# jxhe/vae-lagging-encoder

Measured on AMD Instinct MI355X. Metric: aggressive-loop seqs/sec, higher is better.
Workload: dtype bf16

## Files before the change

### include/lvae.h

```cpp
#ifndef LVAE_H
#define LVAE_H

#include <stdint.h>

#ifdef __cplusplus
extern "C" {
#endif

int lv_gemm_f32(int transA, int transB, int M, int N, int K, float alpha,
                const float* A, long lda, const float* B, long ldb, float* C, long ldc, int accumulate,
                const float* add1, long ld1, int mod1, const float* add2, long ld2, int mod2,
                float* ws , long ws_floats, void* stream);

int lv_gemm_bf16(int transA, int transB, int M, int N, int K, float alpha,
                 const float* A, long lda, const float* B, long ldb, float* C, long ldc, int accumulate,
                 const float* add1, long ld1, int mod1, const float* add2, long ld2, int mod2,
                 float* ws, long ws_floats, void* stream);

int lv_gemm_b16(int transA, int M, int N, int K, float alpha,
                const uint16_t* A, long lda, const uint16_t* B, long ldb, float* C, long ldc, int accumulate,
                const float* add1, long ld1, int mod1, const float* add2, long ld2, int mod2,
                float* ws, long ws_floats, void* stream);
int lv_gemm_b16_dual_supported(int M, int N, int K, long ws_floats);
int lv_gemm_b16_dual(int transA, int M, int N, int K, const uint16_t* A, long lda, const uint16_t* B, long ldb,
                     float* C1, long ldc1, int nsplit, float* C2, long ldc2, float* ws, long ws_floats, void* stream);
int lv_gemm_b16_pair_supported(int transA0, int M0, int N0, int K0, int transA1, int M1, int N1, int K1, long ws_floats);
int lv_gemm_b16_pair_pending(int* pending, void* stream);
int lv_gemm_b16_pair(int transA0, int M0, int N0, int K0, const uint16_t* A0, long lda0, const uint16_t* B0, long ldb0,
                     float* C0, long ldc0, int nsplit0, float* C0b, long ldc0b,
                     int transA1, int M1, int N1, int K1, const uint16_t* A1, long lda1, const uint16_t* B1, long ldb1,
                     float* C1, long ldc1, float* ws, long ws_floats, void* stream);
int lv_gemm_b16_keep(int M, int N, int K, const uint16_t* A, long lda, const uint16_t* B, long ldb, float* C,
                     const uint8_t* keep, float kscale, int Bsz, float* ws, long ws_floats, void* stream);
int lv_gemm_b16_sumsq_parts(int M, int N, int K, long ws_floats);
int lv_gemm_b16_sumsq(int transA, int M, int N, int K, const uint16_t* A, long lda, const uint16_t* B, long ldb, float* C, long ldc,
                      float* ws, long ws_floats, float* sq, int sq_only, void* stream);
int lv_gemm_b16_nll_parts(int N);
int lv_gemm_b16_tile(int tile, int transA, int M, int N, int K, float alpha,
                     const uint16_t* A, long lda, const uint16_t* B, long ldb, float* C, long ldc, int accumulate,
                     const float* add1, long ld1, int mod1, const float* add2, long ld2, int mod2,
                     float* ws, long ws_floats, void* stream);
int lv_gemm_b16_nll_tile(int tile, int M, int N, int K, const uint16_t* A, long lda, const uint16_t* B, long ldb, uint16_t* logits16,
                         long ldl16, const int64_t* ids, long ids_stride, int tgt_off, int Bsz, float* part, float* tgt_logit,
                         void* stream);
int lv_gemm_b16_nll(int M, int N, int K, const uint16_t* A, long lda, const uint16_t* B, long ldb, uint16_t* logits16, long ldl16,
                    const int64_t* ids, long ids_stride, int tgt_off, int Bsz, float* part, float* tgt_logit, void* stream);
int lv_softmax_nll_merge_f32(const float* part, int nparts, const float* tgt_logit, float* lse, float* nll, int R, void* stream);
int lv_softmax_nll_bwd_h16(const uint16_t* logits16, long ldl, const float* lse, const int64_t* ids, long ids_stride, int tgt_off,
                           const float* rowscale, uint16_t* dlogits, long ldo, int T, int B, int V, void* stream);
int lv_cvt_bf16_f32(const float* src, long lds, int R, int C, uint16_t* dst, long ldd, uint16_t* dstT, long ldt,
                    void* stream);
int lv_cvt_bf16_keep_f32(const float* src, long lds, int T, int Bsz, int C, const uint8_t* keep, float kscale,
                         uint16_t* dst, long ldd, uint16_t* dstT, long ldt, void* stream);
int lv_cvt_bf16_hs3_f32(const float* src, long lds, int T, int Bsz, int C, const uint8_t* keep, float kscale, uint16_t* dst, long ldd,
                        uint16_t* dstT, long ldt, uint16_t* hT, long ldh, void* stream);
int lv_cvt_f32_bf16_scaled(const uint16_t* src, long n, float scale, float* dst, void* stream);
int lv_keep_scale_f32(float* x, const uint8_t* keep, float kscale, int T, int Bsz, int C, void* stream);

int lv_cvt_bf16_gates_f32(const float* src, long lds, int H, int C, uint16_t* dst, long ldd, uint16_t* dstT, long ldt,
                          void* stream);
int lv_cvt_bf16_lo_f32(const float* src, long lds, int R, int C, int gate_H, const int64_t* ids, long ids_stride, int Bsz, int V,
                       uint16_t* dst, long ldd, uint16_t* dstT, long ldt, void* stream);
int lv_cvt_h16_f32(const float* src, long lds, int R, int C, int gate_H, const int64_t* ids, long ids_stride, int Bsz, int V,
                   uint16_t* dst, long ldd, uint16_t* dstT, long ldt, void* stream);
int lv_gemm_h16(int M, int N, int K, float alpha, const uint16_t* A, long lda, const uint16_t* B, long ldb,
                float* C, long ldc, int accumulate, const float* add1, long ld1, int mod1,
                const float* add2, long ld2, int mod2, float* ws, long ws_floats, void* stream);
int lv_transpose_f32(const float* in, float* out, int rows, int cols, void* stream);
int lv_transpose_ld_f32(const float* in, long in_ld, float* out, long out_ld, int rows, int cols, void* stream);

int lv_lstm_fwd_f32(const float* gx, const float* whh, float* hs, float* cs, float* gates,
                    const uint8_t* dmask, float dscale, float* hdrop, float* ws, int T, int B, int H, void* stream);
int lv_lstm_fwd_bf16(const float* gx, const float* whh, float* hs, float* cs, float* gates,
                     const uint8_t* dmask, float dscale, float* hdrop, float* ws, int T, int B, int H, void* stream);
int lv_lstm_fwd_bf16_ug(const float* gx, const float* whh, float* hs, float* cs, float* gates,
                        const uint8_t* dmask, float dscale, float* hdrop, float* ws, int T, int B, int H, void* stream);
int lv_lstm_fwd_f32_ug(const float* gx, const float* whh, float* hs, float* cs, float* gates,
                       const uint8_t* dmask, float dscale, float* hdrop, float* ws, int T, int B, int H, void* stream);
long lv_lstm_persist16_wpk_floats(void);
long lv_lstm_persist16_xch_floats(void);
int lv_lstm_persist16_xch_clear(float* xch, void* stream);
long lv_lstm_persist16_saved_floats(int T, int R);
int lv_lstm_persist16_pack(const float* whh, float* wpk, int backward, int H, void* stream);
int lv_lstm_persist16_pack2(const float* whh, float* wpk_fwd, float* wpk_bwd, int H, void* stream);
int lv_lstm_persist16_pack2_h16(const float* whh, float* wpk_fwd, float* wpk_bwd, int H, void* stream);
int lv_lstm_fwd_bf16_persist16(const float* gx, const float* wpk, float* hs, float* cs, float* saved, float* xch, int* status,
                               int T, int B, int R, int flags, int H, void* stream);
int lv_lstm_bwd_bf16_persist16(const float* dh_ext, const float* dh_last, const float* wpk, const float* saved, const float* hs,
                               const float* cs, uint16_t* dG16, float* dGsum, float* xch, int* status, float* dh0, float* dc0,
                               int tanh_init, int T, int B, int R, int flags, int H, void* stream);
int lv_lstm_persist16_import_saved(const float* gates, const float* cs, float* saved, int T, int B, int R, int H, void* stream);
int lv_gate_interleave_f32(const float* a, const float* b, int R, int H, float* out, void* stream);
int lv_lstm_bwd_bf16(const float* dh_ext, const float* dh_last, const uint8_t* dmask, float dscale,
                     const float* whh, const float* gates, const float* hs, const float* cs,
                     float* dG, float* dGsum, float* ws, float* dh0, float* dc0, int tanh_init,
                     int T, int B, int H, void* stream);
int lv_lstm_bwd_bf16_img(const float* dh_ext, const float* dh_last, const uint8_t* dmask, float dscale,
                           const float* whh, const float* gates, const float* hs, const float* cs,
                           float* dG, uint16_t* dG16, float* dGsum, float* ws, float* dh0, float* dc0, int tanh_init,
                           int T, int B, int H, void* stream);
long lv_lstm_ws_floats(int B, int H);
int lv_lstm_bwd_ksplit(int H);
int lv_lstm_bwd_f32(const float* dh_ext, const float* dh_last, const uint8_t* dmask, float dscale,
                    const float* whh, const float* gates, const float* hs, const float* cs,
                    float* dG, float* dGsum, float* ws, float* dh0, float* dc0, int tanh_init,
                    int T, int B, int H, void* stream);
int lv_lstm_fwd_len_f32(const float* gx, const float* whh, float* hs, float* cs, float* gates,
                        const uint8_t* dmask, float dscale, float* hdrop, float* ws,
                        const int* steps, int max_steps, int T, int B, int H, void* stream);
int lv_lstm_bwd_len_f32(const float* dh_ext, const float* dh_last, const uint8_t* dmask, float dscale,
                        const float* whh, const float* gates, const float* hs, const float* cs,
                        float* dG, float* dGsum, float* ws, float* dh0, float* dc0, int tanh_init,
                        const int* steps, int max_steps, int T, int B, int H, void* stream);
int lv_nll_mask_len_f32(float* nll, const int* steps, int max_steps, int T, int B, void* stream);

int lv_embed_gather_f32(const float* emb, const int64_t* ids, long ids_stride, const uint8_t* mask, float scale,
                        float* X, int T, int B, int ni, int V, void* stream);
int lv_embed_gather_b16(const float* emb, const int64_t* ids, long ids_stride, const uint8_t* keep, float kscale,
                        int T, int Bsz, int C, int V, uint16_t* dst, long ldd, uint16_t* dstT, long ldt, void* stream);
int lv_token_sort(const int64_t* ids, long ids_stride, int T, int B, int V,
                  int* out_rows, int* out_tok, int* tmp , void* stream);
int lv_embed_scatter_f32(const float* dX, const uint8_t* mask, float scale, const int* sorted_rows,
                         const int* sorted_tok, int T, int B, float* dE, int ni, int pad_idx, int accumulate,
                         void* stream);
int lv_embed_scatter_full_f32(const float* dX, const uint8_t* mask, float scale, const int* sorted_rows,
                              const int* sorted_tok, int T, int B, float* dE, int ni, int V, int pad_idx, void* stream);
int lv_embed_scatter_sumsq_parts(int T, int B);
int lv_embed_scatter_full_sumsq_f32(const float* dX, const uint8_t* mask, float scale, const int* sorted_rows,
                                    const int* sorted_tok, int T, int B, float* dE, int ni, int V, int pad_idx, float* sq, int sq_only,
                                    void* stream);
int lv_rows_merge_f32(const int64_t* ids_all, const void* rows_all, int b16, int world, int cap, int ni, int V, float scale,
                      float* dE, void* stream);

int lv_reparam_kl_fwd_f32(const float* mulv, const float* eps, float* z, float* kl, int B, int ns, int nz, void* stream);
int lv_reparam_kl_bwd_f32(const float* mulv, const float* eps, const float* dz, const float* dkl, float* dmulv,
                          int B, int ns, int nz, void* stream);

int lv_softmax_nll_fwd_f32(const float* logits, long ldl, const int64_t* ids, long ids_stride, int tgt_off,
                           float* lse, float* nll, int T, int B, int V, void* stream);
int lv_softmax_nll_bwd_f32(float* logits, long ldl, const float* lse, const int64_t* ids, long ids_stride, int tgt_off,
                           const float* rowscale, int T, int B, int V, void* stream);
int lv_softmax_nll_bwd_b16(const float* logits, long ldl, const float* lse, const int64_t* ids, long ids_stride, int tgt_off,
                           const float* rowscale, uint16_t* dlogits, long ldo, int T, int B, int V, void* stream);
int lv_vae_loss_f32(const float* nll, const float* kl, const float* kl_weight_dev, float* loss, float* rec,
                    int T, int B, void* stream);
int lv_loss_bwd_scales_f32(const float* g_loss, const float* g_rec, const float* g_kl, const float* kl_weight_dev,
                           float* rowscale, float* dkl, int B, void* stream);
int lv_loss_assemble_f32(const float* nll, const float* kl, const float* kl_weight_dev, const float* g_loss,
                         float* loss, float* rec, float* rowscale, float* dkl, float* acc_dev, int T, int B, void* stream);
int lv_loss_assemble_rng_f32(const float* nll, const float* kl, const float* kl_weight_dev, const float* g_loss,
                             float* loss, float* rec, float* rowscale, float* dkl, float* acc, int T, int B,
                             uint64_t* rng_state, uint64_t rng_inc, void* stream);

int lv_gx_expand_add_f32(const float* gxw, const float* zp, float* gx, int Td, int B, int ns, int C, void* stream);
int lv_sample_sum_f32(const float* dg, float* dgs, int Td, int B, int ns, int C, void* stream);
int lv_sample_sum_b16(const uint16_t* dg, long ld_in, uint16_t* dgs, long ld_out, int Td, int B, int ns, int C, void* stream);
int lv_repeat_rows_i64(const int64_t* x, int64_t* x_rep, int B, int T, int ns, void* stream);
int lv_loss_assemble_ns_f32(const float* nll, const float* kl, const float* kl_weight_dev, const float* g_loss,
                            float* loss, float* rec, float* rowscale, float* dkl, float* acc_dev, int T, int B, int ns,
                            void* stream);
int lv_loss_assemble_ns_rng_f32(const float* nll, const float* kl, const float* kl_weight_dev, const float* g_loss,
                                float* loss, float* rec, float* rowscale, float* dkl, float* acc_dev, int T, int B, int ns,
                                uint64_t* rng_state, uint64_t rng_inc, void* stream);

int lv_enc_head_fwd_f32(const float* hT, const float* w_lin, const float* eps, float* mulv, float* z, float* kl,
                        int B, int H, int ns, int nz, void* stream);
int lv_enc_head_bwd_f32(const float* mulv, const float* eps, const float* dz, int dz_parts, const float* dkl,
                        const float* hT, const float* w_lin, float* dmulv, float* dhT, float* gw_lin, int B, int H, int ns,
                        int nz, void* stream);
int lv_dec_init_f32(const float* z, const float* w_trans, const float* w_ih, long ld_wih, int col0, const float* b_ih,
                    const float* b_hh, float* c0, float* h0, float* zp, int unit_major, int B, int H, int nz, void* stream);
int lv_dec_tail_parts(int H);
int lv_dec_tail_bwd_f32(const float* dGsum, const float* dc0, const float* z, const float* w_ih, long ld_wih, int col0,
                        const float* w_trans, float* gw_ih, long ld_gwih, float* gw_trans, float* gb_ih, float* gb_hh,
                        float* dz_parts, int B, int H, int nz, void* stream);

int lv_tanh_f32(const float* in, float* out, long n, void* stream);
int lv_colsum_f32(const float* in, long ld, int R, int C, float* out, float* out2, void* stream);
int lv_add_f32(const float* a, const float* b, float* out, long n, void* stream);
int lv_sum_accum_f32(const float* x, long n, float* out_dev, void* stream);
int lv_add_scalar_f32(float* x_dev, float v, void* stream);

int lv_sumsq_workspace_floats(void);
int lv_sumsq_f32(const float* x, long n, float* ws, float* out_dev, int accumulate, void* stream);
int lv_clip_coef_f32(const float* sumsq_dev, float max_norm, float* coef_dev, float* norm_out_dev, void* stream);
int lv_clip_norm2_f32(const float* g1, long n1, const float* g2, long n2, float* ws, float max_norm,
                      float* sumsq_dev, float* coef_dev, float* norm_dev, void* stream);
int lv_sgd_step_f32(float* p, float* g, long n, const float* lr_dev, const float* coef_dev, int write_back_clipped,
                    void* stream);
int lv_scale_f32(float* x, long n, const float* coef_dev, void* stream);
int lv_clip_norm2_txn_f32(const float* g1, long n1, const float* g2, long n2, float* ws, float max_norm,
                          float* sumsq_dev, float* coef_dev, float* norm_dev, const int* status1, const int* status2,
                          const float* guard, float* txn, float* acc, void* stream);
int lv_clip_norm2_fold_txn_f32(const float* g1, long n1, const float* g2, long n2, float* ws, const float* extra, int n_extra,
                               float max_norm, float* sumsq_dev, float* coef_dev, float* norm_dev, const int* status1,
                               const int* status2, const float* guard, float* txn, float* acc, void* stream);
int lv_clip_coef_txn_f32(const float* sumsq_dev, float max_norm, float* coef_dev, float* norm_out_dev, const int* status1,
                         const int* status2, const float* guard, float* txn, float* acc, void* stream);
int lv_txn_guard_f32(const int* status1, const int* status2, float* guard, void* stream);
int lv_sgd_step_txn_f32(float* p, float* g, long n, const float* lr_dev, const float* coef_dev, int write_back_clipped,
                        const float* void_flag_dev, void* stream);
int lv_scale_txn_f32(float* x, long n, const float* coef_dev, const float* void_flag_dev, void* stream);
int lv_sgd_step_scale_txn_f32(float* p, float* g, long n, const float* lr_dev, const float* coef_dev, int write_back_clipped,
                              float* x2, long n2, const float* void_flag_dev, void* stream);
int lv_sgd_step_scale_rows_txn_f32(float* p, float* g, long n, const float* lr_dev, const float* coef_dev, int write_back_clipped,
                                   float* x2, long n2, const float* void_flag_dev, long emb_off, int V, int ni, const int* sorted_tok,
                                   int N, void* stream);
int lv_sgd_momentum_step_f32(float* p, float* g, float* buf, long n, const float* lr_dev, const float* coef_dev, float momentum,
                             int write_back_clipped, void* stream);
int lv_sgd_momentum_step_txn_f32(float* p, float* g, float* buf, long n, const float* lr_dev, const float* coef_dev, float momentum,
                                 int write_back_clipped, const float* void_flag_dev, void* stream);
int lv_sgd_momentum_step_scale_txn_f32(float* p, float* g, float* buf, long n, const float* lr_dev, const float* coef_dev, float momentum,
                                       int write_back_clipped, float* x2, long n2, const float* void_flag_dev, void* stream);
int lv_adam_step_f32(float* p, float* g, float* m, float* v, long n, const float* lr_dev, const float* coef_dev,
                     const float* step_dev, float beta1, float beta2, float eps, int write_back_clipped, void* stream);
int lv_adam_step_txn_f32(float* p, float* g, float* m, float* v, long n, const float* lr_dev, const float* coef_dev, float* step_dev,
                         double beta1, double beta2, float eps, int write_back_clipped, const float* void_flag_dev, void* stream);
int lv_adam_step_scale_txn_f32(float* p, float* g, float* m, float* v, long n, const float* lr_dev, const float* coef_dev,
                               float* step_dev, double beta1, double beta2, float eps, int write_back_clipped, float* x2, long n2,
                               const float* void_flag_dev, void* stream);

int lv_rng_normal_f32(float* out, long n, const uint64_t* state_dev, uint64_t substream, void* stream);
int lv_rng_keepmask_u8(uint8_t* out, long n, float keep_prob, const uint64_t* state_dev, uint64_t substream, void* stream);
int lv_rng_advance(uint64_t* state_dev, uint64_t inc, void* stream);
int lv_rng_noise_step(float* eps, long n_eps, uint8_t* mask_in, long n_in, float keep_in, uint8_t* mask_out, long n_out,
                      float keep_out, uint64_t* state_dev, uint64_t inc, void* stream);
int lv_rng_bernoulli_f32(const float* p, float* out, long n, const uint64_t* state_dev, uint64_t substream,
                         void* stream);

int lv_gauss_logpdf_f32(const float* z, const float* mu, const float* logvar, float* out, int B, int ns, int nz, void* stream);
int lv_logsumexp_rows_f32(const float* in, long ld, int R, int C, float add, float* out, void* stream);
int lv_calc_mi_f32(const float* mu, const float* logvar, const float* z, float* ws, float* out_dev, int Bx, int Bz, int nz,
                   void* stream);
int lv_au_accum_f32(const float* mu, const float* mean, float* acc_dev, int B, int nz, void* stream);

int lv_dec_cond_ll_f32_supported(int V, int ni, int H, int nz, int T);
long lv_dec_cond_ll_f32_ws_floats(int V, int H, int nz, int B, int T);
int lv_dec_cond_ll_f32(const int64_t* x, int B, int T, const float* z, long z_stride, int K, const float* embed,
                       const float* trans, const float* w_ih, const float* w_hh, const float* b_ih, const float* b_hh,
                       const float* pred, int V, int ni, int H, int nz, float* ws, float* cond_ll, void* stream);
// ... 120 lines not shown
```

### profiles/microbench/lstm_fixed_cost_probe.py

```python
import os, sys, torch
sys.path.insert(0, os.path.dirname(os.path.dirname(os.path.dirname(os.path.abspath(__file__)))))
from vae_lagging_encoder_amd import _lib
from vae_lagging_encoder_amd.engine import P, stream_ptr
dev = torch.device("cuda:0"); s = stream_ptr(dev)
lib = _lib.load()
H, B, R = 1024, 32, 4
whh = (torch.rand(4 * H, H, device=dev) * 2 - 1) * 0.03
n = lib.lv_lstm_persist16_wpk_floats()
wf, wb = torch.empty(n, device=dev), torch.empty(n, device=dev)
lib.lv_lstm_persist16_pack2(P(whh), P(wf), P(wb), H, s)
xch = torch.zeros(lib.lv_lstm_persist16_xch_floats(), device=dev)
st = torch.zeros(1, dtype=torch.int32, device=dev)
from types import SimpleNamespace
from vae_lagging_encoder_amd.engine import _xch_flags
wi = SimpleNamespace(xstate={"f": 0, "g": 0, "gcls": [0, 0]})


def t(f, n=20):
    for _ in range(3): f()
    e0, e1 = torch.cuda.Event(enable_timing=True), torch.cuda.Event(enable_timing=True)
    e0.record()
    for _ in range(n): f()
    e1.record(); torch.cuda.synchronize()
    return e0.elapsed_time(e1) * 1e3 / n


Ts = [1, 2, 4, 8, 16, 50, 100, 200]
rows = []
for mode in ("memset", "alternating halves"):
  rows = []
  lib.lv_lstm_persist16_xch_clear(P(xch), s)
  wi.xstate = {"f": 0, "g": 0, "gcls": [0, 0]}
  FF = (lambda: 1) if mode == "memset" else (lambda: 1 | _xch_flags(wi, "f", R, "cpu"))
  FB = (lambda: 1) if mode == "memset" else (lambda: 1 | _xch_flags(wi, "g", R, "cpu"))
  print("== exchange buffer: %s" % ("zeroed by a memset launch in front of every launch (round 4)" if mode == "memset" else
                                    "halves alternate, every launch clears the other half in its prologue (round 5)"))
  for T in Ts:
      gx = (torch.randn(T, B, 4 * H, device=dev) * 0.5)
      hs = torch.zeros(T + 1, B, H, device=dev); cs = torch.zeros(T + 1, B, H, device=dev)
      saved = torch.empty(lib.lv_lstm_persist16_saved_floats(T, R), device=dev)
      dO = torch.randn(T, B, H, device=dev) * 0.1
      dG16 = torch.empty(T, B, 4 * H, dtype=torch.int16, device=dev)
      dGsum = torch.empty(B, 4 * H, device=dev); dc0 = torch.empty(B, H, device=dev)
      f = t(lambda: lib.lv_lstm_fwd_bf16_persist16(P(gx), P(wf), P(hs), P(cs), P(saved), P(xch), P(st), T, B, R, FF(), H, s))
      b = t(lambda: lib.lv_lstm_bwd_bf16_persist16(P(dO), None, P(wb), P(saved), P(hs), P(cs), P(dG16), P(dGsum), P(xch), P(st), None, P(dc0), 1, T, B, R, FB(), H, s))
      rows.append((T, f, b))
      print("T=%3d: forward %7.1f us, BPTT %7.1f us (back-to-back launches)" % (T, f, b))
  import numpy as np
  A = np.array([[1.0, r[0]] for r in rows])
  for name, col in (("forward", 1), ("BPTT", 2)):
      a, b = np.linalg.lstsq(A, np.array([r[col] for r in rows]), rcond=None)[0]
      print("%s: fixed %.1f us per launch + %.3f us per timestep" % (name, a, b))
print("status", int(st.item()))
```

### vae_lagging_encoder_amd/_lib.py

```python
import ctypes
import os
import threading

from . import build as _build

_vp = ctypes.c_void_p
_i = ctypes.c_int
_l = ctypes.c_long
_f = ctypes.c_float
_d = ctypes.c_double
_u64 = ctypes.c_uint64

SIGNATURES = {
    "lv_gemm_f32": [_i, _i, _i, _i, _i, _f, _vp, _l, _vp, _l, _vp, _l, _i, _vp, _l, _i, _vp, _l, _i, _vp, _l, _vp],
    "lv_gemm_bf16": [_i, _i, _i, _i, _i, _f, _vp, _l, _vp, _l, _vp, _l, _i, _vp, _l, _i, _vp, _l, _i, _vp, _l, _vp],
    "lv_gemm_b16": [_i, _i, _i, _i, _f, _vp, _l, _vp, _l, _vp, _l, _i, _vp, _l, _i, _vp, _l, _i, _vp, _l, _vp],
    "lv_gemm_h16": [_i, _i, _i, _f, _vp, _l, _vp, _l, _vp, _l, _i, _vp, _l, _i, _vp, _l, _i, _vp, _l, _vp],
    "lv_gemm_b16_dual_supported": [_i, _i, _i, _l],
    "lv_gemm_b16_dual": [_i, _i, _i, _i, _vp, _l, _vp, _l, _vp, _l, _i, _vp, _l, _vp, _l, _vp],
    "lv_gemm_b16_pair_supported": [_i, _i, _i, _i, _i, _i, _i, _i, _l],
    "lv_gemm_b16_pair_pending": [_vp, _vp],
    "lv_gemm_b16_pair": [_i, _i, _i, _i, _vp, _l, _vp, _l, _vp, _l, _i, _vp, _l,
                         _i, _i, _i, _i, _vp, _l, _vp, _l, _vp, _l, _vp, _l, _vp],
    "lv_gemm_b16_keep": [_i, _i, _i, _vp, _l, _vp, _l, _vp, _vp, _f, _i, _vp, _l, _vp],
    "lv_gemm_b16_sumsq_parts": [_i, _i, _i, _l],
    "lv_gemm_b16_sumsq": [_i, _i, _i, _i, _vp, _l, _vp, _l, _vp, _l, _vp, _l, _vp, _i, _vp],
    "lv_gemm_b16_nll_parts": [_i],
    "lv_gemm_b16_tile": [_i, _i, _i, _i, _i, _f, _vp, _l, _vp, _l, _vp, _l, _i, _vp, _l, _i, _vp, _l, _i, _vp, _l, _vp],
    "lv_gemm_b16_nll_tile": [_i, _i, _i, _i, _vp, _l, _vp, _l, _vp, _l, _vp, _l, _i, _i, _vp, _vp, _vp],
    "lv_gemm_b16_nll": [_i, _i, _i, _vp, _l, _vp, _l, _vp, _l, _vp, _l, _i, _i, _vp, _vp, _vp],
    "lv_softmax_nll_merge_f32": [_vp, _i, _vp, _vp, _vp, _i, _vp],
    "lv_softmax_nll_bwd_h16": [_vp, _l, _vp, _vp, _l, _i, _vp, _vp, _l, _i, _i, _i, _vp],
    "lv_cvt_bf16_f32": [_vp, _l, _i, _i, _vp, _l, _vp, _l, _vp],
    "lv_cvt_bf16_keep_f32": [_vp, _l, _i, _i, _i, _vp, _f, _vp, _l, _vp, _l, _vp],
    "lv_cvt_bf16_hs3_f32": [_vp, _l, _i, _i, _i, _vp, _f, _vp, _l, _vp, _l, _vp, _l, _vp],
    "lv_cvt_f32_bf16_scaled": [_vp, _l, _f, _vp, _vp],
    "lv_keep_scale_f32": [_vp, _vp, _f, _i, _i, _i, _vp],
    "lv_cvt_bf16_gates_f32": [_vp, _l, _i, _i, _vp, _l, _vp, _l, _vp],
    "lv_cvt_bf16_lo_f32": [_vp, _l, _i, _i, _i, _vp, _l, _i, _i, _vp, _l, _vp, _l, _vp],
    "lv_cvt_h16_f32": [_vp, _l, _i, _i, _i, _vp, _l, _i, _i, _vp, _l, _vp, _l, _vp],
    "lv_gate_interleave_f32": [_vp, _vp, _i, _i, _vp, _vp],
    "lv_lstm_fwd_bf16_ug": [_vp, _vp, _vp, _vp, _vp, _vp, _f, _vp, _vp, _i, _i, _i, _vp],
    "lv_lstm_fwd_f32_ug": [_vp, _vp, _vp, _vp, _vp, _vp, _f, _vp, _vp, _i, _i, _i, _vp],
    "lv_loss_assemble_f32": [_vp, _vp, _vp, _vp, _vp, _vp, _vp, _vp, _vp, _i, _i, _vp],
    "lv_loss_assemble_rng_f32": [_vp, _vp, _vp, _vp, _vp, _vp, _vp, _vp, _vp, _i, _i, _vp, _u64, _vp],
    "lv_gx_expand_add_f32": [_vp, _vp, _vp, _i, _i, _i, _i, _vp],
    "lv_sample_sum_f32": [_vp, _vp, _i, _i, _i, _i, _vp],
    "lv_sample_sum_b16": [_vp, _l, _vp, _l, _i, _i, _i, _i, _vp],
    "lv_repeat_rows_i64": [_vp, _vp, _i, _i, _i, _vp],
    "lv_loss_assemble_ns_f32": [_vp, _vp, _vp, _vp, _vp, _vp, _vp, _vp, _vp, _i, _i, _i, _vp],
    "lv_loss_assemble_ns_rng_f32": [_vp, _vp, _vp, _vp, _vp, _vp, _vp, _vp, _vp, _i, _i, _i, _vp, _u64, _vp],
    "lv_enc_head_fwd_f32": [_vp, _vp, _vp, _vp, _vp, _vp, _i, _i, _i, _i, _vp],
    "lv_enc_head_bwd_f32": [_vp, _vp, _vp, _i, _vp, _vp, _vp, _vp, _vp, _vp, _i, _i, _i, _i, _vp],
    "lv_dec_tail_parts": [_i],
    "lv_dec_init_f32": [_vp, _vp, _vp, _l, _i, _vp, _vp, _vp, _vp, _vp, _i, _i, _i, _i, _vp],
    "lv_dec_tail_bwd_f32": [_vp, _vp, _vp, _vp, _l, _i, _vp, _vp, _l, _vp, _vp, _vp, _vp, _i, _i, _i, _vp],
    "lv_clip_norm2_f32": [_vp, _l, _vp, _l, _vp, _f, _vp, _vp, _vp, _vp],
    "lv_clip_norm2_txn_f32": [_vp, _l, _vp, _l, _vp, _f, _vp, _vp, _vp, _vp, _vp, _vp, _vp, _vp, _vp],
    "lv_clip_norm2_fold_txn_f32": [_vp, _l, _vp, _l, _vp, _vp, _i, _f, _vp, _vp, _vp, _vp, _vp, _vp, _vp, _vp, _vp],
    "lv_clip_coef_txn_f32": [_vp, _f, _vp, _vp, _vp, _vp, _vp, _vp, _vp, _vp],
    "lv_txn_guard_f32": [_vp, _vp, _vp, _vp],
    "lv_sgd_step_txn_f32": [_vp, _vp, _l, _vp, _vp, _i, _vp, _vp],
    "lv_scale_txn_f32": [_vp, _l, _vp, _vp, _vp],
    "lv_sgd_step_scale_txn_f32": [_vp, _vp, _l, _vp, _vp, _i, _vp, _l, _vp, _vp],
    "lv_sgd_step_scale_rows_txn_f32": [_vp, _vp, _l, _vp, _vp, _i, _vp, _l, _vp, _l, _i, _i, _vp, _i, _vp],
    "lv_sgd_momentum_step_f32": [_vp, _vp, _vp, _l, _vp, _vp, _f, _i, _vp],
    "lv_sgd_momentum_step_txn_f32": [_vp, _vp, _vp, _l, _vp, _vp, _f, _i, _vp, _vp],
    "lv_sgd_momentum_step_scale_txn_f32": [_vp, _vp, _vp, _l, _vp, _vp, _f, _i, _vp, _l, _vp, _vp],
    "lv_rng_noise_step": [_vp, _l, _vp, _l, _f, _vp, _l, _f, _vp, _u64, _vp],
    "lv_lstm_persist16_wpk_floats": [],
    "lv_lstm_persist16_xch_floats": [],
    "lv_lstm_persist16_xch_clear": [_vp, _vp],
    "lv_lstm_persist16_saved_floats": [_i, _i],
    "lv_lstm_persist16_pack": [_vp, _vp, _i, _i, _vp],
    "lv_lstm_persist16_import_saved": [_vp, _vp, _vp, _i, _i, _i, _i, _vp],
    "lv_lstm_persist16_pack2": [_vp, _vp, _vp, _i, _vp],
    "lv_lstm_persist16_pack2_h16": [_vp, _vp, _vp, _i, _vp],
    "lv_lstm_fwd_bf16_persist16": [_vp, _vp, _vp, _vp, _vp, _vp, _vp, _i, _i, _i, _i, _i, _vp],
    "lv_lstm_bwd_bf16_persist16": [_vp, _vp, _vp, _vp, _vp, _vp, _vp, _vp, _vp, _vp, _vp, _vp, _i, _i, _i, _i, _i, _i, _vp],
    "lv_transpose_f32": [_vp, _vp, _i, _i, _vp],
    "lv_transpose_ld_f32": [_vp, _l, _vp, _l, _i, _i, _vp],
    "lv_lstm_bwd_ksplit": [_i],
    "lv_lstm_ws_floats": [_i, _i],
    "lv_lstm_fwd_f32": [_vp, _vp, _vp, _vp, _vp, _vp, _f, _vp, _vp, _i, _i, _i, _vp],
    "lv_lstm_bwd_f32": [_vp, _vp, _vp, _f, _vp, _vp, _vp, _vp, _vp, _vp, _vp, _vp, _vp, _i, _i, _i, _i, _vp],
    "lv_lstm_fwd_len_f32": [_vp, _vp, _vp, _vp, _vp, _vp, _f, _vp, _vp, _vp, _i, _i, _i, _i, _vp],
    "lv_lstm_bwd_len_f32": [_vp, _vp, _vp, _f, _vp, _vp, _vp, _vp, _vp, _vp, _vp, _vp, _vp, _i, _vp, _i, _i, _i, _i, _vp],
    "lv_nll_mask_len_f32": [_vp, _vp, _i, _i, _i, _vp],
    "lv_lstm_fwd_bf16": [_vp, _vp, _vp, _vp, _vp, _vp, _f, _vp, _vp, _i, _i, _i, _vp],
    "lv_lstm_bwd_bf16": [_vp, _vp, _vp, _f, _vp, _vp, _vp, _vp, _vp, _vp, _vp, _vp, _vp, _i, _i, _i, _i, _vp],
    "lv_lstm_bwd_bf16_img": [_vp, _vp, _vp, _f, _vp, _vp, _vp, _vp, _vp, _vp, _vp, _vp, _vp, _vp, _i, _i, _i, _i, _vp],
    "lv_embed_gather_f32": [_vp, _vp, _l, _vp, _f, _vp, _i, _i, _i, _i, _vp],
    "lv_embed_gather_b16": [_vp, _vp, _l, _vp, _f, _i, _i, _i, _i, _vp, _l, _vp, _l, _vp],
    "lv_token_sort": [_vp, _l, _i, _i, _i, _vp, _vp, _vp, _vp],
    "lv_embed_scatter_f32": [_vp, _vp, _f, _vp, _vp, _i, _i, _vp, _i, _i, _i, _vp],
    "lv_embed_scatter_full_f32": [_vp, _vp, _f, _vp, _vp, _i, _i, _vp, _i, _i, _i, _vp],
    "lv_embed_scatter_sumsq_parts": [_i, _i],
    "lv_embed_scatter_full_sumsq_f32": [_vp, _vp, _f, _vp, _vp, _i, _i, _vp, _i, _i, _i, _vp, _i, _vp],
    "lv_rows_merge_f32": [_vp, _vp, _i, _i, _i, _i, _i, _f, _vp, _vp],
    "lv_reparam_kl_fwd_f32": [_vp, _vp, _vp, _vp, _i, _i, _i, _vp],
    "lv_reparam_kl_bwd_f32": [_vp, _vp, _vp, _vp, _vp, _i, _i, _i, _vp],
    "lv_softmax_nll_fwd_f32": [_vp, _l, _vp, _l, _i, _vp, _vp, _i, _i, _i, _vp],
    "lv_softmax_nll_bwd_f32": [_vp, _l, _vp, _vp, _l, _i, _vp, _i, _i, _i, _vp],
    "lv_softmax_nll_bwd_b16": [_vp, _l, _vp, _vp, _l, _i, _vp, _vp, _l, _i, _i, _i, _vp],
    "lv_vae_loss_f32": [_vp, _vp, _vp, _vp, _vp, _i, _i, _vp],
    "lv_loss_bwd_scales_f32": [_vp, _vp, _vp, _vp, _vp, _vp, _i, _vp],
    "lv_tanh_f32": [_vp, _vp, _l, _vp],
    "lv_colsum_f32": [_vp, _l, _i, _i, _vp, _vp, _vp],
    "lv_add_f32": [_vp, _vp, _vp, _l, _vp],
    "lv_sumsq_workspace_floats": [],
    "lv_sumsq_f32": [_vp, _l, _vp, _vp, _i, _vp],
    "lv_clip_coef_f32": [_vp, _f, _vp, _vp, _vp],
    "lv_sgd_step_f32": [_vp, _vp, _l, _vp, _vp, _i, _vp],
    "lv_scale_f32": [_vp, _l, _vp, _vp],
    "lv_adam_step_f32": [_vp, _vp, _vp, _vp, _l, _vp, _vp, _vp, _f, _f, _f, _i, _vp],
    "lv_adam_step_txn_f32": [_vp, _vp, _vp, _vp, _l, _vp, _vp, _vp, _d, _d, _f, _i, _vp, _vp],
    "lv_adam_step_scale_txn_f32": [_vp, _vp, _vp, _vp, _l, _vp, _vp, _vp, _d, _d, _f, _i, _vp, _l, _vp, _vp],
    "lv_add_scalar_f32": [_vp, _f, _vp],
    "lv_sum_accum_f32": [_vp, _l, _vp, _vp],
    "lv_gauss_logpdf_f32": [_vp, _vp, _vp, _vp, _i, _i, _i, _vp],
    "lv_logsumexp_rows_f32": [_vp, _l, _i, _i, _f, _vp, _vp],
    "lv_calc_mi_f32": [_vp, _vp, _vp, _vp, _vp, _i, _i, _i, _vp],
    "lv_au_accum_f32": [_vp, _vp, _vp, _i, _i, _vp],
    "lv_argmax_rows_f32": [_vp, _l, _i, _i, _vp, _vp],
    "lv_log_softmax_rows_f32": [_vp, _l, _i, _i, _vp, _vp, _l, _vp],
    "lv_sample_rows_f32": [_vp, _l, _i, _i, _vp, _vp, _vp],
    "lv_rng_normal_f32": [_vp, _l, _vp, _u64, _vp],
    "lv_rng_keepmask_u8": [_vp, _l, _f, _vp, _u64, _vp],
    "lv_rng_advance": [_vp, _u64, _vp],
    "lv_rng_bernoulli_f32": [_vp, _vp, _l, _vp, _u64, _vp],
    "lv_im2col_f32": [_vp, _vp, _l, _i, _i, _i, _i, _i, _i, _i, _i, _i, _i, _i, _vp],
    "lv_col2im_f32": [_vp, _l, _vp, _i, _i, _i, _i, _i, _i, _i, _i, _i, _i, _i, _i, _vp],
    "lv_conv_pack_w_f32": [_vp, _vp, _i, _i, _i, _vp],
    "lv_conv_unpack_dw_f32": [_vp, _vp, _i, _i, _i, _i, _vp],
    "lv_conv32_wpack_floats": [_i],
    "lv_conv32_pack_f32": [_vp, _vp, _i, _i, _i, _vp],
    "lv_conv32_f32": [_vp, _vp, _vp, _i, _i, _i, _i, _i, _vp],
    "lv_conv32_wgrad_slabs": [_i, _i],
    "lv_conv32_wgrad_ws_floats": [_i, _i],
    "lv_conv32_wgrad_f32": [_vp, _vp, _vp, _vp, _i, _i, _i, _vp],
    "lv_conv1x1_f32": [_vp, _vp, _vp, _l, _i, _i, _i, _i, _vp],
    "lv_conv1x1_wgrad_ws_floats": [_i, _i],
    "lv_conv32_pack_b16": [_vp, _vp, _i, _i, _i, _vp],
    "lv_conv32_b16": [_vp, _vp, _vp, _vp, _i, _i, _i, _i, _i, _i, _vp],
    "lv_conv32_bnbwd": [_vp, _vp, _vp, _vp, _i, _i, _i, _vp, _vp, _vp, _vp, _i, _i, _vp],
    "lv_conv1x1_bnbwd_f32": [_vp, _vp, _vp, _vp, _l, _i, _i, _vp, _vp, _vp, _vp, _i, _vp],
    "lv_bn_bwd_apply_partials_f32": [_vp, _vp, _vp, _i, _vp, _vp, _vp, _vp, _vp, _vp, _i, _l, _i, _vp],
    "lv_conv32_wgrad_b16": [_vp, _vp, _vp, _vp, _i, _i, _i, _i, _vp],
    "lv_conv32_wgrad_parts": [_i, _i],
    "lv_conv1x1_wgrad_parts": [_l],
    "lv_wgrad_reduce_batched": [_vp, _i, _vp],
    "lv_conv32_blocks": [_i],
    "lv_conv32_bnstat_f32": [_vp, _vp, _vp, _vp, _i, _i, _i, _vp],
    "lv_conv1x1_blocks": [_l],
    "lv_conv1x1_bnstat_f32": [_vp, _vp, _vp, _vp, _l, _i, _i, _vp],
    "lv_bn_fwd_partials_f32": [_vp, _vp, _vp, _vp, _i, _vp, _vp, _vp, _vp, _vp, _f, _f, _vp, _i, _l, _i, _vp],
    "lv_conv1x1_wgrad_f32": [_vp, _vp, _vp, _vp, _l, _i, _i, _i, _vp],
    "lv_mul_inplace_f32": [_vp, _vp, _l, _vp],
    "lv_bn_workspace_floats": [_i],
    "lv_pixelcnn_net_words": [],
    "lv_pixelcnn_block_words": [],
    "lv_pixelcnn_pixel_step_f32": [_vp, _i, _i, _i, _vp],
    "lv_conv32_tap_split": [_i],
    "lv_bn_eval_f32": [_vp, _vp, _vp, _vp, _vp, _f, _vp, _i, _vp, _vp, _vp, _l, _i, _vp],
    "lv_bn_fwd_f32": [_vp, _vp, _vp, _vp, _i, _vp, _vp, _vp, _vp, _vp, _f, _f, _vp, _l, _i, _vp],
    "lv_bn_bwd_f32": [_vp, _vp, _vp, _vp, _vp, _vp, _i, _vp, _vp, _vp, _vp, _i, _vp, _l, _i, _vp],
    "lv_bn_bwd2_f32": [_vp, _vp, _vp, _vp, _vp, _vp, _vp, _i, _vp, _vp, _vp, _vp, _i, _vp, _l, _i, _vp],
    "lv_bn_bwd4_f32": [_vp, _vp, _vp, _vp, _vp, _vp, _vp, _vp, _vp, _i, _vp, _vp, _vp, _vp, _i, _vp, _l, _i, _vp],
    "lv_sigmoid_bce_fwd_f32": [_vp, _vp, _vp, _i, _i, _f, _vp],
    "lv_sigmoid_bce_bwd_f32": [_vp, _vp, _vp, _vp, _i, _i, _f, _vp],
    "lv_dec_input_fwd_f32": [_vp, _vp, _vp, _i, _i, _i, _vp],
    "lv_dec_input_bwd_f32": [_vp, _vp, _i, _i, _i, _vp],
    "lv_sigmoid_bce_ns_fwd_f32": [_vp, _vp, _vp, _i, _i, _i, _f, _vp],
    "lv_sigmoid_bce_ns_bwd_f32": [_vp, _vp, _vp, _vp, _i, _i, _i, _f, _vp],
    "lv_dec_input_ns_fwd_f32": [_vp, _vp, _vp, _i, _i, _i, _i, _vp],
    "lv_bn_partial_floats": [_l, _i],
    "lv_bn_finish_fwd_f32": [_vp, _i, _l, _i, _f, _f, _vp, _vp, _vp, _vp, _vp],
    "lv_bn_fwd_stats_f32": [_vp, _vp, _vp, _vp, _i, _vp, _vp, _vp, _l, _i, _vp],
    "lv_bn_finish_bwd_f32": [_vp, _i, _i, _vp, _vp, _vp, _i, _vp],
    "lv_bn_bwd_stats_f32": [_vp, _vp, _vp, _vp, _vp, _vp, _vp, _l, _i, _vp],
    "lv_dec_cond_ll_f32_supported": [_i, _i, _i, _i, _i],
    "lv_dec_cond_ll_f32_ws_floats": [_i, _i, _i, _i, _i],
    "lv_dec_cond_ll_f32": [_vp, _i, _i, _vp, _l, _i, _vp, _vp, _vp, _vp, _vp, _vp, _vp, _i, _i, _i, _i, _vp, _vp, _vp],
    "lv_grid_posterior_f32": [_vp, _vp, _l, _i, _i, _i, _vp, _vp, _vp],
    "lv_mh_chain_f32_supported": [_i, _i, _i, _i, _i],
    "lv_mh_chain_f32_ws_floats": [_i, _i, _i, _i, _i],
    "lv_mh_chain_prep_f32": [_vp, _i, _i, _vp, _vp, _vp, _vp, _vp, _vp, _vp, _i, _i, _i, _i, _vp, _vp],
    "lv_mh_chain_f32": [_vp, _i, _i, _vp, _i, _i, _i, _i, _vp, _vp, _vp, _vp, _vp, _i, _i, _i, _i, _i, _f, _i, _vp, _vp, _vp, _vp],
    "lv_mh_step_f32": [_vp, _vp, _vp, _vp, _vp, _vp, _vp, _f, _vp, _i, _i, _i, _i, _i, _i, _vp, _vp, _vp],
    "lv_beam_supported": [_i, _i, _i],
    "lv_beam_ws_floats": [_i, _i, _i],
    "lv_beam_init_f32": [_vp, _vp, _vp, _vp, _vp, _vp, _vp, _vp, _vp, _vp, _i, _i, _i, _i, _i, _vp],
    "lv_beam_select_f32": [_vp, _l, _vp, _vp, _vp, _vp, _vp, _vp, _i, _i, _i, _vp],
    "lv_beam_advance_f32": [_vp, _vp, _vp, _vp, _vp, _vp, _vp, _vp, _vp, _vp, _vp, _vp, _vp, _i, _i, _i, _i, _i, _i, _i, _vp],
    "lv_beam_backtrace": [_vp, _vp, _vp, _vp, _vp, _vp, _vp, _vp, _i, _i, _i, _i, _vp],
    "lv_rollout_init_f32": [_vp, _vp, _vp, _vp, _vp, _vp, _vp, _vp, _vp, _vp, _i, _i, _i, _i, _vp],
    "lv_rollout_pick_f32": [_vp, _l, _vp, _vp, _vp, _vp, _vp, _vp, _vp, _vp, _vp, _vp, _vp, _vp, _i, _i, _i, _i, _i, _i, _vp],
}


_LONG_FNS = ("lv_lstm_ws_floats", "lv_conv1x1_wgrad_ws_floats", "lv_conv1x1_blocks", "lv_lstm_persist16_wpk_floats", "lv_lstm_persist16_xch_floats", "lv_lstm_persist16_saved_floats", "lv_conv32_wpack_floats",
             "lv_conv32_wgrad_ws_floats", "lv_dec_cond_ll_f32_ws_floats", "lv_beam_ws_floats", "lv_bn_partial_floats",
             "lv_mh_chain_f32_ws_floats")


class LvaeError(RuntimeError):
    pass


class Lib(object):

    def __init__(self, cdll, path):
        self.cdll = cdll
        self.path = path
        missing = []
        for name, argtypes in SIGNATURES.items():
            try:
                fn = getattr(cdll, name)
            except AttributeError:
                missing.append(name)
                continue
            fn.argtypes = argtypes
            fn.restype = ctypes.c_long if name in _LONG_FNS else ctypes.c_int
            setattr(self, "_raw_" + name, fn)
        if missing:
            raise LvaeError("%s does not export: %s" % (path, ", ".join(missing)))
        self._value_fns = {"lv_gemm_b16_dual_supported", "lv_gemm_b16_pair_supported", "lv_lstm_bwd_ksplit", "lv_dec_tail_parts", "lv_gemm_b16_nll_parts", "lv_gemm_b16_sumsq_parts", "lv_embed_scatter_sumsq_parts", "lv_conv32_wpack_floats",
                           "lv_conv32_wgrad_slabs", "lv_conv32_wgrad_ws_floats", "lv_conv32_wgrad_parts", "lv_conv1x1_wgrad_parts", "lv_conv32_blocks", "lv_conv1x1_blocks", "lv_conv1x1_wgrad_ws_floats", "lv_sumsq_workspace_floats", "lv_lstm_ws_floats", "lv_bn_workspace_floats",
                           "lv_lstm_persist16_wpk_floats", "lv_lstm_persist16_xch_floats", "lv_lstm_persist16_saved_floats",
                           "lv_pixelcnn_net_words", "lv_pixelcnn_block_words", "lv_conv32_tap_split", "lv_dec_cond_ll_f32_supported",
                           "lv_dec_cond_ll_f32_ws_floats", "lv_beam_supported", "lv_beam_ws_floats", "lv_bn_partial_floats",
# ... 47 lines not shown
```

### vae_lagging_encoder_amd/csrc/lv_device.h

```cpp
#pragma once

#ifdef LV_EMU
#include "hip_emu.h"
#define LV_LAUNCH(kern, grid, block, shmem, stream, ...) \
    lv_emu::launch((grid), (block), (shmem), [=]() { kern(__VA_ARGS__); })
#define LV_DYN_SHARED(name) char* name = lv_emu::dyn_smem()
static inline f32x4 lv_mfma_16x16x4(float a, float b, f32x4 c) { return lv_emu_mfma_16x16x4(a, b, c); }
static inline f32x16 lv_mfma_32x32x2(float a, float b, f32x16 c) { return lv_emu_mfma_32x32x2(a, b, c); }
#define LV_SCHED_BARRIER() do { } while (0)
static inline int lv_wave_uniform(int v) { return v; }
#define LV_LAUNCH_RESIDENT(kern, grid, block, shmem, stream, ...) \
    lv_emu::launch_concurrent((grid), (block), (shmem), [=]() { kern(__VA_ARGS__); })
#define LV_BLOCK_SHARED(T, name) T& name = *reinterpret_cast<T*>(lv_emu::block_shared(sizeof(T)))
static inline unsigned long long lv_agent_load_u64(const unsigned long long* p) {
    lv_emu::yield_all();
    return __atomic_load_n(p, __ATOMIC_RELAXED);
}
static inline void lv_agent_store_u64(unsigned long long* p, unsigned long long v) { __atomic_store_n(p, v, __ATOMIC_RELAXED); }
static inline void lv_xcd_store_u64(unsigned long long* p, unsigned long long v) { __atomic_store_n(p, v, __ATOMIC_RELAXED); }
static inline void lv_poll_backoff() { }
#define LV_WAIT_LDS() lv_emu::wave_sync()
template <class T> static inline void lv_store_nt(T v, T* p) { *p = v; }
static inline int lv_device_cus() { return 1 << 20; }
#define LV_SPIN_LIMIT (1 << 15)
// ... 30 lines not shown
    }
    lv_emu::wave_sync();
    uint2 r;
    memcpy(&r, o, 8);
    return r;
}
template <int SHIFT, int BANK> static inline float lv_row_shr_into(float old, float src) {
    auto& w = lv_emu::my_wave();
    const int l = lv_emu::lane();
    uint32_t b;
    memcpy(&b, &src, 4);
    w.u[l] = b;
    lv_emu::wave_sync();
    float out = old;
    if (((l & 15) >> 2) == BANK && (l & 15) >= SHIFT) { const uint32_t v = (uint32_t)w.u[l - SHIFT]; memcpy(&out, &v, 4); }
    lv_emu::wave_sync();
    return out;
}
static inline float lv_sat_f16(float x) { return x != x ? x : fminf(fmaxf(x, -65504.f), 65504.f); }
static inline uint16_t lv_f32_to_f16_bits(float x) {
    uint32_t u;
    memcpy(&u, &x, 4);
    const uint32_t sign = (u >> 16) & 0x8000u;
    u &= 0x7FFFFFFFu;
    if (u >= 0x7F800000u) return (uint16_t)(sign | (u > 0x7F800000u ? 0x7E00u : 0x7C00u));
    if (u >= 0x477FF000u) return (uint16_t)(sign | 0x7C00u);
    if (u < 0x33000001u) return (uint16_t)sign;
    if (u < 0x38800000u) {
        const int shift = 126 - (int)(u >> 23);
        const uint32_t mant = (u & 0x7FFFFFu) | 0x800000u;
        uint32_t h = mant >> shift;
        const uint32_t rem = mant & ((1u << shift) - 1u), half = 1u << (shift - 1);
        if (rem > half || (rem == half && (h & 1u))) ++h;
        return (uint16_t)(sign | h);
    }
    uint32_t h = ((u - 0x38000000u) >> 13);
    const uint32_t rem = u & 0x1FFFu;
    if (rem > 0x1000u || (rem == 0x1000u && (h & 1u))) ++h;
    return (uint16_t)(sign | h);
}
static inline float lv_f16_bits_to_f32(uint16_t h) {
    const uint32_t sign = ((uint32_t)h & 0x8000u) << 16, e = (h >> 10) & 0x1Fu, m = h & 0x3FFu;
    uint32_t u;
    if (e == 0) {
        if (m == 0) u = sign;
        else {
            int sh = 0;
            uint32_t mm = m;
            while (!(mm & 0x400u)) { mm <<= 1; ++sh; }
            u = sign | ((uint32_t)(113 - sh) << 23) | ((mm & 0x3FFu) << 13);
        }
    } else if (e == 31) u = sign | 0x7F800000u | (m << 13);
    else u = sign | ((e + 112u) << 23) | (m << 13);
    float f;
    memcpy(&f, &u, 4);
    return f;
}
static inline float lv_lane_xor1(float v) { return __shfl_xor(v, 1, 64); }
static inline uint32_t lv_lane_xor1_u32(uint32_t v) { return (uint32_t)__shfl_xor((int)v, 1, 64); }
template <int I> static inline uint32_t lv_quad_bcast_u32(uint32_t v) { return (uint32_t)lv_emu_xchg((int)v, (lv_emu::lane() & ~3) + I); }
static inline float lv_add_xor16(float x) { return x + __shfl_xor(x, 16, 64); }
static inline float lv_add_xor32(float x) { return x + __shfl_xor(x, 32, 64); }
static inline float lv_add_xor8(float x) { return x + __shfl_xor(x, 8, 64); }
static inline float lv_fold8(float x, float y) {
    const float xs = __shfl_xor(x, 8, 64), ys = __shfl_xor(y, 8, 64);
    return (lv_emu::lane() & 8) ? ys + y : x + xs;
}
static inline float lv_fold16(float x, float y) {
    const float xs = __shfl_xor(x, 16, 64), ys = __shfl_xor(y, 16, 64);
    return (lv_emu::lane() & 16) ? ys + y : x + xs;
}
static inline float lv_fold32(float x, float y) {
    const float xs = __shfl_xor(x, 32, 64), ys = __shfl_xor(y, 32, 64);
    return (lv_emu::lane() & 32) ? ys + y : x + xs;
}
static inline void lv_agent_load_q4x4(const void* p0, const void* p1, const void* p2, const void* p3, uint4 (&v)[4]) {
    lv_emu::yield_all();
    const void* ps[4] = {p0, p1, p2, p3};
    for (int i = 0; i < 4; ++i) {
        const unsigned* q = static_cast<const unsigned*>(ps[i]);
        v[i] = make_uint4(__atomic_load_n(q, __ATOMIC_RELAXED), __atomic_load_n(q + 1, __ATOMIC_RELAXED),
                          __atomic_load_n(q + 2, __ATOMIC_RELAXED), __atomic_load_n(q + 3, __ATOMIC_RELAXED));
    }
}
static inline void lv_agent_load_q4x8(const void* const (&ps)[8], uint4 (&v)[8]) {
    lv_emu::yield_all();
    for (int i = 0; i < 8; ++i) {
        const unsigned* q = static_cast<const unsigned*>(ps[i]);
        v[i] = make_uint4(__atomic_load_n(q, __ATOMIC_RELAXED), __atomic_load_n(q + 1, __ATOMIC_RELAXED),
                          __atomic_load_n(q + 2, __ATOMIC_RELAXED), __atomic_load_n(q + 3, __ATOMIC_RELAXED));
    }
}
static inline void lv_agent_load_q4x8_rows(const char* p, uint4 (&v)[8]) {
    const void* ps[8];
    for (int i = 0; i < 8; ++i) ps[i] = p + i * 4096;
    lv_agent_load_q4x8(ps, v);
}
template <int S> static inline void lv_agent_load_q4x8_rs(const char* p, uint4 (&v)[8]) {
    const void* ps[8];
    for (int i = 0; i < 8; ++i) ps[i] = p + (i & 3) * S + (i >> 2) * 128;
    lv_agent_load_q4x8(ps, v);
}
static inline void lv_agent_store_q4(void* p, uint4 v) {
    unsigned* q = static_cast<unsigned*>(p);
    __atomic_store_n(q + 2, v.z, __ATOMIC_RELAXED); __atomic_store_n(q + 3, v.w, __ATOMIC_RELAXED);
    lv_emu::yield_all();
    __atomic_store_n(q, v.x, __ATOMIC_RELAXED); __atomic_store_n(q + 1, v.y, __ATOMIC_RELAXED);
}
static inline void lv_xcd_store_q4(void* p, uint4 v) { lv_agent_store_q4(p, v); }
static inline uint32_t lv_pack_f16x2(float lo, float hi) { return (uint32_t)lv_f32_to_f16_bits(lo) | ((uint32_t)lv_f32_to_f16_bits(hi) << 16); }
static inline f32x16 lv_mfma_32x32x16_f16(uint4 a, uint4 b, f32x16 c) {
    auto& w = lv_emu::my_wave();
    const int l = lv_emu::lane();
    w.qa[l] = a; w.qb[l] = b;
    lv_emu::wave_sync();
    f32x16 d = c;
    const int col = l & 31;
    for (int r = 0; r < 16; ++r) {
        const int row = (r & 3) + 8 * (r >> 2) + 4 * (l >> 5);
        float acc = c[r];
        for (int h = 0; h < 2; ++h) {
            unsigned short ea[8], eb[8];
            memcpy(ea, &w.qa[row + 32 * h], 16);
            memcpy(eb, &w.qb[col + 32 * h], 16);
            for (int e = 0; e < 8; ++e) acc = fmaf(lv_f16_bits_to_f32(ea[e]), lv_f16_bits_to_f32(eb[e]), acc);
        }
        d[r] = acc;
    }
    lv_emu::wave_sync();
    return d;
}
static inline f32x4 lv_mfma_16x16x32_f16_areg(uint4 a, uint4 b, f32x4 c) {
    auto& w = lv_emu::my_wave();
    const int l = lv_emu::lane();
    w.qa[l] = a; w.qb[l] = b;
    lv_emu::wave_sync();
    f32x4 d = c;
    const int col = l & 15;
    for (int r = 0; r < 4; ++r) {
        const int row = (l >> 4) * 4 + r;
        float acc = c[r];
        for (int g = 0; g < 4; ++g) {
            unsigned short ea[8], eb[8];
            memcpy(ea, &w.qa[row + 16 * g], 16);
            memcpy(eb, &w.qb[col + 16 * g], 16);
            for (int e = 0; e < 8; ++e) acc = fmaf(lv_f16_bits_to_f32(ea[e]), lv_f16_bits_to_f32(eb[e]), acc);
        }
        d[r] = acc;
    }
    lv_emu::wave_sync();
    return d;
}
static inline f32x4 lv_mfma_16x16x32_f16_areg_first(uint4 a, uint4 b) { return lv_mfma_16x16x32_f16_areg(a, b, f32x4{0.f, 0.f, 0.f, 0.f}); }
#else
#include <hip/hip_runtime.h>
typedef float f32x4 __attribute__((ext_vector_type(4)));
typedef float f32x16 __attribute__((ext_vector_type(16)));
#define LV_LAUNCH(kern, grid, block, shmem, stream, ...) \
    hipLaunchKernelGGL(kern, (grid), (block), (shmem), (hipStream_t)(stream), __VA_ARGS__)
#define LV_DYN_SHARED(name) extern __shared__ __attribute__((aligned(16))) char name[]
#define LV_SCHED_BARRIER() __builtin_amdgcn_sched_barrier(0)
__device__ __forceinline__ int lv_wave_uniform(int v) { return __builtin_amdgcn_readfirstlane(v); }
#define LV_LAUNCH_RESIDENT(kern, grid, block, shmem, stream, ...) LV_LAUNCH(kern, grid, block, shmem, stream, __VA_ARGS__)
#define LV_BLOCK_SHARED(T, name) __shared__ T name
__device__ __forceinline__ unsigned long long lv_agent_load_u64(const unsigned long long* p) {
    return __hip_atomic_load(p, __ATOMIC_RELAXED, __HIP_MEMORY_SCOPE_AGENT);
}
__device__ __forceinline__ void lv_agent_store_u64(unsigned long long* p, unsigned long long v) {
    __hip_atomic_store(p, v, __ATOMIC_RELAXED, __HIP_MEMORY_SCOPE_AGENT);
}
__device__ __forceinline__ void lv_xcd_store_u64(unsigned long long* p, unsigned long long v) {
    __hip_atomic_store(p, v, __ATOMIC_RELAXED, __HIP_MEMORY_SCOPE_WORKGROUP);
}
#define LV_SPIN_LIMIT (1 << 22)
#define LV_WAIT_LDS() __builtin_amdgcn_s_waitcnt(0xc07f)
template <class T> __device__ __forceinline__ void lv_store_nt(T v, T* p) { __builtin_nontemporal_store(v, p); }
static inline int lv_device_cus() {
    static int cache[64];
    int dev = 0;
    if (hipGetDevice(&dev) != hipSuccess || dev < 0 || dev >= 64) return 0;
    int c = __atomic_load_n(&cache[dev], __ATOMIC_RELAXED);
    if (c == 0) {
        if (hipDeviceGetAttribute(&c, hipDeviceAttributeMultiprocessorCount, dev) != hipSuccess) return 0;
        __atomic_store_n(&cache[dev], c, __ATOMIC_RELAXED);
    }
    return c;
}
__device__ __forceinline__ f32x4 lv_mfma_16x16x4(float a, float b, f32x4 c) {
    return __builtin_amdgcn_mfma_f32_16x16x4f32(a, b, c, 0, 0, 0);
}
__device__ __forceinline__ f32x16 lv_mfma_32x32x2(float a, float b, f32x16 c) {
    return __builtin_amdgcn_mfma_f32_32x32x2f32(a, b, c, 0, 0, 0);
}
typedef __bf16 lv_bf16x8 __attribute__((ext_vector_type(8)));
__device__ __forceinline__ f32x16 lv_mfma_32x32x16_bf16(uint4 a, uint4 b, f32x16 c) {
    return __builtin_amdgcn_mfma_f32_32x32x16_bf16(*reinterpret_cast<lv_bf16x8*>(&a), *reinterpret_cast<lv_bf16x8*>(&b),
                                                   c, 0, 0, 0);
}
__device__ __forceinline__ f32x4 lv_mfma_16x16x32_bf16(uint4 a, uint4 b, f32x4 c) {
    return __builtin_amdgcn_mfma_f32_16x16x32_bf16(*reinterpret_cast<lv_bf16x8*>(&a), *reinterpret_cast<lv_bf16x8*>(&b),
                                                   c, 0, 0, 0);
}
typedef unsigned int lv_u32x4v __attribute__((ext_vector_type(4)));
__device__ __forceinline__ f32x4 lv_mfma_16x16x32_bf16_areg(uint4 a, uint4 b, f32x4 c) {
    const lv_u32x4v av = {a.x, a.y, a.z, a.w}, bv = {b.x, b.y, b.z, b.w};
    asm volatile("v_mfma_f32_16x16x32_bf16 %0, %1, %2, %0" : "+v"(c) : "a"(av), "v"(bv));
    return c;
}
__device__ __forceinline__ f32x4 lv_mfma_16x16x32_bf16_areg_first(uint4 a, uint4 b) {
    const lv_u32x4v av = {a.x, a.y, a.z, a.w}, bv = {b.x, b.y, b.z, b.w};
    f32x4 c;
    asm volatile("v_mfma_f32_16x16x32_bf16 %0, %1, %2, 0" : "=v"(c) : "a"(av), "v"(bv));
    return c;
}
typedef _Float16 lv_f16x8 __attribute__((ext_vector_type(8)));
__device__ __forceinline__ f32x16 lv_mfma_32x32x16_f16(uint4 a, uint4 b, f32x16 c) {
    return __builtin_amdgcn_mfma_f32_32x32x16_f16(*reinterpret_cast<lv_f16x8*>(&a), *reinterpret_cast<lv_f16x8*>(&b), c, 0, 0, 0);
}
__device__ __forceinline__ f32x4 lv_mfma_16x16x32_f16_areg(uint4 a, uint4 b, f32x4 c) {
    const lv_u32x4v av = {a.x, a.y, a.z, a.w}, bv = {b.x, b.y, b.z, b.w};
    asm volatile("v_mfma_f32_16x16x32_f16 %0, %1, %2, %0" : "+v"(c) : "a"(av), "v"(bv));
    return c;
}
__device__ __forceinline__ f32x4 lv_mfma_16x16x32_f16_areg_first(uint4 a, uint4 b) {
    const lv_u32x4v av = {a.x, a.y, a.z, a.w}, bv = {b.x, b.y, b.z, b.w};
    f32x4 c;
    asm volatile("v_mfma_f32_16x16x32_f16 %0, %1, %2, 0" : "=v"(c) : "a"(av), "v"(bv));
    return c;
}
#define LV_MFMA_DRAIN() asm volatile("s_nop 15\n\ts_nop 3" ::: "memory")
__device__ __forceinline__ void LV_MFMA_RESULT(f32x4& c) { asm volatile("" : "+v"(c)); }
typedef short lv_s16x4 __attribute__((ext_vector_type(4)));
__device__ __forceinline__ f32x4 lv_mfma_4x4x4_16b_bf16(uint2 a, uint2 b, f32x4 c) {
    return __builtin_amdgcn_mfma_f32_4x4x4bf16_1k(*reinterpret_cast<lv_s16x4*>(&a), *reinterpret_cast<lv_s16x4*>(&b), c, 0, 0, 0);
}
__device__ __forceinline__ void lv_glds16(const void* g, void* lds_wave_base) {
    __builtin_amdgcn_global_load_lds((const __attribute__((address_space(1))) void*)g,
                                     (__attribute__((address_space(3))) void*)lds_wave_base, 16, 0, 0);
}
#ifndef LV_GLDS_POLICY
#define LV_GLDS_POLICY ""
#endif
__device__ __forceinline__ void lv_glds16_uncounted(const void* g, void* lds_wave_base) {
    unsigned keep;
    const unsigned dst = (unsigned)__builtin_amdgcn_readfirstlane((int)(unsigned)(uintptr_t)(__attribute__((address_space(3))) void*)lds_wave_base);
    asm volatile("s_mov_b32 %0, m0\n\ts_mov_b32 m0, %2\n\ts_nop 0\n\tglobal_load_lds_dwordx4 %1, off" LV_GLDS_POLICY "\n\ts_mov_b32 m0, %0"
                 : "=&s"(keep) : "v"(g), "s"(dst) : "memory");
}
#define LV_WAIT_VMEM() asm volatile("s_waitcnt vmcnt(0)" ::: "memory")
typedef float lv_f32x4_wt __attribute__((ext_vector_type(4)));
__device__ __forceinline__ void lv_store_wt_f4(float4* p, float4 v) {
    const lv_f32x4_wt x = {v.x, v.y, v.z, v.w};
    asm volatile("global_store_dwordx4 %0, %1, off sc1\n\ts_nop 1" :: "v"(p), "v"(x) : "memory");
}
__device__ __forceinline__ void lv_acquire_agent() { __builtin_amdgcn_fence(__ATOMIC_ACQUIRE, "agent"); }
__device__ __forceinline__ unsigned lv_agent_load_u32(const unsigned* p) { return __hip_atomic_load(p, __ATOMIC_RELAXED, __HIP_MEMORY_SCOPE_AGENT); }
__device__ __forceinline__ void lv_sleep_short() { __builtin_amdgcn_s_sleep(8); }
#define LV_ARRIVAL_POLLS 64
#define LV_WAIT_VMEM_N(n) asm volatile("s_waitcnt vmcnt(" #n ")" ::: "memory")
#define LV_S_BARRIER() __builtin_amdgcn_s_barrier()
#define LV_SETPRIO(n) __builtin_amdgcn_s_setprio(n)
typedef short lv_s16x4_lds __attribute__((ext_vector_type(4)));
__device__ __forceinline__ uint2 lv_ds_read_tr16_b64(const void* lds_ptr) {
    lv_s16x4_lds v = __builtin_amdgcn_ds_read_tr16_b64_v4i16((__attribute__((address_space(3))) lv_s16x4_lds*)lds_ptr);
    return *reinterpret_cast<uint2*>(&v);
}
__device__ __forceinline__ float lv_sat_f16(float x) { return x != x ? x : fminf(fmaxf(x, -65504.f), 65504.f); }
__device__ __forceinline__ uint16_t lv_f32_to_f16_bits(float x) {
    const _Float16 h = (_Float16)x;
    uint16_t b;
    __builtin_memcpy(&b, &h, 2);
    return b;
}
__device__ __forceinline__ float lv_f16_bits_to_f32(uint16_t b) {
    _Float16 h;
    __builtin_memcpy(&h, &b, 2);
    return (float)h;
}
__device__ __forceinline__ float lv_lane_xor1(float v) {
    const int r = __builtin_amdgcn_update_dpp(0, __builtin_bit_cast(int, v), 0xB1, 0xF, 0xF, true);
    return __builtin_bit_cast(float, r);
}
__device__ __forceinline__ uint32_t lv_lane_xor1_u32(uint32_t v) {
    return (uint32_t)__builtin_amdgcn_update_dpp(0, (int)v, 0xB1, 0xF, 0xF, true);
}
template <int I> __device__ __forceinline__ uint32_t lv_quad_bcast_u32(uint32_t v) {
    return (uint32_t)__builtin_amdgcn_update_dpp(0, (int)v, I * 0x55, 0xF, 0xF, true);
}
__device__ __forceinline__ float lv_add_xor16(float x) {
    const auto r = __builtin_amdgcn_permlane16_swap(__builtin_bit_cast(unsigned, x), __builtin_bit_cast(unsigned, x), false, false);
    return __builtin_bit_cast(float, (unsigned)r[0]) + __builtin_bit_cast(float, (unsigned)r[1]);
}
__device__ __forceinline__ float lv_add_xor32(float x) {
    const auto r = __builtin_amdgcn_permlane32_swap(__builtin_bit_cast(unsigned, x), __builtin_bit_cast(unsigned, x), false, false);
    return __builtin_bit_cast(float, (unsigned)r[0]) + __builtin_bit_cast(float, (unsigned)r[1]);
}
__device__ __forceinline__ float lv_add_xor8(float x) {
    const int r = __builtin_amdgcn_update_dpp(0, __builtin_bit_cast(int, x), 0x128, 0xF, 0xF, true);
    return x + __builtin_bit_cast(float, r);
}
__device__ __forceinline__ float lv_fold8(float x, float y) {
    const float xs = lv_add_xor8(x), ys = lv_add_xor8(y);
    return (threadIdx.x & 8) ? ys : xs;
}
__device__ __forceinline__ float lv_fold16(float x, float y) {
    const auto r = __builtin_amdgcn_permlane16_swap(__builtin_bit_cast(unsigned, x), __builtin_bit_cast(unsigned, y), false, false);
    return __builtin_bit_cast(float, (unsigned)r[0]) + __builtin_bit_cast(float, (unsigned)r[1]);
}
__device__ __forceinline__ float lv_fold32(float x, float y) {
    const auto r = __builtin_amdgcn_permlane32_swap(__builtin_bit_cast(unsigned, x), __builtin_bit_cast(unsigned, y), false, false);
    return __builtin_bit_cast(float, (unsigned)r[0]) + __builtin_bit_cast(float, (unsigned)r[1]);
}
__device__ __forceinline__ void lv_agent_load_q4x4(const void* p0, const void* p1, const void* p2, const void* p3, uint4 (&v)[4]) {
    lv_u32x4v r0, r1, r2, r3;
    asm volatile("global_load_dwordx4 %0, %4, off sc1\n\tglobal_load_dwordx4 %1, %5, off sc1\n\tglobal_load_dwordx4 %2, %6, off sc1\n\t"
                 "global_load_dwordx4 %3, %7, off sc1\n\ts_waitcnt vmcnt(0)"
                 : "=&v"(r0), "=&v"(r1), "=&v"(r2), "=&v"(r3) : "v"(p0), "v"(p1), "v"(p2), "v"(p3) : "memory");
    v[0] = make_uint4(r0.x, r0.y, r0.z, r0.w); v[1] = make_uint4(r1.x, r1.y, r1.z, r1.w);
    v[2] = make_uint4(r2.x, r2.y, r2.z, r2.w); v[3] = make_uint4(r3.x, r3.y, r3.z, r3.w);
}
__device__ __forceinline__ void lv_agent_load_q4x8(const void* const (&ps)[8], uint4 (&v)[8]) {
    lv_u32x4v r0, r1, r2, r3, r4, r5, r6, r7;
    asm volatile("global_load_dwordx4 %0, %8, off sc1\n\tglobal_load_dwordx4 %1, %9, off sc1\n\tglobal_load_dwordx4 %2, %10, off sc1\n\t"
                 "global_load_dwordx4 %3, %11, off sc1\n\tglobal_load_dwordx4 %4, %12, off sc1\n\tglobal_load_dwordx4 %5, %13, off sc1\n\t"
                 "global_load_dwordx4 %6, %14, off sc1\n\tglobal_load_dwordx4 %7, %15, off sc1\n\ts_waitcnt vmcnt(0)"
                 : "=&v"(r0), "=&v"(r1), "=&v"(r2), "=&v"(r3), "=&v"(r4), "=&v"(r5), "=&v"(r6), "=&v"(r7)
                 : "v"(ps[0]), "v"(ps[1]), "v"(ps[2]), "v"(ps[3]), "v"(ps[4]), "v"(ps[5]), "v"(ps[6]), "v"(ps[7]) : "memory");
    v[0] = make_uint4(r0.x, r0.y, r0.z, r0.w); v[1] = make_uint4(r1.x, r1.y, r1.z, r1.w);
    v[2] = make_uint4(r2.x, r2.y, r2.z, r2.w); v[3] = make_uint4(r3.x, r3.y, r3.z, r3.w);
    v[4] = make_uint4(r4.x, r4.y, r4.z, r4.w); v[5] = make_uint4(r5.x, r5.y, r5.z, r5.w);
    v[6] = make_uint4(r6.x, r6.y, r6.z, r6.w); v[7] = make_uint4(r7.x, r7.y, r7.z, r7.w);
}
__device__ __forceinline__ void lv_agent_load_q4x8_rows(const char* p, uint4 (&v)[8]) {
    const char *p1 = p + 4096, *p3 = p + 3 * 4096, *p5 = p + 5 * 4096, *p7 = p + 7 * 4096;
    lv_u32x4v r0, r1, r2, r3, r4, r5, r6, r7;
    asm volatile("global_load_dwordx4 %0, %8, off offset:-4096 sc1\n\tglobal_load_dwordx4 %1, %8, off sc1\n\t"
                 "global_load_dwordx4 %2, %9, off offset:-4096 sc1\n\tglobal_load_dwordx4 %3, %9, off sc1\n\t"
                 "global_load_dwordx4 %4, %10, off offset:-4096 sc1\n\tglobal_load_dwordx4 %5, %10, off sc1\n\t"
                 "global_load_dwordx4 %6, %11, off offset:-4096 sc1\n\tglobal_load_dwordx4 %7, %11, off sc1\n\ts_waitcnt vmcnt(0)"
                 : "=&v"(r0), "=&v"(r1), "=&v"(r2), "=&v"(r3), "=&v"(r4), "=&v"(r5), "=&v"(r6), "=&v"(r7)
                 : "v"(p1), "v"(p3), "v"(p5), "v"(p7) : "memory");
    v[0] = make_uint4(r0.x, r0.y, r0.z, r0.w); v[1] = make_uint4(r1.x, r1.y, r1.z, r1.w);
    v[2] = make_uint4(r2.x, r2.y, r2.z, r2.w); v[3] = make_uint4(r3.x, r3.y, r3.z, r3.w);
    v[4] = make_uint4(r4.x, r4.y, r4.z, r4.w); v[5] = make_uint4(r5.x, r5.y, r5.z, r5.w);
    v[6] = make_uint4(r6.x, r6.y, r6.z, r6.w); v[7] = make_uint4(r7.x, r7.y, r7.z, r7.w);
}
template <int S> __device__ __forceinline__ void lv_agent_load_q4x8_rs(const char* p, uint4 (&v)[8]) {
    static_assert(3 * S + 128 < 8192, "two address registers reach 8 KB");
    const char* const ph = p + 4096;
#define LV_RS_O(i) (((i) & 3) * S + ((i) >> 2) * 128)
#define LV_RS_P(i) (LV_RS_O(i) < 4096 ? p : ph)
    lv_u32x4v r0, r1, r2, r3, r4, r5, r6, r7;
    asm volatile("global_load_dwordx4 %0, %8, off offset:%16 sc1\n\tglobal_load_dwordx4 %1, %9, off offset:%17 sc1\n\t"
                 "global_load_dwordx4 %2, %10, off offset:%18 sc1\n\tglobal_load_dwordx4 %3, %11, off offset:%19 sc1\n\t"
                 "global_load_dwordx4 %4, %12, off offset:%20 sc1\n\tglobal_load_dwordx4 %5, %13, off offset:%21 sc1\n\t"
                 "global_load_dwordx4 %6, %14, off offset:%22 sc1\n\tglobal_load_dwordx4 %7, %15, off offset:%23 sc1\n\ts_waitcnt vmcnt(0)"
                 : "=&v"(r0), "=&v"(r1), "=&v"(r2), "=&v"(r3), "=&v"(r4), "=&v"(r5), "=&v"(r6), "=&v"(r7)
                 : "v"(LV_RS_P(0)), "v"(LV_RS_P(1)), "v"(LV_RS_P(2)), "v"(LV_RS_P(3)), "v"(LV_RS_P(4)), "v"(LV_RS_P(5)), "v"(LV_RS_P(6)), "v"(LV_RS_P(7)),
                   "n"(LV_RS_O(0) & 4095), "n"(LV_RS_O(1) & 4095), "n"(LV_RS_O(2) & 4095), "n"(LV_RS_O(3) & 4095),
                   "n"(LV_RS_O(4) & 4095), "n"(LV_RS_O(5) & 4095), "n"(LV_RS_O(6) & 4095), "n"(LV_RS_O(7) & 4095)
                 : "memory");
#undef LV_RS_O
#undef LV_RS_P
    v[0] = make_uint4(r0.x, r0.y, r0.z, r0.w); v[1] = make_uint4(r1.x, r1.y, r1.z, r1.w);
    v[2] = make_uint4(r2.x, r2.y, r2.z, r2.w); v[3] = make_uint4(r3.x, r3.y, r3.z, r3.w);
    v[4] = make_uint4(r4.x, r4.y, r4.z, r4.w); v[5] = make_uint4(r5.x, r5.y, r5.z, r5.w);
    v[6] = make_uint4(r6.x, r6.y, r6.z, r6.w); v[7] = make_uint4(r7.x, r7.y, r7.z, r7.w);
}
__device__ __forceinline__ void lv_agent_store_q4(void* p, uint4 v) {
    const lv_u32x4v d = {v.x, v.y, v.z, v.w};
    asm volatile("global_store_dwordx4 %0, %1, off sc1\n\ts_nop 1" :: "v"(p), "v"(d) : "memory");
}
#ifndef LV_POLL_SLEEP
#define LV_POLL_SLEEP 0
#endif
__device__ __forceinline__ void lv_poll_backoff() { if (LV_POLL_SLEEP > 0) __builtin_amdgcn_s_sleep(LV_POLL_SLEEP); }
#ifndef LV_XCD_ST_MODS
#define LV_XCD_ST_MODS ""
#endif
__device__ __forceinline__ void lv_xcd_store_q4(void* p, uint4 v) {
// ... 99 lines not shown
```

### vae_lagging_encoder_amd/csrc/lv_lstm_persist16.hip

```cpp
#include "lv_device.h"
#include "lv_persist_common.h"

#if defined(LV_TRACE) && !defined(LV_EMU)
__device__ unsigned long long* lv_trace_buf = nullptr;
extern "C" int lv_trace_set(void* p) { return (int)hipMemcpyToSymbol(HIP_SYMBOL(lv_trace_buf), &p, sizeof(p)); }
#endif

#ifndef LV_SBB16
#define LV_SBB16 8
#endif
#ifndef LV_HB16
#define LV_HB16 2
#endif
#ifndef LV_SBK16
#define LV_SBK16 4
#endif
#ifndef LV_GJ16
#define LV_GJ16 16
#endif
#ifndef LV_FWD_Q
#define LV_FWD_Q 2
#endif
#ifndef LV_RS_Q
#define LV_RS_Q 2
#endif
#ifndef LV_P16_ABL
#define LV_P16_ABL 0
#endif

namespace {

using namespace lvp;

__device__ __forceinline__ float abl_u2f(uint32_t u) { float f; memcpy(&f, &u, 4); return f; }

constexpr int HP16 = PH / 2 + 8;
constexpr int DP16 = 64 + 8;
constexpr int RED_SLOTS = 33;
constexpr int SAVED_PER_ROW = 160;
constexpr int RS16_SLOTS_MAX = 256;
template <int V> struct lv_const { static constexpr int value = V; };

__global__ __launch_bounds__(256) void pack_w_k16_kernel(const float* __restrict__ whh, uint4* __restrict__ wpk, int f16);
__global__ __launch_bounds__(256) void pack_w_rs16_kernel(const float* __restrict__ whh, uint4* __restrict__ wpk);

__device__ __forceinline__ void pack_w_k16_one(const float* __restrict__ whh, uint4* __restrict__ wpk, long idx, int f16 = 0) {
    const int l = (int)(idx & 63), nb = (int)((idx >> 6) & 7), ks = (int)((idx >> 9) & 7);
    const int wave_id = (int)(idx >> 12), m = wave_id >> 2, w = wave_id & 3;
    const int c = l & 15, kq = l >> 4, col = 16 * nb + c;
    const float* row = whh + ((long)(col & 3) * PH + 32 * m + (col >> 2)) * PH + 256 * w + 32 * ks + 8 * kq;
    if (f16) {
        float r[8];
#pragma unroll
        for (int e = 0; e < 8; ++e) r[e] = lv_sat_f16(row[e]);
        wpk[idx] = make_uint4(lv_pack_f16x2(r[0], r[1]), lv_pack_f16x2(r[2], r[3]), lv_pack_f16x2(r[4], r[5]), lv_pack_f16x2(r[6], r[7]));
    }
    else
        wpk[idx] = make_uint4(lv_pack_bf16x2(row[0], row[1]), lv_pack_bf16x2(row[2], row[3]), lv_pack_bf16x2(row[4], row[5]),
                              lv_pack_bf16x2(row[6], row[7]));
}
__device__ __forceinline__ void pack_w_rs16_one(const float* __restrict__ whh, uint4* __restrict__ wpk, long idx) {
    const int l = (int)(idx & 63), nb = (int)((idx >> 6) & 15), ks = (int)((idx >> 10) & 3);
    const int wave_id = (int)(idx >> 12), m = wave_id >> 2, w = wave_id & 3;
    const int c = l & 15, kq = l >> 4, j = 256 * w + 16 * nb + c;
    float v[8];
#pragma unroll
    for (int e = 0; e < 8; ++e) {
        const int n2 = 32 * ks + 8 * kq + e;
        v[e] = whh[((long)(n2 & 3) * PH + 32 * m + (n2 >> 2)) * PH + j];
    }
    wpk[idx] = make_uint4(lv_pack_bf16x2(v[0], v[1]), lv_pack_bf16x2(v[2], v[3]), lv_pack_bf16x2(v[4], v[5]), lv_pack_bf16x2(v[6], v[7]));
}
__global__ __launch_bounds__(256) void pack_w_both16_kernel(const float* __restrict__ whh, uint4* __restrict__ wfwd, uint4* __restrict__ wbwd,
                                                            int fwd_f16) {
    const long n = 128L * 64 * 64;
    const long idx = (long)blockIdx.x * 256 + threadIdx.x;
    if (idx < n) pack_w_k16_one(whh, wfwd, idx, fwd_f16);
    else if (idx < 2 * n) pack_w_rs16_one(whh, wbwd, idx - n);
}

__global__ __launch_bounds__(256) void pack_w_k16_kernel(const float* __restrict__ whh, uint4* __restrict__ wpk, int f16) {
    const long idx = (long)blockIdx.x * 256 + threadIdx.x;
    if (idx < 128L * 8 * 8 * 64) pack_w_k16_one(whh, wpk, idx, f16);
}
__global__ __launch_bounds__(256) void pack_w_rs16_kernel(const float* __restrict__ whh, uint4* __restrict__ wpk) {
    const long idx = (long)blockIdx.x * 256 + threadIdx.x;
    if (idx < 128L * 4 * 16 * 64) pack_w_rs16_one(whh, wpk, idx);
}

struct Fwd16P {
    const float* gx; const uint4* wpk;
    float* hs; float* cs; float* saved;
    gran_t* hx;
    int* status;
    int T, B, R;
    uint4* clr; long clr_n;
};

__device__ __forceinline__ void clear_other_half(uint4* q, long n) {
    if (!q) return;
    const long stride = (long)gridDim.x * blockDim.x;
    for (long i = (long)blockIdx.x * blockDim.x + threadIdx.x; i < n; i += stride) q[i] = make_uint4(0u, 0u, 0u, 0u);
}

template <int RP> struct Cfg16 {
    static constexpr int NP = RP > 8 ? 2 : 1;
    static constexpr int SBK = RP > 8 ? LV_SBK16 : 8;
    static constexpr int SBB = RP > 8 ? LV_SBB16 : 8;
    static constexpr int GJ = RP > 8 ? LV_GJ16 : (RP > 4 ? 16 : 8);
};

template <int RP>
struct __attribute__((aligned(16))) Fwd16Lds {
    uint32_t hl[RP * HP16];
    f32x4 red[2][4][RP][RED_SLOTS];
    uint32_t dump[256];
    int abort;
};

template <int RP, bool LOCAL, bool F16 = false>
__global__ __launch_bounds__(256) void lstm_fwd_persist_k16_kernel(Fwd16P p) {
    auto h16 = [](float v) -> uint32_t { return F16 ? (uint32_t)lv_f32_to_f16_bits(v) : lv_f32_to_bf16_bits(v); };
    auto put = [](gran_t* q, gran_t v) { if (LOCAL) lv_xcd_store_u64(q, v); else gran_store(q, v); };
    constexpr int NP = Cfg16<RP>::NP, SBK = Cfg16<RP>::SBK, GJ = Cfg16<RP>::GJ;
    LV_BLOCK_SHARED(Fwd16Lds<RP>, sm);
    int& s_abort = sm.abort;
    const int tid = (int)threadIdx.x, l = tid & 63, w = tid >> 6;
    const int group = (int)blockIdx.x % PGROUPS, member = (int)blockIdx.x / PGROUPS;
    const int wave_id = member * 4 + w;
    const int B = p.B, R = p.R, T = p.T;
    const int b0 = group * R;
    const int rows = (b0 >= B) ? 0 : ((B - b0) < R ? (B - b0) : R);
    clear_other_half(p.clr, p.clr_n);
    if (rows == 0) return;
    if (tid == 0) s_abort = 0;

    uint4 wreg[8][8];
    {
        const uint4* wp = p.wpk + (long)wave_id * 8 * 8 * 64 + l;
#pragma unroll
        for (int ks = 0; ks < 8; ++ks)
#pragma unroll
            for (int nb = 0; nb < 8; ++nb) wreg[ks][nb] = wp[(ks * 8 + nb) * 64];
    }

    const int uw = tid & 31, punit = 32 * member + uw;
    const long BH = (long)B * PH;
    const long rec = (long)R * SAVED_PER_ROW;
    float* const sv = p.saved + (long)(group * PMEMBERS + member) * T * rec;
    int prow[NP]; bool own[NP]; long pidx[NP]; float c_state[NP]; int sg[NP], sc[NP];
#pragma unroll
    for (int q = 0; q < NP; ++q) {
        prow[q] = (tid >> 5) + 8 * q;
        own[q] = prow[q] < rows;
        pidx[q] = (long)(b0 + (own[q] ? prow[q] : 0)) * PH + punit;
        c_state[q] = own[q] ? p.cs[pidx[q]] : 0.f;
        sg[q] = (prow[q] * 32 + uw) * 4;
        sc[q] = R * 128 + prow[q] * 32 + uw;
    }
    gran_t* const hx_g = p.hx + (long)group * 16 * (PH / 2);
    const long hx_par = (long)PGROUPS * 16 * (PH / 2);
    const bool even = !(uw & 1);

    constexpr bool QF = LV_FWD_Q == 2 || (RP == 4 && LV_FWD_Q == 1);
    auto tagq = [](int state) -> uint32_t { return 1u + (uint32_t)state % 0xFFFFu; };
    auto publish_q = [&](int state, int q, float hval) {
        const uint32_t dw = h16(hval) | (tagq(state) << 16);
        const uint32_t d1 = lv_quad_bcast_u32<1>(dw), d2 = lv_quad_bcast_u32<2>(dw), d3 = lv_quad_bcast_u32<3>(dw);
        if (own[q] && !(uw & 3)) {
            char* d = reinterpret_cast<char*>(hx_g + (long)(state & 1) * hx_par + (long)prow[q] * (PH / 2)) + (punit >> 2) * 16;
            if (LOCAL) lv_xcd_store_q4(d, make_uint4(dw, d1, d2, d3)); else lv_agent_store_q4(d, make_uint4(dw, d1, d2, d3));
        }
    };
#pragma unroll
    for (int q = 0; q < NP; ++q) {
        if constexpr (QF) { publish_q(0, q, own[q] ? p.hs[pidx[q]] : 0.f); continue; }
        const uint32_t mine = h16(own[q] ? p.hs[pidx[q]] : 0.f);
        const uint32_t next = lv_lane_xor1_u32(mine);
        if (own[q] && even) put(hx_g + (long)prow[q] * (PH / 2) + (punit >> 1), ((gran_t)1u << 32) | (gran_t)(mine | (next << 16)));
    }

    float4 gxb[NP][SBK];
    f32x4 recb[NP][SBK];
    float cb[NP][SBK], hb[NP][SBK];
    auto load_slots = [&](int tb, int lo, int hi) {
#pragma unroll
        for (int q = 0; q < NP; ++q)
#pragma unroll
            for (int s2 = 0; s2 < SBK; ++s2) {
                if (s2 < lo || s2 >= hi) continue;
                const int t = tb + s2 < T ? tb + s2 : T - 1;
                gxb[q][s2] = *reinterpret_cast<const float4*>(p.gx + ((long)t * BH + pidx[q]) * 4);
            }
    };
    auto store_block = [&](int tb) {
#pragma unroll
        for (int q = 0; q < NP; ++q)
#pragma unroll
            for (int s2 = 0; s2 < SBK; ++s2) {
                const int t = tb + s2;
                if (own[q] && t < T) {
                    lv_store_nt(recb[q][s2],
                                reinterpret_cast<f32x4*>(sv + (long)t * rec + sg[q]));
                    lv_store_nt(cb[q][s2], sv + (long)t * rec + sc[q]);
                    lv_store_nt(hb[q][s2], p.hs + (long)(t + 1) * BH + pidx[q]);
                    if (t == T - 1) p.cs[(long)T * BH + pidx[q]] = cb[q][s2];
                }
            }
    };
    load_slots(0, 0, SBK);
    __syncthreads();

    const int nq = rows * 128;
    const int brow = (l & 15) < rows ? (l & 15) : 0;
    const int kq = l >> 4;
    uint32_t abl_keep[8] = {0u, 0u, 0u, 0u, 0u, 0u, 0u, 0u};
    for (int tb = 0; tb < T; tb += SBK) {
#pragma unroll
        for (int s2 = 0; s2 < SBK; ++s2) {
            const int t = tb + s2;
            if (t >= T) break;
            LV_TRACE_MARK(t, 0);
            const gran_t* src = hx_g + (long)(t & 1) * hx_par + 128 * w;
            const uint32_t want = (uint32_t)(t + 1);
            if constexpr (QF) {
                constexpr int QR = RP == 4 ? 4 : 8;
                const char* sq = reinterpret_cast<const char*>(hx_g + (long)(t & 1) * hx_par) + (64 * w + l) * 16;
                const long rowb = (long)(PH / 2) * 8;
                const uint32_t wq = tagq(t) << 16;
                auto round = [&](auto R0) {
                    constexpr int r0 = decltype(R0)::value;
                    if (r0 >= rows) return;
                    uint4 v[QR];
                    int spins = 0;
                    bool ok;
                    do {
                        if constexpr (QR == 4)
                            lv_agent_load_q4x4(sq, sq + (rows > 1 ? rowb : 0), sq + (rows > 2 ? 2 * rowb : 0), sq + (rows > 3 ? 3 * rowb : 0), v);
                        else {
                            static_assert((PH / 2) * 8 == 4096, "lv_agent_load_q4x8_rows: rows 4 KB apart");
                            lv_agent_load_q4x8_rows(sq + r0 * rowb, reinterpret_cast<uint4 (&)[8]>(v));
                        }
                        uint32_t x = 0u;
#pragma unroll
                        for (int j = 0; j < QR; ++j)
                            if (r0 + j < rows) x |= (v[j].x ^ wq) | (v[j].y ^ wq) | (v[j].z ^ wq) | (v[j].w ^ wq);
                        ok = (LV_P16_ABL & 2) ? true : (x >> 16) == 0u;
                        ok = __all(ok);
                        if (!ok && ++spins > SPIN_LIMIT) { s_abort = 1; break; }
                        if (!ok) lv_poll_backoff();
                    } while (!ok);
                    LV_TRACE_VAL(t, 6, spins);
#pragma unroll
                    for (int j = 0; j < QR; ++j)
                        if (r0 + j < rows)
                            *reinterpret_cast<uint2*>(&sm.hl[(r0 + j) * HP16 + 128 * w + 2 * l]) =
                                make_uint2((v[j].x & 0xFFFFu) | (v[j].y << 16), (v[j].z & 0xFFFFu) | (v[j].w << 16));
                };
                round(lv_const<0>());
                if constexpr (RP > QR) round(lv_const<QR>());
            } else
            for (int base = 0; base < nq; base += 64 * GJ) {
                gran_t v[GJ];
                int spins = 0;
                bool ok;
                do {
                    ok = true;
#pragma unroll
                    for (int j = 0; j < GJ; ++j) {
                        const int q = base + j * 64 + l;
                        const bool in = q < nq;
                        if constexpr (LV_P16_ABL & 32) { v[j] = ((gran_t)want << 32) | (gran_t)(uint32_t)(q + t); continue; }
                        v[j] = gran_load(src + (in ? (q >> 7) * (PH / 2) + (q & 127) : 0));
                        if (!(LV_P16_ABL & 2)) ok = ok && (!in || (uint32_t)(v[j] >> 32) == want);
                    }
                    ok = __all(ok);
                    if (!ok && ++spins > SPIN_LIMIT) { s_abort = 1; break; }
                } while (!ok);
                LV_TRACE_VAL(t, 6, spins);
                if constexpr (LV_P16_ABL & 16) {
#pragma unroll
                    for (int j = 0; j < GJ; ++j) abl_keep[j & 7] ^= (uint32_t)v[j];
                } else {
#pragma unroll
                for (int j = 0; j < GJ; ++j) {
                    const int q = base + j * 64 + l;
                    uint32_t* dstw = q < nq ? &sm.hl[(q >> 7) * HP16 + 128 * w + (q & 127)] : &sm.dump[tid];
                    *dstw = (uint32_t)v[j];
                }
                }
            }
            if (s2 == 0 && tb > 0) { store_block(tb - SBK); load_slots(tb, SBK - 1, SBK); }
            if (s2 == SBK - 1) load_slots(tb + SBK, 0, SBK - 1);
            LV_TRACE_MARK(t, 1);
            LV_WAIT_LDS();
            LV_TRACE_MARK(t, 2);

            f32x4 acc[8];
            const uint4* bp = reinterpret_cast<const uint4*>(sm.hl + brow * HP16 + 128 * w) + kq;
            uint4 bfr[8];
            if constexpr (LV_P16_ABL & 16) {
#pragma unroll
                for (int ks = 0; ks < 8; ++ks) bfr[ks] = make_uint4(abl_keep[ks], abl_keep[(ks + 1) & 7], abl_keep[(ks + 2) & 7], abl_keep[(ks + 3) & 7]);
            } else {
#pragma unroll
            for (int ks = 0; ks < 8; ++ks) bfr[ks] = bp[ks * 4];
            }
            LV_SCHED_BARRIER();
            if constexpr (LV_P16_ABL & 1) {
#pragma unroll
                for (int nb = 0; nb < 8; ++nb) acc[nb] = f32x4{abl_u2f(bfr[nb].x), abl_u2f(bfr[nb].y), 0.f, 0.f};
            } else {
#pragma unroll
            for (int ks = 0; ks < 8; ++ks)
#pragma unroll
                for (int nb = 0; nb < 8; ++nb)
                    if constexpr (F16)
                        acc[nb] = ks == 0 ? lv_mfma_16x16x32_f16_areg_first(wreg[0][nb], bfr[0]) : lv_mfma_16x16x32_f16_areg(wreg[ks][nb], bfr[ks], acc[nb]);
                    else
                        acc[nb] = ks == 0 ? lv_mfma_16x16x32_bf16_areg_first(wreg[0][nb], bfr[0]) : lv_mfma_16x16x32_bf16_areg(wreg[ks][nb], bfr[ks], acc[nb]);
            LV_MFMA_DRAIN();
#pragma unroll
            for (int nb = 0; nb < 8; ++nb) LV_MFMA_RESULT(acc[nb]);
            }
            if ((l & 15) < RP) {
                f32x4* rd = sm.red[t & 1][w][l & 15];
#pragma unroll
                for (int nb = 0; nb < 8; ++nb) rd[4 * nb + kq] = acc[nb];
            }
            LV_TRACE_MARK(t, 3);
            if (!(LV_P16_ABL & 8))
            __syncthreads();
            LV_TRACE_MARK(t, 4);
            if (s_abort) { if (tid == 0) atomicExch(p.status, 100 + t); return; }

#pragma unroll
            for (int q = 0; q < NP; ++q) {
                float h = 0.f;
                if (own[q]) {
                    const f32x4 q0 = sm.red[t & 1][0][prow[q]][uw], q1 = sm.red[t & 1][1][prow[q]][uw];
                    const f32x4 q2 = sm.red[t & 1][2][prow[q]][uw], q3 = sm.red[t & 1][3][prow[q]][uw];
                    const float4 gxv = gxb[q][s2];
                    auto sg_ = [](float x) { return (LV_P16_ABL & 4) ? 0.5f + 0.25f * x : lv_sigmoid_fast(x); };
                    auto th_ = [](float x) { return (LV_P16_ABL & 4) ? 0.9f * x : lv_tanh_fast(x); };
                    const float ig = sg_(gxv.x + ((q0[0] + q1[0]) + (q2[0] + q3[0])));
                    const float fg = sg_(gxv.y + ((q0[1] + q1[1]) + (q2[1] + q3[1])));
                    const float gg = th_(gxv.z + ((q0[2] + q1[2]) + (q2[2] + q3[2])));
                    const float og = sg_(gxv.w + ((q0[3] + q1[3]) + (q2[3] + q3[3])));
                    const float c = fg * c_state[q] + ig * gg;
                    h = og * th_(c);
                    c_state[q] = c;
                    recb[q][s2] = f32x4{ig, fg, gg, og};
                    cb[q][s2] = c; hb[q][s2] = h;
                }
                if constexpr (QF) { publish_q(t + 1, q, h); continue; }
                const uint32_t mine = h16(h);
                const uint32_t next = lv_lane_xor1_u32(mine);
                if (own[q] && even)
                    put(hx_g + (long)((t + 1) & 1) * hx_par + (long)prow[q] * (PH / 2) + (punit >> 1),
                        ((gran_t)(uint32_t)(t + 2) << 32) | (gran_t)(mine | (next << 16)));
            }
            LV_TRACE_MARK(t, 5);
        }
    }
    store_block((T - 1) / SBK * SBK);
}

struct Bwd16P {
    const float* dh_ext; const float* dh_last;
    const uint4* wpk;
    const float* saved; const float* cs; const float* hs;
    uint16_t* dG16; float* dGsum;
    float* dh0; float* dc0; int tanh_init;
    gran_t* gxch;
    int* status;
    int T, B, R;
    uint4* clr; long clr_n;
};

template <int RP>
struct __attribute__((aligned(16))) Bwd16Lds {
    uint32_t dgl[2][16 * DP16];
    uint16_t og[2][RP][4][32];
    int abort;
};

template <int RP, bool LOCAL, bool HAS_EXT>
__global__ __launch_bounds__(256) void lstm_bwd_persist_rs16_kernel(Bwd16P p) {
    auto put = [](gran_t* q, gran_t v) { if (LOCAL) lv_xcd_store_u64(q, v); else gran_store(q, v); };
    constexpr int NP = Cfg16<RP>::NP, SBK = Cfg16<RP>::SBB;
    constexpr int NB = RP / 4;
    constexpr int SLOTS = 16 * RP;
    LV_BLOCK_SHARED(Bwd16Lds<RP>, sm);
    int& s_abort = sm.abort;
    const int tid = (int)threadIdx.x, l = tid & 63, w = tid >> 6;
    const int group = (int)blockIdx.x % PGROUPS, member = (int)blockIdx.x / PGROUPS;
    const int wave_id = member * 4 + w;
    const int B = p.B, R = p.R, T = p.T;
    const int b0 = group * R;
    const int rows = (b0 >= B) ? 0 : ((B - b0) < R ? (B - b0) : R);
    clear_other_half(p.clr, p.clr_n);
    if (rows == 0) return;
    if (tid == 0) s_abort = 0;
    for (int i = tid; i < 2 * 16 * DP16; i += 256) sm.dgl[0][i] = 0u;

    uint4 wreg[4][16];
    {
        const uint4* wp = p.wpk + (long)wave_id * 4 * 16 * 64 + l;
#pragma unroll
        for (int ks = 0; ks < 4; ++ks)
#pragma unroll
            for (int nb = 0; nb < 16; ++nb) wreg[ks][nb] = wp[(ks * 16 + nb) * 64];
    }

    constexpr bool QB = LV_RS_Q == 2 || (RP == 4 && LV_RS_Q == 1);
    constexpr bool Q4 = RP == 4 && QB;
    const int pp = l & 15;
    const int uw = QB ? 16 * (w >> 1) + 4 * (l & 3) + 2 * ((l >> 4) & 1) + (l >> 5)
                      : 16 * (w >> 1) + 4 * (pp & 3) + 2 * (w & 1) + ((l >> 4) & 1);
    const int punit = 32 * member + uw;
    const long BH = (long)B * PH;
    const long rec = (long)R * SAVED_PER_ROW;
    const float* const sv = p.saved + (long)(group * PMEMBERS + member) * T * rec;
    int prow[NP]; bool own[NP]; long pidx[NP]; int sg[NP], sc[NP];
#pragma unroll
    for (int q = 0; q < NP; ++q) {
        const int beta = 2 * q + (l >> 5);
        prow[q] = Q4 ? 2 * (w & 1) + ((l & 7) >> 2) : QB ? (RP / 2) * (w & 1) + 4 * q + 2 * ((l >> 3) & 1) + ((l >> 2) & 1) : 4 * beta + (pp >> 2);
        own[q] = (Q4 ? !(l & 8) : QB ? true : beta < NB) && prow[q] < rows;
        pidx[q] = (long)(b0 + (own[q] ? prow[q] : 0)) * PH + punit;
        sg[q] = ((own[q] ? prow[q] : 0) * 32 + uw) * 4;
        sc[q] = R * 128 + (own[q] ? prow[q] : 0) * 32 + uw;
    }
    const long px_par = (long)PGROUPS * PMEMBERS * PMEMBERS * SLOTS;
    gran_t* const px_g = p.gxch + (long)group * PMEMBERS * PMEMBERS * SLOTS;
    const gran_t* const rx = px_g + ((long)member * PMEMBERS + 8 * (l >> 4)) * SLOTS + 4 * RP * w + pp;
    gran_t* const tx = px_g + ((long)(8 * w) * PMEMBERS + member) * SLOTS + 4 * (l & 15) + (l >> 4);
    gran_t* const tx4 = px_g + ((long)(8 * w + (((l & 15) >> 2) >> 1)) * PMEMBERS + member) * SLOTS + 2 * (((l & 15) >> 2) & 1) * 4 * RP +
                        4 * (l & 3) + (l >> 4);

    const char* const rx_q = reinterpret_cast<const char*>(px_g) + ((long)member * PMEMBERS + 4 * (l >> 3)) * SLOTS * 8 + (2 * RP * w + (l & 7)) * 16;
    char* const tx_q = RP == 4 ? reinterpret_cast<char*>(px_g) + ((long)(8 * w + (((l & 15) >> 2) >> 1)) * PMEMBERS + member) * SLOTS * 8 +
                                     ((((l & 15) >> 2) & 1) * 16 + 4 * (l & 3) + (l >> 4)) * 16
                               : reinterpret_cast<char*>(px_g) + ((long)(8 * w) * PMEMBERS + member) * SLOTS * 8 + (4 * (l & 15) + (l >> 4)) * 16;
    float dc_rec[NP], gsum[NP][4];
    float dhb[HAS_EXT ? NP : 1][HAS_EXT ? SBK : 1], ctb[NP][SBK + 1];
    float4 recb[NP][SBK];
#pragma unroll
    for (int q = 0; q < NP; ++q) { dc_rec[q] = 0.f; gsum[q][0] = gsum[q][1] = gsum[q][2] = gsum[q][3] = 0.f; }
    auto load_block = [&](int t_hi) {
#pragma unroll
        for (int q = 0; q < NP; ++q) {
#pragma unroll
            for (int s2 = 0; s2 < SBK; ++s2) {
                const int t = t_hi - s2 < 0 ? 0 : t_hi - s2;
                if constexpr (HAS_EXT) dhb[q][s2] = p.dh_ext[(long)t * BH + pidx[q]];
                recb[q][s2] = *reinterpret_cast<const float4*>(sv + (long)t * rec + sg[q]);
            }
#pragma unroll
            for (int s2 = 0; s2 <= SBK; ++s2) {
                const int t = t_hi - s2;
                const float* src = t >= 0 ? sv + (long)t * rec + sc[q] : p.cs + pidx[q];
                ctb[q][s2] = *src;
            }
        }
    };
    auto store_step = [&](int par, int t) {
        for (int c = tid; c < RP * 16; c += 256) {
            const int qq = c & 3, g = (c >> 2) & 3, r = c >> 4;
            if (r < rows) {
                const f32x4 v = *reinterpret_cast<const f32x4*>(&sm.og[par][r][g][8 * qq]);
                uint16_t* dst = p.dG16 + ((long)t * B + (b0 + r)) * 4 * PH + (long)g * PH + 32 * member + 8 * qq;
                lv_store_nt(v, reinterpret_cast<f32x4*>(dst));
            }
        }
    };
    load_block(T - 1);
    __syncthreads();

    const int brow = l & 15, kq = l >> 4;
    const bool closing = p.dh0 || p.tanh_init;

    constexpr int HB = NB < LV_HB16 ? NB : LV_HB16;
    LV_TRACE_ONLY(int tr_spins[2] = {0, 0};)
    auto receive_round = [&](auto H0, const gran_t* src, uint32_t want, float (&dh_rec)[NP]) -> bool {
        constexpr int h0 = decltype(H0)::value;
        gran_t v[HB][8];
        int spins = 0;
        bool ok;
        do {
            ok = true;
#pragma unroll
            for (int bt = 0; bt < HB; ++bt)
#pragma unroll
                for (int j = 0; j < 8; ++j) {
                    v[bt][j] = gran_load(src + (long)j * SLOTS + 16 * (h0 + bt));
                    if (!(LV_P16_ABL & 2)) ok = ok && (uint32_t)(v[bt][j] >> 56) == want;
                }
            ok = __all(ok);
            if (!ok && ++spins > SPIN_LIMIT) { s_abort = 1; return false; }
        } while (!ok);
        LV_TRACE_ONLY(tr_spins[h0 ? 1 : 0] = spins;)
#pragma unroll
        for (int bt = 0; bt < HB; ++bt) {
            float a = 0.f, b = 0.f;
#pragma unroll
            for (int j = 0; j < 8; ++j) { a += rs_lo(v[bt][j]); b += rs_hi(v[bt][j]); }
            a = lv_add_xor16(a); b = lv_add_xor16(b);
            a = lv_add_xor32(a); b = lv_add_xor32(b);
            if ((l >> 5) == ((h0 + bt) & 1)) dh_rec[(h0 + bt) >> 1] = (l & 16) ? b : a;
        }
        return true;
    };
    auto receive_q4 = [&](int k, float (&dh_rec)[NP]) -> bool {
// ... 199 lines not shown
            LV_TRACE_MARK(t, 2);
            if (!(LV_P16_ABL & 8))
            __syncthreads();
            LV_TRACE_MARK(t, 3);
            if (s_abort) { aborted = true; continue; }
            if (t > 0 || closing) send(par, T - t);
            store_step(par, t);
            LV_TRACE_MARK(t, 4);
        }
        if (aborted) { if (tid == 0) atomicExch(p.status, 200 + (t_hi < 0 ? 0 : t_hi)); return; }
    }

#pragma unroll
    for (int q = 0; q < NP; ++q)
        if (own[q]) {
#pragma unroll
            for (int g = 0; g < 4; ++g) p.dGsum[(long)(b0 + prow[q]) * 4 * PH + (long)g * PH + punit] = gsum[q][g];
        }
    if (closing) {
        float s0[NP];
        const bool fine = receive(T, s0);
        __syncthreads();
        if (!fine || s_abort) { if (tid == 0) atomicExch(p.status, 300); return; }
#pragma unroll
        for (int q = 0; q < NP; ++q)
            if (own[q]) {
                if (p.dh0) p.dh0[pidx[q]] = s0[q];
                float dc = dc_rec[q];
                if (p.tanh_init) { const float h0 = p.hs[pidx[q]]; dc += s0[q] * (1.f - h0 * h0); }
                if (p.dc0) p.dc0[pidx[q]] = dc;
            }
    } else {
#pragma unroll
        for (int q = 0; q < NP; ++q)
            if (own[q] && p.dc0) p.dc0[pidx[q]] = dc_rec[q];
    }
}

constexpr long XCH_FWD16_BYTES = 2L * PGROUPS * 16 * (PH / 2) * 8;
constexpr long XCH_RS16_BYTES = 2L * PGROUPS * PMEMBERS * PMEMBERS * RS16_SLOTS_MAX * 8;

int check_R(int B, int R) { return R >= 1 && R <= 16 && (long)R * PGROUPS >= B; }

}

constexpr long XCH_FWD_OFF[2] = {0, XCH_FWD16_BYTES};
constexpr long XCH_BWD_OFF[2] = {2 * XCH_FWD16_BYTES, 2 * XCH_FWD16_BYTES + XCH_RS16_BYTES};
extern "C" long lv_lstm_persist16_xch_floats(void) { return (2 * XCH_FWD16_BYTES + 2 * XCH_RS16_BYTES) / 4 + 64; }
extern "C" int lv_lstm_persist16_xch_clear(float* xch, void* stream) {
    if (!xch) return LV_ERR_ARG;
    return (int)hipMemsetAsync(xch, 0, (size_t)(2 * XCH_FWD16_BYTES + 2 * XCH_RS16_BYTES), (hipStream_t)stream);
}
extern "C" long lv_lstm_persist16_wpk_floats(void) { return 128L * 64 * 64 * 16 / 4; }

extern "C" long lv_lstm_persist16_saved_floats(int T, int R) {
    return T < 0 || R < 1 || R > 16 ? 0 : (long)PGROUPS * PMEMBERS * T * R * SAVED_PER_ROW;
}

namespace {
__global__ __launch_bounds__(256) void import_saved16_kernel(const float* __restrict__ gates, const float* __restrict__ cs,
                                                             float* __restrict__ saved, int T, int B, int R) {
    const long idx = (long)blockIdx.x * 256 + threadIdx.x;
    const long BH = (long)B * PH;
    if (idx >= (long)T * BH) return;
    const int u = (int)(idx % PH), b = (int)((idx / PH) % B), t = (int)(idx / BH);
    const int group = b / R, row = b % R, member = u >> 5, uw = u & 31;
    const long rec = (long)R * SAVED_PER_ROW;
    float* dst = saved + ((long)(group * PMEMBERS + member) * T + t) * rec;
    const f32x4 g = *reinterpret_cast<const f32x4*>(gates + idx * 4);
    *reinterpret_cast<f32x4*>(dst + (row * 32 + uw) * 4) = g;
    dst[R * 128 + row * 32 + uw] = cs[idx + BH];
}
}

extern "C" int lv_lstm_persist16_import_saved(const float* gates, const float* cs, float* saved, int T, int B, int R, int H,
                                              void* stream) {
    if (!gates || !cs || !saved) return LV_ERR_ARG;
    if (T < 0 || B <= 0) return LV_ERR_SHAPE;
    if (H != PH || !check_R(B, R)) return LV_ERR_UNSUPPORTED;
    if (((((uintptr_t)gates) | ((uintptr_t)saved)) & 15) != 0) return LV_ERR_ALIGN;
    if (T == 0) return LV_OK;
    LV_LAUNCH(import_saved16_kernel, dim3((unsigned)lv_cdiv((long)T * B * PH, 256)), dim3(256), 0, stream, gates, cs, saved, T, B, R);
    LV_CHECK_LAUNCH();
    return LV_OK;
}

extern "C" int lv_lstm_persist16_pack(const float* whh, float* wpk, int backward, int H, void* stream) {
    if (!whh || !wpk) return LV_ERR_ARG;
    if (H != PH) return LV_ERR_UNSUPPORTED;
    if ((((uintptr_t)wpk) & 15) != 0) return LV_ERR_ALIGN;
    const dim3 grid((unsigned)lv_cdiv(128L * 64 * 64, 256)), block(256);
    if (backward == 1) LV_LAUNCH(pack_w_rs16_kernel, grid, block, 0, stream, whh, reinterpret_cast<uint4*>(wpk));
    else LV_LAUNCH(pack_w_k16_kernel, grid, block, 0, stream, whh, reinterpret_cast<uint4*>(wpk), backward == 2 ? 1 : 0);
    LV_CHECK_LAUNCH();
    return LV_OK;
}

extern "C" int lv_lstm_persist16_pack2(const float* whh, float* wpk_fwd, float* wpk_bwd, int H, void* stream) {
    if (!whh || !wpk_fwd || !wpk_bwd) return LV_ERR_ARG;
    if (H != PH) return LV_ERR_UNSUPPORTED;
    if (((((uintptr_t)wpk_fwd) | ((uintptr_t)wpk_bwd)) & 15) != 0) return LV_ERR_ALIGN;
    LV_LAUNCH(pack_w_both16_kernel, dim3((unsigned)lv_cdiv(2 * 128L * 64 * 64, 256)), dim3(256), 0, stream, whh,
              reinterpret_cast<uint4*>(wpk_fwd), reinterpret_cast<uint4*>(wpk_bwd), 0);
    LV_CHECK_LAUNCH();
    return LV_OK;
}
extern "C" int lv_lstm_persist16_pack2_h16(const float* whh, float* wpk_fwd, float* wpk_bwd, int H, void* stream) {
    if (!whh || !wpk_fwd || !wpk_bwd) return LV_ERR_ARG;
    if (H != PH) return LV_ERR_UNSUPPORTED;
    if (((((uintptr_t)wpk_fwd) | ((uintptr_t)wpk_bwd)) & 15) != 0) return LV_ERR_ALIGN;
    LV_LAUNCH(pack_w_both16_kernel, dim3((unsigned)lv_cdiv(2 * 128L * 64 * 64, 256)), dim3(256), 0, stream, whh,
              reinterpret_cast<uint4*>(wpk_fwd), reinterpret_cast<uint4*>(wpk_bwd), 1);
    LV_CHECK_LAUNCH();
    return LV_OK;
}

extern "C" int lv_lstm_fwd_bf16_persist16(const float* gx, const float* wpk, float* hs, float* cs, float* saved, float* xch,
                                          int* status, int T, int B, int R, int flags, int H, void* stream) {
    if (!gx || !wpk || !hs || !cs || !saved || !xch || !status) return LV_ERR_ARG;
    if (T < 0 || B <= 0 || H <= 0) return LV_ERR_SHAPE;
    if (H != PH || !check_R(B, R)) return LV_ERR_UNSUPPORTED;
    if ((((uintptr_t)wpk) & 15) != 0 || (((uintptr_t)saved) & 15) != 0 || (((uintptr_t)gx) & 15) != 0 || (((uintptr_t)xch) & 15) != 0)
        return LV_ERR_ALIGN;
    if (lv_device_cus() < PGROUPS * PMEMBERS) return LV_ERR_UNSUPPORTED;
    if (T == 0) return LV_OK;
    char* const xb = reinterpret_cast<char*>(xch);
    const int dbl = (flags >> 1) & 1, half = dbl ? (flags >> 2) & 1 : 0;
    gran_t* hx = reinterpret_cast<gran_t*>(xb + XCH_FWD_OFF[half]);
    if (!dbl) (void)hipMemsetAsync(hx, 0, (size_t)XCH_FWD16_BYTES, (hipStream_t)stream);
    Fwd16P p{gx, reinterpret_cast<const uint4*>(wpk), hs, cs, saved, hx, status, T, B, R,
             dbl ? reinterpret_cast<uint4*>(xb + XCH_FWD_OFF[1 - half]) : nullptr, XCH_FWD16_BYTES / 16};
    const dim3 grid(PGROUPS * PMEMBERS), block(256);
    if (flags & 32) {
        if (flags & 1) {
            if (R <= 4) LV_LAUNCH_RESIDENT((lstm_fwd_persist_k16_kernel<4, true, true>), grid, block, 0, stream, p);
            else if (R <= 8) LV_LAUNCH_RESIDENT((lstm_fwd_persist_k16_kernel<8, true, true>), grid, block, 0, stream, p);
            else LV_LAUNCH_RESIDENT((lstm_fwd_persist_k16_kernel<16, true, true>), grid, block, 0, stream, p);
        } else {
            if (R <= 4) LV_LAUNCH_RESIDENT((lstm_fwd_persist_k16_kernel<4, false, true>), grid, block, 0, stream, p);
            else if (R <= 8) LV_LAUNCH_RESIDENT((lstm_fwd_persist_k16_kernel<8, false, true>), grid, block, 0, stream, p);
            else LV_LAUNCH_RESIDENT((lstm_fwd_persist_k16_kernel<16, false, true>), grid, block, 0, stream, p);
        }
        LV_CHECK_LAUNCH();
        return LV_OK;
    }
    if (flags & 1) {
        if (R <= 4) LV_LAUNCH_RESIDENT((lstm_fwd_persist_k16_kernel<4, true>), grid, block, 0, stream, p);
        else if (R <= 8) LV_LAUNCH_RESIDENT((lstm_fwd_persist_k16_kernel<8, true>), grid, block, 0, stream, p);
        else LV_LAUNCH_RESIDENT((lstm_fwd_persist_k16_kernel<16, true>), grid, block, 0, stream, p);
    } else {
        if (R <= 4) LV_LAUNCH_RESIDENT((lstm_fwd_persist_k16_kernel<4, false>), grid, block, 0, stream, p);
        else if (R <= 8) LV_LAUNCH_RESIDENT((lstm_fwd_persist_k16_kernel<8, false>), grid, block, 0, stream, p);
        else LV_LAUNCH_RESIDENT((lstm_fwd_persist_k16_kernel<16, false>), grid, block, 0, stream, p);
    }
    LV_CHECK_LAUNCH();
    return LV_OK;
}

extern "C" int lv_lstm_bwd_bf16_persist16(const float* dh_ext, const float* dh_last, const float* wpk, const float* saved,
                                          const float* hs, const float* cs, uint16_t* dG16, float* dGsum, float* xch, int* status,
                                          float* dh0, float* dc0, int tanh_init, int T, int B, int R, int flags, int H, void* stream) {
    if (!wpk || !saved || !cs || !dG16 || !dGsum || !xch || !status) return LV_ERR_ARG;
    if (T <= 0 || B <= 0 || H <= 0) return LV_ERR_SHAPE;
    if (tanh_init && !hs) return LV_ERR_ARG;
    if (H != PH || !check_R(B, R)) return LV_ERR_UNSUPPORTED;
    if ((((uintptr_t)wpk) & 15) != 0 || (((uintptr_t)saved) & 15) != 0 || (((uintptr_t)xch) & 15) != 0 || (((uintptr_t)dG16) & 15) != 0)
        return LV_ERR_ALIGN;
    if (lv_device_cus() < PGROUPS * PMEMBERS) return LV_ERR_UNSUPPORTED;
    char* const xb = reinterpret_cast<char*>(xch);
    const int dbl = (flags >> 1) & 1, half = dbl ? (flags >> 2) & 1 : 0;
    gran_t* gxch = reinterpret_cast<gran_t*>(xb + XCH_BWD_OFF[half]);
    const int RPi = R <= 4 ? 4 : (R <= 8 ? 8 : 16);
    const long extent = XCH_RS16_BYTES / RS16_SLOTS_MAX * 16 * RPi;
    const int ccls = (flags >> 3) & 3;
    const long cextent = XCH_RS16_BYTES / RS16_SLOTS_MAX * 16 * (ccls == 0 ? RPi : (4 << (ccls - 1)));
    if (!dbl) (void)hipMemsetAsync(gxch, 0, (size_t)extent, (hipStream_t)stream);
    Bwd16P p{dh_ext, dh_last, reinterpret_cast<const uint4*>(wpk), saved, cs, hs, dG16, dGsum, dh0, dc0, tanh_init, gxch, status, T, B, R,
             dbl ? reinterpret_cast<uint4*>(xb + XCH_BWD_OFF[1 - half]) : nullptr, cextent / 16};
    const dim3 grid(PGROUPS * PMEMBERS), block(256);
    const bool local = (flags & 1) != 0, ext = dh_ext != nullptr;
#define LV_BWD16_LAUNCH(RP_) do { \
        if (local && ext) LV_LAUNCH_RESIDENT((lstm_bwd_persist_rs16_kernel<RP_, true, true>), grid, block, 0, stream, p); \
        else if (local) LV_LAUNCH_RESIDENT((lstm_bwd_persist_rs16_kernel<RP_, true, false>), grid, block, 0, stream, p); \
        else if (ext) LV_LAUNCH_RESIDENT((lstm_bwd_persist_rs16_kernel<RP_, false, true>), grid, block, 0, stream, p); \
        else LV_LAUNCH_RESIDENT((lstm_bwd_persist_rs16_kernel<RP_, false, false>), grid, block, 0, stream, p); \
    } while (0)
    if (R <= 4) LV_BWD16_LAUNCH(4);
    else if (R <= 8) LV_BWD16_LAUNCH(8);
    else LV_BWD16_LAUNCH(16);
#undef LV_BWD16_LAUNCH
    LV_CHECK_LAUNCH();
    return LV_OK;
}
```

### vae_lagging_encoder_amd/engine.py

```python
import ctypes
import os

import torch

from . import _lib

def backend_for(device):
    device = torch.device(device)
    if device.type == "cuda":
        return _lib.load()
    raise _lib.LvaeError(
        "vae_lagging_encoder_amd runs on MI355X (ROCm 'cuda' tensors) through its HIP extension; got a %s tensor. "
        "There is no CPU fallback." % device.type)


def stream_ptr(device):
    device = torch.device(device)
    if device.type == "cuda":
        return ctypes.c_void_p(torch.cuda.current_stream(device).cuda_stream)
    return None


def P(t, offset_elems=0):
    if t is None:
# ... 201 lines not shown
    def __exit__(self, *a):
        if self.on:
            self.e1.record()
            PROFILE.setdefault(self.name, []).append((self.e0, self.e1, self.work, self.launches))


_GEMM_WS = {}
_PERSISTENT_DEFAULT = True


def _gemm_ws(lib, s):
    dev = torch.device("cuda", torch.cuda.current_device()) if s is not None else torch.device("cpu")
    ws = _GEMM_WS.get(dev)
    if ws is None:
        ws = torch.empty(1 << 26 if dev.type == "cuda" else 1 << 20, dtype=torch.float32, device=dev)
        _GEMM_WS[dev] = ws
    return ws


def _gemm(lib, s, tA, tB, M, N, K, A, lda, B, ldb, C, ldc, alpha=1.0, acc=0, add1=None, ld1=0, mod1=1,
          add2=None, ld2=0, mod2=1, prec="f32", ws=None):
    if ws is None:
        ws = _gemm_ws(lib, s)
    fn = lib.lv_gemm_bf16 if prec == "bf16" else lib.lv_gemm_f32
    with _prof("gemm_" + prec, 2.0 * M * N * K):
        fn(tA, tB, M, N, K, alpha, A, lda, B, ldb, C, ldc, acc, add1, ld1, mod1, add2, ld2, mod2, P(ws), ws.numel(), s)


def _gemm16(lib, s, tA, M, N, K, A16, lda, B16, ldb, C, ldc, add1=None, ld1=0, mod1=1, add2=None, ld2=0, mod2=1, ws=None, acc=0):
    if ws is None:
        ws = _gemm_ws(lib, s)
    with _prof("gemm_bf16", 2.0 * M * N * K):
        lib.lv_gemm_b16(tA, M, N, K, 1.0, A16, lda, B16, ldb, C, ldc, acc, add1, ld1, mod1, add2, ld2, mod2,
                        P(ws), ws.numel(), s)


class _AuxStream(object):

    def __init__(self):
        self.stream = None
        self.done = None

    def run(self, device, fn, keep=()):
        device = torch.device(device)
        if device.type != "cuda" or torch.cuda.is_current_stream_capturing():
            fn(None)
            return
        if self.stream is None:
            self.stream = torch.cuda.Stream(device)
        ev = torch.cuda.Event()
        ev.record(torch.cuda.current_stream(device))
        self.stream.wait_event(ev)
        for t in keep:
            t.record_stream(self.stream)
        with torch.cuda.stream(self.stream):
            fn(self.stream.cuda_stream)
            self.done = torch.cuda.Event()
            self.done.record(self.stream)

    def join(self, device):
        if self.done is not None:
            torch.cuda.current_stream(torch.device(device)).wait_event(self.done)
            self.done = None


class _TokenSortCache(object):
    LIMIT = 8192

    def __init__(self):
        import collections
        self.map = collections.OrderedDict()

    def _entries(self, key_tensor, create):
        i = id(key_tensor)
        ent = self.map.get(i)
        if ent is not None and ent[0]() is key_tensor:
            self.map.move_to_end(i)
            return ent[1]
        if not create:
            return None
        import weakref
        while len(self.map) >= self.LIMIT:
            self.map.popitem(last=False)
        self.map[i] = (weakref.ref(key_tensor, lambda _r, i=i, m=self.map: m.pop(i, None)), {})
        return self.map[i][1]

    def get(self, key_tensor, tag):
        ent = self._entries(key_tensor, False)
        hit = ent.get(tag) if ent is not None else None
        return hit[1:] if hit is not None and hit[0] == key_tensor._version else None

    def put(self, key_tensor, tag, srows, stok):
        self._entries(key_tensor, True)[tag] = (key_tensor._version, srows, stok)

    def invalidate(self, key_tensor=None):
        if key_tensor is None:
            self.map.clear()
        else:
            self.map.pop(id(key_tensor), None)


def reset_persistent_status(eng):
    if eng.status is not None:
        eng.status.zero_()


PERSIST_RUNGS = ("persistent, XCD-local hand-off", "persistent, write-through hand-off", "launch-per-timestep kernels")


def persist_rung(eng):
    if not eng.persistent:
        return 2
    return 0 if (eng.persist_flags & 1) else 1


def demote_persistent(eng):
    r = persist_rung(eng)
    if r == 0:
        eng.persist_flags &= ~1
    elif r == 1:
        eng.persistent = False
    else:
        raise _lib.LvaeError("a persistent-launch timeout was reported although the engine runs the launch-per-timestep kernels")
    reset_persistent_status(eng)
    eng.ladder_gen = getattr(eng, "ladder_gen", 0) + 1
    return r + 1


def status_ptr(eng):
    return P(eng.status) if eng.status is not None else None


_PERSIST_H = 1024
_PERSIST_MAX_B = 128


def _persist_rows(eng, B):
    rows = getattr(eng, "persist_rows", None)
    if rows is not None and 8 * rows >= B and 1 <= rows <= 16:
        return int(rows)
    return (B + 7) // 8


def _saved_floats(eng, T, B, H):
    n = T * B * 4 * H
    if H == _PERSIST_H and eng.precision == "bf16" and eng.persistent and B <= _PERSIST_MAX_B:
        n = max(n, eng.lib.lv_lstm_persist16_saved_floats(T, _persist_rows(eng, B)))
    return n


def _persistent_ok(eng, img, B, H, device, max_b):
    return (eng.precision == "bf16" and img is not None and eng.persistent and H == _PERSIST_H and B <= max_b
            and torch.device(device).type == "cuda" and torch.cuda.get_device_properties(device).multi_processor_count >= 256)


def weights_version(eng):
    return (sum(p._version for p in eng.flat.params), eng.wgen)


def _weight_images(eng, lib, s, device, want_persist, lstm=True, pred=False):
    wi = eng._wimg
    V, ni, H = eng.dims()[:3]
    v = eng.flat.views
    c = eng.wsc
    if wi is None:
        wi = eng._wimg = _NS()
        wi.ver = object()
        wi.W = wi.WT = wi.pred = wi.predT = wi.fwd16 = wi.bwd16 = wi.xch = None
        if lstm:
            wi.W = c.i16(4 * H, ni)
            wi.WT = c.i16(ni, 4 * H)
        wi.ldv = _round_up(V, 32)
        if pred:
            wi.pred = c.i16(V, H)
            wi.predT = c.i16(H, wi.ldv)
        wi.packed16 = False
    ver = weights_version(eng) if eng.cache_weight_images else object()
    h16 = bool(getattr(eng, "_h16_now", False))
    stale = wi.ver != ver or getattr(wi, "h16", False) != h16
    if stale:
        wih = v["lstm.weight_ih_l0"]
        if wi.W is not None and h16:
            lib.lv_cvt_h16_f32(P(wih), wih.shape[1], 4 * H, ni, H, None, 0, 1, 0, P(wi.W), ni, P(wi.WT), 4 * H, s)
        elif wi.W is not None:
            lib.lv_cvt_bf16_gates_f32(P(wih), wih.shape[1], H, ni, P(wi.W), ni, P(wi.WT), 4 * H, s)
        wi.h16 = h16
        if wi.pred is not None:
            lib.lv_cvt_bf16_f32(P(v["pred_linear.weight"]), H, V, H, P(wi.pred), H, P(wi.predT), wi.ldv, s)
        wi.ver = ver
        wi.packed16 = False
    if want_persist and not wi.packed16:
        if wi.fwd16 is None:
            n = lib.lv_lstm_persist16_wpk_floats()
            wi.fwd16, wi.bwd16 = c.f32(n), c.f32(n)
            wi.xch = torch.zeros(lib.lv_lstm_persist16_xch_floats(), dtype=torch.float32, device=c.device)
            wi.xstate = {"f": 0, "g": 0, "gcls": [0, 0]}
        (lib.lv_lstm_persist16_pack2_h16 if h16 else lib.lv_lstm_persist16_pack2)(P(v["lstm.weight_hh_l0"]), P(wi.fwd16), P(wi.bwd16), H, s)
        wi.packed16 = True
    return wi


def _xch_flags(wi, kind, rows, device, T=1):
    st = wi.xstate
    if T <= 0:
        return 0
    if torch.device(device).type == "cuda" and torch.cuda.is_current_stream_capturing():
        st["captured"] = True
    if st.get("captured"):
        return 0
    half = st[kind]
    st[kind] = 1 - half
    fl = 2 | (half << 2)
    if kind == "g":
        cls = 1 if rows <= 4 else (2 if rows <= 8 else 3)
        fl |= st["gcls"][1 - half] << 3
        st["gcls"][half] = cls
        st["gcls"][1 - half] = 0
    return fl


class SeqLengths(object):

    def __init__(self, lengths, B, T, device):
        if torch.is_tensor(lengths):
            if lengths.dtype not in (torch.int64, torch.int32, torch.int16, torch.int8, torch.uint8) or lengths.dim() != 1:
                raise ValueError("sentence lengths: a 1-D integer tensor or a list of ints expected, got %s %s"
                                 % (lengths.dtype, tuple(lengths.shape)))
            host = [int(v) for v in lengths.detach().cpu().tolist()]
        else:
            try:
                host = list(lengths)
            except TypeError:
                raise ValueError("sentence lengths: a 1-D integer tensor or a list of ints expected, got %r" % (type(lengths),))
            if not all(isinstance(v, int) and not isinstance(v, bool) for v in host):
                raise ValueError("sentence lengths: a list of ints expected")
        if len(host) != B:
            raise ValueError("sentence lengths: %d values for a batch of %d sentences" % (len(host), B))
        if B > 0 and min(host) < 2:
            raise ValueError("sentence lengths: every sentence holds at least <s> and </s>; got a length of %d" % min(host))
        if B > 0 and max(host) > T:
            raise ValueError("sentence lengths: a length of %d in a batch tensor of %d columns" % (max(host), T))
        self.host, self.B, self.T = host, B, T
        self.device = torch.device(device)
        self.max = max(host) if host else 0
        self.enc = torch.tensor(host, dtype=torch.int32).to(self.device)
        self._dec = {}

    def dec(self, ns=1):
        d = self._dec.get(ns)
        if d is None:
            d = self._dec[ns] = (self.enc - 1).repeat_interleave(ns).contiguous()
        return d

    @staticmethod
    def of(lengths, B, T, device):
        if isinstance(lengths, SeqLengths) and (lengths.B, lengths.T, lengths.device) == (B, T, torch.device(device)):
            return lengths
        return SeqLengths(lengths.host if isinstance(lengths, SeqLengths) else lengths, B, T, device)


def varlen_batch(x):
    xt, lengths = x
    if not (torch.is_tensor(xt) and xt.dim() == 2 and xt.dtype == torch.int64):
        raise ValueError("a variable-length batch is a pair (int64 tensor [batch][seq_len], lengths)")
    B, T = xt.shape
    L = SeqLengths.of(lengths, B, T, xt.device)
    if B > 0 and L.max < T:
        xt = xt[:, :L.max].contiguous()
        L = SeqLengths.of(L, B, L.max, xt.device)
    return xt, L


def length_groups(L):
    by = {}
    for b, n in enumerate(L.host):
        by.setdefault(n, []).append(b)
    return [(n, torch.tensor(by[n], dtype=torch.int64).to(L.device)) for n in sorted(by, reverse=True)]


class GroupedBackward(object):
    FIELDS = ("last", "last_ns", "last_steps", "_sort")

    def __init__(self, eng):
        self.eng = eng
        self.saved = []

    def after_forward(self, w):
        self.saved.append(({k: getattr(self.eng, k, None) for k in self.FIELDS}, w))

    def backward(self, i, current_ws, run):
        eng = self.eng
        rec, w = self.saved[i]
        for k, val in rec.items():
            setattr(eng, k, val)
        if current_ws() is not w:
            raise _lib.LvaeError("the by-length route's activations were dropped from the workspace cache between forward and backward "
                                 "(raise engine.WORKSPACE_BUDGET_FRACTION)")
        out = run(rec["last"][-1])
        if hasattr(eng, "join"):
            eng.join()
        f = eng.flat
        lib, s = eng.lib, stream_ptr(f.device)
        if i == 0:
            self.total = f.grad.clone()
        else:
            lib.lv_add_f32(P(self.total), P(f.grad), P(self.total), f.grad.numel(), s)
        if i == len(self.saved) - 1 and i > 0:
            f.grad.copy_(self.total)
        return out


def _refuse_bf16_lengths(eng):
    if eng.precision == "bf16":
        raise _lib.LvaeError("variable-length batches (x, lengths) run the exact-f32 configuration only: the bf16 and the persistent "
                             "recurrences have no length-aware form; call set_precision('f32') or batch by length")


def _same_device(what, dev, **operands):
    for name, t in operands.items():
        if t is not None and t.device != dev:
            raise _lib.LvaeError("%s: %s is on %s, x on %s" % (what, name, t.device, dev))


def _lstm_forward(eng, lib, s, img, w, Gx, whh, mask, scale, hdrop, T, B, H, device, steps=None):
    args = (Gx, whh, P(w.hs), P(w.cs), P(w.gates), mask, scale, hdrop)
    w.saved_layout = ("canonical", T, B, 0)
    if steps is not None:
        _refuse_bf16_lengths(eng)
        lib.lv_lstm_fwd_len_f32(*args, P(w.lstm_ws), P(steps[0]), steps[1], T, B, H, s)
    elif eng.precision != "bf16":
        lib.lv_lstm_fwd_f32(*args, P(w.lstm_ws), T, B, H, s)
    elif img is None:
        lib.lv_lstm_fwd_bf16(*args, P(w.lstm_ws), T, B, H, s)
    elif _persistent_ok(eng, img, B, H, device, _PERSIST_MAX_B):
        wi = eng._wimg
        rows = _persist_rows(eng, B)
        if mask is not None or hdrop is not None:
            raise _lib.LvaeError("the persistent forward has no in-kernel dropout (the engine applies it on the images)")
        need = lib.lv_lstm_persist16_saved_floats(T, rows)
        if w.gates.numel() < need:
            w.gates = torch.empty(need, dtype=torch.float32, device=w.gates.device)
        lib.lv_lstm_fwd_bf16_persist16(Gx, P(wi.fwd16), P(w.hs), P(w.cs), P(w.gates), P(wi.xch), P(eng.status), T, B, rows,
                                       eng.persist_flags | _xch_flags(wi, "f", rows, device, T) | (32 if getattr(wi, "h16", False) else 0), H, s)
        w.saved_layout = ("persist16", T, B, rows)
    else:
        lib.lv_lstm_fwd_bf16_ug(*args, P(w.lstm_ws), T, B, H, s)


_PERSIST_BWD_MAX_B = 128


def check_persistent_status(eng):
    st = eng.status
    if st is not None and int(st.item()) != 0:
        raise _lib.LvaeError("persistent LSTM kernel reported hand-off timeout (status %d) on ladder rung %d (%s): not all 256 "
                             "workgroups were resident (e.g. another kernel held compute units for seconds), or -- with "
                             "eng.persist_flags bit 0 set -- a group's workgroups were not placed on one XCD.  The fused trainers "
                             "recover from this by themselves (engine.demote_persistent); on the drop-in autograd path call it and "
                             "redo the step" % (int(st.item()), persist_rung(eng), PERSIST_RUNGS[persist_rung(eng)]))


def _need_canonical_saved(w):
    lay = getattr(w, "saved_layout", None)
    if lay is not None and lay[0] != "canonical":
        raise _lib.LvaeError("the saved activations are in the 16-row persistent kernels' own order %r, but the backward was routed to a "
                             "kernel that reads gates [T][B][4H] / cs: eng.persistent / eng.persist_rows changed between forward and "
                             "backward" % (lay,))


def _lstm_backward(eng, lib, s, img, w, dh_ext, dh_last, mask, scale, whh, dh0, dc0, tanh_init, T, B, H, device, steps=None):
    if steps is not None:
        _refuse_bf16_lengths(eng)
        lib.lv_lstm_bwd_len_f32(dh_ext, dh_last, mask, scale, whh, P(w.gates), P(w.hs), P(w.cs), P(w.dG), P(w.dGsum), P(w.lstm_ws),
                                dh0, dc0, tanh_init, P(steps[0]), steps[1], T, B, H, s)
        return
    if eng.precision != "bf16":
        lib.lv_lstm_bwd_f32(dh_ext, dh_last, mask, scale, whh, P(w.gates), P(w.hs), P(w.cs), P(w.dG), P(w.dGsum), P(w.lstm_ws),
                            dh0, dc0, tanh_init, T, B, H, s)
        return
    dG = P(w.dG) if img is None else None
    dG16 = P(img.dG) if img is not None else None
    if _persistent_ok(eng, img, B, H, device, _PERSIST_BWD_MAX_B):
        wi = eng._wimg
        rows = _persist_rows(eng, B)
        if mask is not None:
            raise _lib.LvaeError("the persistent BPTT has no in-kernel dropout mask (the engine applies it on dO)")
        if getattr(w, "saved_layout", None) != ("persist16", T, B, rows):
            raise _lib.LvaeError("the saved activations were not written by a persistent forward with the same T, B and rows per "
                                 "group (%r): eng.persist_rows / eng.persistent changed between forward and backward" % (getattr(w, "saved_layout", None),))
        lib.lv_lstm_bwd_bf16_persist16(dh_ext, dh_last, P(wi.bwd16), P(w.gates), P(w.hs), P(w.cs), dG16, P(w.dGsum), P(wi.xch),
                                       P(eng.status), dh0, dc0, tanh_init, T, B, rows, eng.persist_flags | _xch_flags(wi, "g", rows, device, T), H, s)
    else:
        _need_canonical_saved(w)
        lib.lv_lstm_bwd_bf16_img(dh_ext, dh_last, mask, scale, whh, P(w.gates), P(w.hs), P(w.cs), dG, dG16, P(w.dGsum),
                                 P(w.lstm_ws), dh0, dc0, tanh_init, T, B, H, s)


DUAL_WGRAD = os.environ.get("LVAE_DUAL_WGRAD", "1") != "0"
PAIR_WGRAD = os.environ.get("LVAE_PAIR_WGRAD", "1") != "0"
HS3_CVT = os.environ.get("LVAE_HS3_CVT", "1") != "0"


class _LstmImages(object):

    def __init__(self, c, TB, ni, H, key=None):
        self.TB, self.ni, self.H = TB, ni, H
        self.key = key
        self.ldr = _round_up(TB, 8)
        self.X = c.i16(TB, ni)
        self.XhT = c.i16(ni + H, self.ldr)
        self.addend = None
        self.dG = c.i16(TB, 4 * H)
        self.hT_gen = None
        self.hT_ld = self.ldr

    @property
    def XT(self):
        return self.XhT[:self.ni]

    @property
    def hT(self):
        return self.XhT[self.ni:]

    @staticmethod
    def usable(precision, native16, ni, H):
        return precision == "bf16" and native16 and ni % 8 == 0 and H % 8 == 0

    def forward(self, lib, s, X, W16, Gx, add_a, add_b, rows, wsc, addend_um=None, gather=None, h16=False):
        TB, ni, H = self.TB, self.ni, self.H
        if addend_um is not None:
            addend = addend_um
        else:
            if self.addend is None or self.addend.shape[0] != rows:
                self.addend = wsc.f32(rows, 4 * H)
                if self.key is not None:
                    wsc.grew(self.key, rows * 4 * H * 4)
            lib.lv_gate_interleave_f32(add_a, add_b, rows, H, P(self.addend), s)
            addend = P(self.addend)
        if h16:
            emb, ids, ids_stride, keep, kscale, T, B, V = gather
            assert keep is None
            lib.lv_cvt_h16_f32(emb, ni, TB, ni, 0, ids, ids_stride, B, V, P(self.X), ni, P(self.XT), self.ldr, s)
            ws = _gemm_ws(lib, s)
            with _prof("gemm_bf16", 2.0 * TB * 4 * H * ni):
                lib.lv_gemm_h16(TB, 4 * H, ni, 1.0, P(self.X), ni, W16, ni, Gx, 4 * H, 0, addend, 4 * H if rows > 1 else 0, rows, None, 0, 1,
                                P(ws), ws.numel(), s)
            return
        if gather is not None:
            emb, ids, ids_stride, keep, kscale, T, B, V = gather
            lib.lv_embed_gather_b16(emb, ids, ids_stride, keep, kscale, T, B, ni, V, P(self.X), ni, P(self.XT), self.ldr, s)
        else:
            lib.lv_cvt_bf16_f32(X, ni, TB, ni, P(self.X), ni, P(self.XT), self.ldr, s)
        _gemm16(lib, s, 0, TB, 4 * H, ni, P(self.X), ni, W16, ni, Gx, 4 * H,
                add1=addend, ld1=4 * H if rows > 1 else 0, mod1=rows)

    def backward(self, lib, s, dG, h_prev, WT16, dX, gW_ih, ld_gw, gW_hh, ws=None, between=None, hT_current=False):
        TB, ni, H = self.TB, self.ni, self.H
        if dG is not None:
            lib.lv_cvt_bf16_f32(dG, 4 * H, TB, 4 * H, P(self.dG), 4 * H, None, 0, s)
        wsd = ws if ws is not None else _gemm_ws(lib, s)
        if PAIR_WGRAD and DUAL_WGRAD and lib.lv_gemm_b16_pair_supported(1, 4 * H, ni + H, TB, 0, TB, ni, 4 * H, wsd.numel()):
            if not hT_current:
                lib.lv_cvt_bf16_f32(h_prev, H, TB, H, None, 0, P(self.hT), self.ldr, s)
            with _prof("gemm_bf16", 2.0 * 4 * H * (ni + H) * TB + 2.0 * TB * ni * 4 * H):
                lib.lv_gemm_b16_pair(1, 4 * H, ni + H, TB, P(self.dG), 4 * H, P(self.XhT), self.ldr, gW_ih, ld_gw, ni, gW_hh, H,
                                     0, TB, ni, 4 * H, P(self.dG), 4 * H, WT16, 4 * H, dX, ni, P(wsd), wsd.numel(), s)
            if between is not None:
                between()
            return
        _gemm16(lib, s, 0, TB, ni, 4 * H, P(self.dG), 4 * H, WT16, 4 * H, dX, ni, ws=ws)
        if between is not None:
            between()
        if not hT_current:
            lib.lv_cvt_bf16_f32(h_prev, H, TB, H, None, 0, P(self.hT), self.ldr, s)
        if DUAL_WGRAD and ni % 4 == 0 and lib.lv_gemm_b16_dual_supported(4 * H, ni + H, TB, wsd.numel()):
            with _prof("gemm_bf16", 2.0 * 4 * H * (ni + H) * TB):
                lib.lv_gemm_b16_dual(1, 4 * H, ni + H, TB, P(self.dG), 4 * H, P(self.XhT), self.ldr, gW_ih, ld_gw, ni, gW_hh, H,
                                     P(wsd), wsd.numel(), s)
            return
        _gemm16(lib, s, 1, 4 * H, ni, TB, P(self.dG), 4 * H, P(self.XT), self.ldr, gW_ih, ld_gw, ws=ws)
        _gemm16(lib, s, 1, 4 * H, H, TB, P(self.dG), 4 * H, P(self.hT), self.ldr, gW_hh, H, ws=ws)


class _LstmImagesMS(object):

    def __init__(self, c, Td, B, ns, ni, H):
        self.Td, self.B, self.ns, self.ni, self.H = Td, B, ns, ni, H
        self.TB, self.TBd = Td * B, Td * B * ns
        self.ldr, self.ldrd = _round_up(self.TB, 8), _round_up(self.TBd, 8)
        self.X = c.i16(self.TB, ni)
        self.XT = c.i16(ni, self.ldr)
        self.hT = c.i16(H, self.ldrd)
        self.dG = c.i16(self.TBd, 4 * H)
        self.dGs = c.i16(self.TB, 4 * H)
        self.hT_gen = None
        self.hT_ld = self.ldrd

    def forward(self, lib, s, W16, Gxw, gather):
        emb, ids, ids_stride, keep, kscale, T, B, V = gather
        lib.lv_embed_gather_b16(emb, ids, ids_stride, keep, kscale, T, B, self.ni, V, P(self.X), self.ni, P(self.XT), self.ldr, s)
        _gemm16(lib, s, 0, self.TB, 4 * self.H, self.ni, P(self.X), self.ni, W16, self.ni, Gxw, 4 * self.H)

    def backward(self, lib, s, dG, h_prev, WT16, dX, gW_ih, ld_gw, gW_hh, ws=None, hT_current=False):
        assert dG is None
        ni, H = self.ni, self.H
        lib.lv_sample_sum_b16(P(self.dG), 4 * H, P(self.dGs), 4 * H, self.Td, self.B, self.ns, 4 * H, s)
        wsd = ws if ws is not None else _gemm_ws(lib, s)
        if PAIR_WGRAD and lib.lv_gemm_b16_pair_supported(1, 4 * H, ni, self.TB, 0, self.TB, ni, 4 * H, wsd.numel()):
            with _prof("gemm_bf16", 4.0 * 4 * H * ni * self.TB):
                lib.lv_gemm_b16_pair(1, 4 * H, ni, self.TB, P(self.dGs), 4 * H, P(self.XT), self.ldr, gW_ih, ld_gw, 0, None, 0,
                                     0, self.TB, ni, 4 * H, P(self.dGs), 4 * H, WT16, 4 * H, dX, ni, P(wsd), wsd.numel(), s)
        else:
            _gemm16(lib, s, 0, self.TB, ni, 4 * H, P(self.dGs), 4 * H, WT16, 4 * H, dX, ni, ws=ws)
            _gemm16(lib, s, 1, 4 * H, ni, self.TB, P(self.dGs), 4 * H, P(self.XT), self.ldr, gW_ih, ld_gw, ws=ws)
        if not hT_current:
            lib.lv_cvt_bf16_f32(h_prev, H, self.TBd, H, None, 0, P(self.hT), self.ldrd, s)
        _gemm16(lib, s, 1, 4 * H, H, self.TBd, P(self.dG), 4 * H, P(self.hT), self.ldrd, gW_hh, H, ws=ws)


def _wgrad(lib, s, M, N, K, A, lda, Bm, ldb, C, ldc, prec, ws=None):
    _gemm(lib, s, 1, 0, M, N, K, A, lda, Bm, ldb, C, ldc, prec=prec, ws=ws)


def _sorted_tokens(eng, lib, s, x, x_key, ids_stride, T_used, B, V, w):
    key = x_key if x_key is not None else x
    capturing = x.device.type == "cuda" and torch.cuda.is_current_stream_capturing()
    use_cache = eng.ws_evictable and not capturing
    if use_cache:
        hit = eng._sorts.get(key, (T_used, B))
        if hit is not None:
            return hit
        srows, stok = eng.wsc.i32(T_used * B), eng.wsc.i32(T_used * B)
    else:
        srows, stok = w.srows, w.stok
    eng._aux.run(x.device, lambda sa: lib.lv_token_sort(P(x), ids_stride, T_used, B, V, P(srows), P(stok), P(w.stmp), sa if sa is not None else s),
                 keep=(x, srows, stok))
    if use_cache:
        eng._sorts.put(key, (T_used, B), srows, stok)
    return srows, stok


class LSTMEncoderEngine(object):

    def __init__(self, module):
        self.m = module
        self.flat = None
        self.wsc = None
        self.ws_evictable = True
        self.gen = 0
        self.precision = "f32"
        self.native16 = True
        self.persistent = _PERSISTENT_DEFAULT
        self.persist_rows = None
        self.persist_flags = 1
        self.status = None
        self.fold = None
        self.embed_rows = None
        self.cache_weight_images = False
        self.wgen = 0
        self.exact_forward = ()
        self.exact_impl = "auto"
        self.fwd_operands = "f16"
        self._h16_now = False
        self._wimg = None
        self._aux = _AuxStream()
        self._sorts = _TokenSortCache()

    def _quiesce_side_streams(self):
        dev = self.flat.device if self.flat is not None else None
        if dev is not None and dev.type == "cuda" and self._aux.stream is not None:
            torch.cuda.current_stream(dev).wait_stream(self._aux.stream)

    def _b16(self, B, T):
        V, ni, H, nz2 = self.dims()
        if not _LstmImages.usable(self.precision, self.native16, ni, H):
            return None
        return self.wsc.get(("b16", B, T), lambda: _LstmImages(self.wsc, T * B, ni, H, key=("b16", B, T)))

    def _exact(self, img):
        ex = tuple(self.exact_forward or ())
        assert all(e in ("gx", "rec") for e in ex), ex
        return ex if (img is not None and self.precision == "bf16") else ()

    def fold_parts(self, B, T):
        return {"embed": self.lib.lv_embed_scatter_sumsq_parts(T, B)}

    def refresh_weight_images(self, B, device):
        V, ni, H, nz2 = self.dims()
        if not _LstmImages.usable(self.precision, self.native16, ni, H):
            return None
        self.ensure(device)
        persist = self.persistent and H == _PERSIST_H and B <= _PERSIST_MAX_B and torch.device(device).type == "cuda" and \
            torch.cuda.get_device_properties(device).multi_processor_count >= 256
        return _weight_images(self, self.lib, stream_ptr(device), device, persist)

    def ensure(self, device):
        device = torch.device(device)
        if self.flat is None or self.flat.device != device or not self.flat.bound():
            named = [("embed.weight", self.m.embed.weight), ("lstm.weight_ih_l0", self.m.lstm.weight_ih_l0),
                     ("lstm.weight_hh_l0", self.m.lstm.weight_hh_l0), ("lstm.bias_ih_l0", self.m.lstm.bias_ih_l0),
                     ("lstm.bias_hh_l0", self.m.lstm.bias_hh_l0), ("linear.weight", self.m.linear.weight)]
            self.flat = FlatBuffer(named, device)
            self.flat.flat_grads = getattr(self, "_flat_grads_pref", True)
            self.wsc = _WS(device)
            self.wsc.evictable = self.ws_evictable
            self.wsc.before_evict = self._quiesce_side_streams
            self._wimg = None
            for p in self.flat.params:
                p._lvae_engine = self
        self.lib = backend_for(device)
        if self.status is None or self.status.device != device:
            self.status = torch.zeros(1, dtype=torch.int32, device=device)
        return self.flat

    def dims(self):
        V, ni = self.m.embed.weight.shape
        H = self.m.lstm.weight_hh_l0.shape[1]
        nz2 = self.m.linear.weight.shape[0]
        return V, ni, H, nz2

    def _ws(self, B, T):
        V, ni, H, nz2 = self.dims()
        c = self.wsc

        def build():
            w = _NS()
            w.X = c.f32(T * B, ni)
            w.Gx = c.f32(T * B, 4 * H)
            w.hs = torch.zeros(T + 1, B, H, dtype=torch.float32, device=c.device)
            w.cs = torch.zeros(T + 1, B, H, dtype=torch.float32, device=c.device)
            w.gates = c.f32(_saved_floats(self, T, B, H))
            w.mulv = c.f32(B, nz2)
            w.dmulv = c.f32(B, nz2)
            w.dG = c.f32(T * B, 4 * H)
            w.dGsum = c.f32(B, 4 * H)
            w.lstm_ws = c.f32(self.lib.lv_lstm_ws_floats(B, H))
            w.dhT = c.f32(B, H)
            w.dX = c.f32(T * B, ni)
            w.srows = c.i32(T * B)
            w.stok = c.i32(T * B)
            w.stmp = c.i32(2 * T * B)
            return w
        return c.get((B, T), build)

    def forward(self, x, head=None, x_key=None, lengths=None):
        assert x.dtype == torch.int64 and x.dim() == 2
        x = x.contiguous()
        B, T = x.shape
        steps = None
        if lengths is not None:
            _refuse_bf16_lengths(self)
            if head is not None:
                raise _lib.LvaeError("the fused head takes equal-length batches only")
            lengths = SeqLengths.of(lengths, B, T, x.device)
            steps = (lengths.enc, lengths.max)
        f = self.ensure(x.device)
        lib, s = self.lib, stream_ptr(x.device)
        V, ni, H, nz2 = self.dims()
        w = self._ws(B, T)
        v = f.views
        img = self._b16(B, T)
        exact = self._exact(img)
        self._h16_now = img is not None and not exact and self.fwd_operands == "f16"
        split = (self.exact_impl == "auto" and set(exact) == {"gx", "rec"} and _persistent_ok(self, img, B, H, x.device, _PERSIST_MAX_B))
        if img is None or ("gx" in exact and not split):
            lib.lv_embed_gather_f32(P(v["embed.weight"]), P(x), T, None, 1.0, P(w.X), T, B, ni, V, s)
        self._sort = _sorted_tokens(self, lib, s, x, x_key, T, T, B, V, w)
        biases = dict(add1=P(v["lstm.bias_ih_l0"]), ld1=0, mod1=1, add2=P(v["lstm.bias_hh_l0"]), ld2=0, mod2=1)
        gx_unit_major = True
        if split:
            self._exact_forward_split(lib, s, img, w, x, T, B, V, ni, H)
        elif img is not None and "gx" in exact:
            self.refresh_weight_images(B, x.device)
            lib.lv_embed_gather_b16(P(v["embed.weight"]), P(x), T, None, 1.0, T, B, ni, V, P(img.X), ni, P(img.XT), img.ldr, s)
            _gemm(lib, s, 0, 1, T * B, 4 * H, ni, P(w.X), ni, P(v["lstm.weight_ih_l0"]), ni, P(w.Gx), 4 * H, prec="f32", **biases)
            gx_unit_major = False
            if "rec" not in exact:
                if getattr(w, "Gx_gm", None) is None:
                    w.Gx_gm = self.wsc.f32(T * B, 4 * H)
                w.Gx, w.Gx_gm = w.Gx_gm, w.Gx
                lib.lv_gate_interleave_f32(P(w.Gx_gm), None, T * B, H, P(w.Gx), s)
                gx_unit_major = True
        elif img is not None:
            wi = self.refresh_weight_images(B, x.device)
            img.forward(lib, s, None, P(wi.W), P(w.Gx), P(v["lstm.bias_ih_l0"]), P(v["lstm.bias_hh_l0"]), 1, self.wsc,
                        gather=(P(v["embed.weight"]), P(x), T, None, 1.0, T, B, V), h16=self._h16_now)
        else:
            _gemm(lib, s, 0, 1, T * B, 4 * H, ni, P(w.X), ni, P(v["lstm.weight_ih_l0"]), ni, P(w.Gx), 4 * H,
                  prec=self.precision, **biases)
        gx_round = getattr(self, "gx_round", None)
        if gx_round is not None and not split:
            w.Gx.copy_(w.Gx.to(torch.float16 if gx_round == "f16" else torch.bfloat16).to(torch.float32))
        if split:
            pass
        elif "rec" in exact:
            self._exact_recurrence(lib, s, img, w, gx_unit_major, T, B, H, x.device)
        else:
            with _prof("lstm_fwd_enc", float(T), 1 if _persistent_ok(self, img, B, H, x.device, _PERSIST_MAX_B) else T):
                _lstm_forward(self, lib, s, img, w, P(w.Gx), P(v["lstm.weight_hh_l0"]), None, 1.0, None, T, B, H, x.device, steps=steps)
        if head is not None and not fused_ends_ok(B, nz2 // 2, head[0].shape[1]):
            eps, z, kl = head
            _gemm(lib, s, 0, 1, B, nz2, H, P(w.hs, T * B * H), H, P(v["linear.weight"]), H, P(w.mulv), nz2)
            lib.lv_reparam_kl_fwd_f32(P(w.mulv), P(eps), P(z), P(kl), B, eps.shape[1], nz2 // 2, s)
        elif head is not None:
            eps, z, kl = head
            lib.lv_enc_head_fwd_f32(P(w.hs, T * B * H), P(v["linear.weight"]), P(eps), P(w.mulv), P(z), P(kl), B, H,
                                    eps.shape[1], nz2 // 2, s)
        else:
            _gemm(lib, s, 0, 1, B, nz2, H, P(w.hs, T * B * H), H, P(v["linear.weight"]), H, P(w.mulv), nz2)
        self.gen += 1
        self.last = (x, B, T, self.gen)
        self.last_steps = steps
        return w.mulv

    def _exact_forward_split(self, lib, s, img, w, x, T, B, V, ni, H):
        v = self.flat.views
        TB = T * B
        wi = self.refresh_weight_images(B, x.device)
        c = self.wsc
        if getattr(wi, "Ww", None) is None:
            wi.Ww = c.i16(4 * H, 3 * ni)
            wi.Whh_lo = c.i16(4 * H, H)
        wih, whh = v["lstm.weight_ih_l0"], v["lstm.weight_hh_l0"]
        lib.lv_cvt_bf16_gates_f32(P(wih), wih.shape[1], H, ni, P(wi.Ww), 3 * ni, None, 0, s)
        lib.lv_cvt_bf16_gates_f32(P(wih), wih.shape[1], H, ni, P(wi.Ww, ni), 3 * ni, None, 0, s)
        lib.lv_cvt_bf16_lo_f32(P(wih), wih.shape[1], 4 * H, ni, H, None, 0, 1, 0, P(wi.Ww, 2 * ni), 3 * ni, None, 0, s)
        lib.lv_cvt_bf16_lo_f32(P(whh), H, 4 * H, H, H, None, 0, 1, 0, P(wi.Whh_lo), H, None, 0, s)
        if getattr(img, "Xw", None) is None:
            img.Xw = c.i16(TB, 3 * ni)
            img.h16 = c.i16(TB, H)
            if img.key is not None:
                c.grew(img.key, TB * (3 * ni + H) * 2)
        emb = P(v["embed.weight"])
        lib.lv_embed_gather_b16(emb, P(x), T, None, 1.0, T, B, ni, V, P(img.Xw), 3 * ni, P(img.XT), img.ldr, s)
        lib.lv_cvt_bf16_lo_f32(emb, ni, TB, ni, 0, P(x), T, B, V, P(img.Xw, ni), 3 * ni, None, 0, s)
        lib.lv_embed_gather_b16(emb, P(x), T, None, 1.0, T, B, ni, V, P(img.Xw, 2 * ni), 3 * ni, None, 0, s)
        if img.addend is None or img.addend.shape[0] != 1:
            img.addend = c.f32(1, 4 * H)
        lib.lv_gate_interleave_f32(P(v["lstm.bias_ih_l0"]), P(v["lstm.bias_hh_l0"]), 1, H, P(img.addend), s)
        _gemm16(lib, s, 0, TB, 4 * H, 3 * ni, P(img.Xw), 3 * ni, P(wi.Ww), 3 * ni, P(w.Gx), 4 * H, add1=P(img.addend), ld1=0, mod1=1)
        with _prof("lstm_fwd_enc", float(T), 1):
            _lstm_forward(self, lib, s, img, w, P(w.Gx), P(whh), None, 1.0, None, T, B, H, x.device)
        lib.lv_cvt_bf16_f32(P(w.hs), H, TB, H, P(img.h16), H, None, 0, s)
        _gemm16(lib, s, 0, TB, 4 * H, H, P(img.h16), H, P(wi.Whh_lo), H, P(w.Gx), 4 * H, acc=1)
        with _prof("lstm_fwd_enc", float(T), 1):
            _lstm_forward(self, lib, s, img, w, P(w.Gx), P(whh), None, 1.0, None, T, B, H, x.device)

    def _exact_recurrence(self, lib, s, img, w, gx_unit_major, T, B, H, device):
        v = self.flat.views
        n = T * B * 4 * H
        if getattr(w, "gates_canon", None) is None or w.gates_canon.numel() < n:
            w.gates_canon = self.wsc.f32(n)
        fwd = lib.lv_lstm_fwd_f32_ug if gx_unit_major else lib.lv_lstm_fwd_f32
        persist_bwd = _persistent_ok(self, img, B, H, device, _PERSIST_BWD_MAX_B)
        gates = w.gates_canon if persist_bwd else w.gates
        with _prof("lstm_fwd_enc", float(T), T):
            fwd(P(w.Gx), P(v["lstm.weight_hh_l0"]), P(w.hs), P(w.cs), P(gates), None, 1.0, None, P(w.lstm_ws), T, B, H, s)
        w.saved_layout = ("canonical", T, B, 0)
        if persist_bwd:
            rows = _persist_rows(self, B)
            need = lib.lv_lstm_persist16_saved_floats(T, rows)
            if w.gates.numel() < need:
                w.gates = torch.empty(need, dtype=torch.float32, device=w.gates.device)
            lib.lv_lstm_persist16_import_saved(P(w.gates_canon), P(w.cs), P(w.gates), T, B, rows, H, s)
            w.saved_layout = ("persist16", T, B, rows)

    def backward(self, dmulv, gen=None, head=None, after_bptt=None, after_embed=None):
        x, B, T, g = self.last
        if gen is not None and gen != g:
            raise _lib.LvaeError("encoder activations were overwritten by a later forward(); the HIP engine keeps "
                                 "one in-flight step per module")
        self.embed_rows = None
        f = self.flat
        lib, s = self.lib, stream_ptr(x.device)
        V, ni, H, nz2 = self.dims()
        w = self._ws(B, T)
        v, gv = f.views, f.gviews
        if head is not None and not fused_ends_ok(B, nz2 // 2, head[0].shape[1]):
            eps, dz, parts, dkl = head
            assert parts == 1
            lib.lv_reparam_kl_bwd_f32(P(w.mulv), P(eps), P(dz), P(dkl), P(w.dmulv), B, eps.shape[1], nz2 // 2, s)
            _gemm(lib, s, 0, 0, B, H, nz2, P(w.dmulv), nz2, P(v["linear.weight"]), H, P(w.dhT), H)
            _gemm(lib, s, 1, 0, nz2, H, B, P(w.dmulv), nz2, P(w.hs, T * B * H), H, P(gv["linear.weight"]), H)
        elif head is not None:
            eps, dz, parts, dkl = head
            lib.lv_enc_head_bwd_f32(P(w.mulv), P(eps), P(dz), parts, P(dkl), P(w.hs, T * B * H), P(v["linear.weight"]), P(w.dmulv),
                                    P(w.dhT), P(gv["linear.weight"]), B, H, eps.shape[1], nz2 // 2, s)
        else:
            dmulv = dmulv.contiguous()
            _gemm(lib, s, 0, 0, B, H, nz2, P(dmulv), nz2, P(v["linear.weight"]), H, P(w.dhT), H)
            _gemm(lib, s, 1, 0, nz2, H, B, P(dmulv), nz2, P(w.hs, T * B * H), H, P(gv["linear.weight"]), H)
        img = self._b16(B, T)
        with _prof("lstm_bwd_enc", float(T), 1 if _persistent_ok(self, img, B, H, x.device, _PERSIST_BWD_MAX_B) else 2 * T):
            _lstm_backward(self, lib, s, img, w, None, P(w.dhT), None, 1.0, P(v["lstm.weight_hh_l0"]), None, None, 0, T, B, H, x.device,
                           steps=getattr(self, "last_steps", None))
        if after_bptt is not None:
            after_bptt()
        def embed_grad():
            self._aux.join(x.device)
            self.embed_rows = (self._sort[1], T * B)
            if self.fold and "embed" in self.fold:
                sq, only = self.fold["embed"]
                if only:
                    self.embed_rows = None
                lib.lv_embed_scatter_full_sumsq_f32(P(w.dX), None, 1.0, P(self._sort[0]), P(self._sort[1]), T, B, P(gv["embed.weight"]), ni,
                                                    V, -1, P(sq), int(only), s)
            else:
                lib.lv_embed_scatter_full_f32(P(w.dX), None, 1.0, P(self._sort[0]), P(self._sort[1]), T, B, P(gv["embed.weight"]), ni, V, -1, s)
            if after_embed is not None:
                after_embed()
        if img is not None:
            img.backward(lib, s, None, P(w.hs), P(self._wimg.WT), P(w.dX), P(gv["lstm.weight_ih_l0"]), ni, P(gv["lstm.weight_hh_l0"]),
                         between=embed_grad)
        else:
            _gemm(lib, s, 0, 0, T * B, ni, 4 * H, P(w.dG), 4 * H, P(v["lstm.weight_ih_l0"]), ni, P(w.dX), ni, prec=self.precision)
            embed_grad()
            _wgrad(lib, s, 4 * H, ni, T * B, P(w.dG), 4 * H, P(w.X), ni, P(gv["lstm.weight_ih_l0"]), ni, self.precision)
            _wgrad(lib, s, 4 * H, H, T * B, P(w.dG), 4 * H, P(w.hs), H, P(gv["lstm.weight_hh_l0"]), H, self.precision)
        lib.lv_colsum_f32(P(w.dGsum), 4 * H, B, 4 * H, P(gv["lstm.bias_ih_l0"]), P(gv["lstm.bias_hh_l0"]), s)


class LSTMDecoderEngine(object):

    def __init__(self, module):
        self.m = module
        self.flat = None
        self.wsc = None
        self.ws_evictable = True
        self.gen = 0
        self.precision = "f32"
        self.overlap = None
        self.native16 = True
        self.persistent = _PERSISTENT_DEFAULT
        self.persist_rows = None
        self.persist_flags = 1
        self.status = None
        self.fold = None
        self.cache_weight_images = True
        self.fused_nll = True
        self.wgen = 0
        self._wimg = None
        self._side = None
        self._side_ws = None
        self._pending = None
        self._aux = _AuxStream()
        self._sorts = _TokenSortCache()

    def _quiesce_side_streams(self):
        dev = self.flat.device if self.flat is not None else None
        if dev is not None and dev.type == "cuda":
            for st in (self._aux.stream, self._side):
                if st is not None:
                    torch.cuda.current_stream(dev).wait_stream(st)

    def _fork(self, device):
        import contextlib
        if not (torch.device(device).type == "cuda" and self._overlap_on()):
            return contextlib.nullcontext(), None
        if self._side is None:
            self._side = torch.cuda.Stream(device)
            self._side_ws = torch.empty(1 << 26, dtype=torch.float32, device=device)
        ev = torch.cuda.Event()
        ev.record(torch.cuda.current_stream(device))
        self._side.wait_event(ev)
        return torch.cuda.stream(self._side), self._side_ws

    def _overlap_on(self):
        if self.overlap is not None:
            return bool(self.overlap)
        return self.precision == "f32"

    def _mark_pending(self, device):
        if self._side is not None and torch.device(device).type == "cuda" and self._overlap_on():
            ev = torch.cuda.Event()
            ev.record(self._side)
            self._pending = ev

    def join(self):
        if self._pending is not None:
            torch.cuda.current_stream().wait_event(self._pending)
            self._pending = None

    def ensure(self, device):
        device = torch.device(device)
        if self.flat is None or self.flat.device != device or not self.flat.bound():
            m = self.m
            named = [("embed.weight", m.embed.weight), ("trans_linear.weight", m.trans_linear.weight),
                     ("lstm.weight_ih_l0", m.lstm.weight_ih_l0), ("lstm.weight_hh_l0", m.lstm.weight_hh_l0),
                     ("lstm.bias_ih_l0", m.lstm.bias_ih_l0), ("lstm.bias_hh_l0", m.lstm.bias_hh_l0),
                     ("pred_linear.weight", m.pred_linear.weight)]
            self.flat = FlatBuffer(named, device)
            self.flat.flat_grads = getattr(self, "_flat_grads_pref", True)
            self.wsc = _WS(device)
            self.wsc.evictable = self.ws_evictable
            self.wsc.before_evict = self._quiesce_side_streams
            self._wimg = None
            for p in self.flat.params:
                p._lvae_engine = self
        self.lib = backend_for(device)
        if self.status is None or self.status.device != device:
            self.status = torch.zeros(1, dtype=torch.int32, device=device)
        return self.flat

    def dims(self):
        V, ni = self.m.embed.weight.shape
        H = self.m.lstm.weight_hh_l0.shape[1]
        nz = self.m.trans_linear.weight.shape[1]
        return V, ni, H, nz

    def _ws(self, Bd, Td, ns=1):
        V, ni, H, nz = self.dims()
        c = self.wsc
        ldl = _round_up(V, 32)
        Bs = Bd // ns
        key = (Bd, Td) if ns == 1 else (Bs, ns, Td)

        def build():
            w = _DecWS()
            w.ldl = ldl
            w._alloc = lambda: c.f32(Td * Bd, ldl)
            w._grew = lambda nb: c.grew(key, nb)
            w.X = c.f32(Td * Bs, ni)
            if ns > 1:
                w.Gxw = c.f32(Td * Bs, 4 * H)
                w.dGs = c.f32(Td * Bs, 4 * H)
                w.x_rep = torch.empty(Bd, Td + 1, dtype=torch.int64, device=c.device)
                w.Zp_um = c.f32(Bd, 4 * H)
            w.Zp = c.f32(Bd, 4 * H)
            w.Gx = c.f32(Td * Bd, 4 * H)
            w.hs = c.f32(Td + 1, Bd, H)
            w.cs = c.f32(Td + 1, Bd, H)
            w.gates = c.f32(_saved_floats(self, Td, Bd, H))
            w.O = c.f32(Td * Bd, H)
            w._logits = None
            w.lse = c.f32(Td * Bd)
            w.nll = c.f32(Td * Bd)
            w.rec = c.f32(Bd)
            w.dO = c.f32(Td * Bd, H)
            w.dG = c.f32(Td * Bd, 4 * H)
            w.dGsum = c.f32(Bd, 4 * H)
            w.lstm_ws = c.f32(self.lib.lv_lstm_ws_floats(Bd, H))
            w.dc0 = c.f32(Bd, H)
            w.dX = c.f32(Td * Bs, ni)
            w.dz = c.f32(Bd, nz)
            w.dz_parts = self.lib.lv_dec_tail_parts(H)
            w.dzp = c.f32(w.dz_parts, Bd, nz)
            w.srows = c.i32(Td * Bs)
            w.stok = c.i32(Td * Bs)
            w.stmp = c.i32(2 * Td * Bs)
            w.zero1 = torch.zeros(1, dtype=torch.float32, device=c.device)
            w.klz = torch.zeros(Bd, dtype=torch.float32, device=c.device)
            w.loss = c.f32(Bd)
            return w
        return c.get(key, build)

    def fold_parts(self, B, Td, ns=1):
        out = {"embed": self.lib.lv_embed_scatter_sumsq_parts(Td, B)}
        V, ni, H, nz = self.dims()
        if self._b16(B * ns, Td, ns) is not None:
            dev = self.flat.device
            on_side = torch.device(dev).type == "cuda" and self._overlap_on()
            ws_n = (1 << 26) if on_side else _gemm_ws(self.lib, stream_ptr(dev)).numel()
            n = self.lib.lv_gemm_b16_sumsq_parts(V, H, Td * B * ns, ws_n)
            if n > 0:
                out["pred"] = n
        return out

    def _b16(self, Bd, Td, ns=1):
        V, ni, H, nz = self.dims()
        if self.precision != "bf16" or not self.native16 or H % 8 != 0:
            return None
        c = self.wsc

        def build():
            b = _NS()
            b.ldr = _round_up(Td * Bd, 8)
            b.ldv = _round_up(V, 32)
            b.O = c.i16(Td * Bd, H)
            b.OT = c.i16(H, b.ldr)
            b.dl = c.i16(Td * Bd, b.ldv)
            b.l16 = c.i16(Td * Bd, b.ldv)
            b.nparts = self.lib.lv_gemm_b16_nll_parts(V)
            b.part = c.f32(Td * Bd, 2 * b.nparts)
            b.tgt = c.f32(Td * Bd)
            return b
        return c.get(("b16", Bd, Td) if ns == 1 else ("b16", Bd // ns, ns, Td), build)

    def refresh_weight_images(self, B, device):
        V, ni, H, nz = self.dims()
        use_pred = self.precision == "bf16" and self.native16 and H % 8 == 0
        use_lstm = _LstmImages.usable(self.precision, self.native16, ni, H)
        if not (use_pred or use_lstm):
            return None
        self.ensure(device)
        persist = use_lstm and self.persistent and H == _PERSIST_H and B <= _PERSIST_MAX_B and \
            torch.device(device).type == "cuda" and torch.cuda.get_device_properties(device).multi_processor_count >= 256
        return _weight_images(self, self.lib, stream_ptr(device), device, persist, lstm=use_lstm, pred=use_pred)

    def _lstm_images(self, Bd, Td, ns=1):
        V, ni, H, nz = self.dims()
        if not _LstmImages.usable(self.precision, self.native16, ni, H):
            return None
        if ns > 1:
            return self.wsc.get(("b16lstm", Bd // ns, ns, Td), lambda: _LstmImagesMS(self.wsc, Td, Bd // ns, ns, ni, H))
        return self.wsc.get(("b16lstm", Bd, Td), lambda: _LstmImages(self.wsc, Td * Bd, ni, H, key=("b16lstm", Bd, Td)))

    def forward(self, x, z, mask_in, mask_out, p_in, p_out, want_rec=True, x_key=None, lengths=None):
        assert x.dtype == torch.int64 and x.dim() == 2
        x = x.contiguous()
        B, T = x.shape
        Td = T - 1
        if z.dim() != 3 or z.shape[0] != B or z.shape[1] < 1:
            raise _lib.LvaeError("the HIP decoder path takes z of shape [B, nsamples, nz]; got %s for a batch of %d" % (tuple(z.shape), B))
        ns = int(z.shape[1])
        Bd = B * ns
        steps = None
        if lengths is not None:
            _refuse_bf16_lengths(self)
            _same_device("the length-aware decoder", x.device, z=z, mask_in=mask_in, mask_out=mask_out)
            lengths = SeqLengths.of(lengths, B, T, x.device)
            steps = (lengths.dec(ns), lengths.max - 1)
        z2 = z.reshape(Bd, -1).contiguous()
        f = self.ensure(x.device)
        lib, s = self.lib, stream_ptr(x.device)
        V, ni, H, nz = self.dims()
        w = self._ws(Bd, Td, ns)
        v = f.views
        sc_in = 1.0 / (1.0 - p_in) if mask_in is not None else 1.0
        sc_out = 1.0 / (1.0 - p_out) if mask_out is not None else 1.0
        if mask_in is not None:
            assert mask_in.dtype == torch.uint8 and tuple(mask_in.shape) == (B, Td, ni) and mask_in.is_contiguous()
        if mask_out is not None:
            assert mask_out.dtype == torch.uint8 and tuple(mask_out.shape) == (Bd, Td, H) and mask_out.is_contiguous()
        gather = (P(v["embed.weight"]), P(x), T, P(mask_in), sc_in, Td, B, V)
        img = self._lstm_images(Bd, Td, ns)
        if img is None:
            lib.lv_embed_gather_f32(P(v["embed.weight"]), P(x), T, P(mask_in), sc_in, P(w.X), Td, B, ni, V, s)
        self._sort = _sorted_tokens(self, lib, s, x, x_key, T, Td, B, V, w)
        ids = x
        if ns > 1:
            lib.lv_repeat_rows_i64(P(x), P(w.x_rep), B, T, ns, s)
            ids = w.x_rep
        wih = v["lstm.weight_ih_l0"]
        fused = fused_ends_ok(Bd, nz)
        if fused:
            lib.lv_dec_init_f32(P(z2), P(v["trans_linear.weight"]), P(wih), ni + nz, ni, P(v["lstm.bias_ih_l0"]),
                                P(v["lstm.bias_hh_l0"]), P(w.cs), P(w.hs), P(w.Zp), 1 if img is not None else 0, Bd, H, nz, s)
        else:
            _gemm(lib, s, 0, 1, Bd, H, nz, P(z2), nz, P(v["trans_linear.weight"]), nz, P(w.cs), H)
            lib.lv_tanh_f32(P(w.cs), P(w.hs), Bd * H, s)
            _gemm(lib, s, 0, 1, Bd, 4 * H, nz, P(z2), nz, P(wih, ni), ni + nz, P(w.Zp), 4 * H,
                  add1=P(v["lstm.bias_ih_l0"]), ld1=0, mod1=1, add2=P(v["lstm.bias_hh_l0"]), ld2=0, mod2=1)
        if ns > 1:
            zp = w.Zp
            if img is not None and not fused:
                lib.lv_gate_interleave_f32(P(w.Zp), None, Bd, H, P(w.Zp_um), s)
                zp = w.Zp_um
            if img is not None:
                wi = self.refresh_weight_images(Bd, x.device)
                img.forward(lib, s, P(wi.W), P(w.Gxw), gather)
            else:
                _gemm(lib, s, 0, 1, Td * B, 4 * H, ni, P(w.X), ni, P(wih), ni + nz, P(w.Gxw), 4 * H, prec=self.precision)
            lib.lv_gx_expand_add_f32(P(w.Gxw), P(zp), P(w.Gx), Td, B, ns, 4 * H, s)
        elif img is not None:
            wi = self.refresh_weight_images(B, x.device)
            if fused:
                img.forward(lib, s, None, P(wi.W), P(w.Gx), None, None, B, self.wsc, addend_um=P(w.Zp), gather=gather)
            else:
                img.forward(lib, s, None, P(wi.W), P(w.Gx), P(w.Zp), None, B, self.wsc, gather=gather)
        else:
            _gemm(lib, s, 0, 1, Td * B, 4 * H, ni, P(w.X), ni, P(wih), ni + nz, P(w.Gx), 4 * H,
                  add1=P(w.Zp), ld1=4 * H, mod1=B, prec=self.precision)
        b16 = self._b16(Bd, Td, ns)
        late_mask = b16 is not None and _persistent_ok(self, img, Bd, H, x.device, _PERSIST_MAX_B)
        with _prof("lstm_fwd_dec", float(Td), 1 if _persistent_ok(self, img, Bd, H, x.device, _PERSIST_MAX_B) else Td):
            if late_mask:
                _lstm_forward(self, lib, s, img, w, P(w.Gx), P(v["lstm.weight_hh_l0"]), None, 1.0, None, Td, Bd, H, x.device)
            else:
                _lstm_forward(self, lib, s, img, w, P(w.Gx), P(v["lstm.weight_hh_l0"]), P(mask_out), sc_out, P(w.O), Td, Bd, H, x.device,
                              steps=steps)
        hs3 = HS3_CVT and late_mask and img is not None
        if hs3:
            lib.lv_cvt_bf16_hs3_f32(P(w.hs), H, Td, Bd, H, P(mask_out), sc_out, P(b16.O), H, P(b16.OT), b16.ldr, P(img.hT), img.hT_ld, s)
        if b16 is not None:
            if hs3:
                pass
            elif late_mask and mask_out is not None:
                lib.lv_cvt_bf16_keep_f32(P(w.hs, Bd * H), H, Td, Bd, H, P(mask_out), sc_out, P(b16.O), H, P(b16.OT), b16.ldr, s)
            elif late_mask:
                lib.lv_cvt_bf16_f32(P(w.hs, Bd * H), H, Td * Bd, H, P(b16.O), H, P(b16.OT), b16.ldr, s)
            else:
                lib.lv_cvt_bf16_f32(P(w.O), H, Td * Bd, H, P(b16.O), H, P(b16.OT), b16.ldr, s)
            wi = self.refresh_weight_images(Bd, x.device)
            if self.fused_nll:
                with _prof("gemm_bf16", 2.0 * Td * Bd * V * H):
                    lib.lv_gemm_b16_nll(Td * Bd, V, H, P(b16.O), H, P(wi.pred), H, P(b16.l16), b16.ldv, P(ids), T, 1, Bd,
                                        P(b16.part), P(b16.tgt), s)
                lib.lv_softmax_nll_merge_f32(P(b16.part), b16.nparts, P(b16.tgt), P(w.lse), P(w.nll), Td * Bd, s)
            else:
                _gemm16(lib, s, 0, Td * Bd, V, H, P(b16.O), H, P(wi.pred), H, P(w.logits), w.ldl)
        else:
            _gemm(lib, s, 0, 1, Td * Bd, V, H, P(w.O), H, P(v["pred_linear.weight"]), H, P(w.logits), w.ldl, prec=self.precision)
        if not (b16 is not None and self.fused_nll):
            lib.lv_softmax_nll_fwd_f32(P(w.logits), w.ldl, P(ids), T, 1, P(w.lse), P(w.nll), Td, Bd, V, s)
        if steps is not None:
            lib.lv_nll_mask_len_f32(P(w.nll), P(steps[0]), steps[1], Td, Bd, s)
        if want_rec:
            lib.lv_vae_loss_f32(P(w.nll), P(w.klz), P(w.zero1), P(w.loss), P(w.rec), Td, Bd, s)
        self.gen += 1
        if img is not None:
            img.hT_gen = self.gen if hs3 else None
        self.last = (x, z2, mask_in, mask_out, sc_in, sc_out, B, T, self.gen)
        self.last_ns = ns
        self.last_steps = steps
        return w.rec

    def cond_ll_supported(self, T):
        V, ni, H, nz = self.dims()
        return bool(self.lib.lv_dec_cond_ll_f32_supported(V, ni, H, nz, int(T)))

    def cond_ll(self, x, z):
        device = x.device
        if z.device != device:
            raise _lib.LvaeError("cond_ll: z is on %s, x on %s" % (z.device, device))
        self.ensure(device)
        V, ni, H, nz = self.dims()
        v = self.flat.views
        B, T = x.shape
        if x.dtype != torch.int64 or z.dim() not in (2, 3) or z.shape[-1] != nz or (z.dim() == 3 and z.shape[0] != B):
            raise ValueError("cond_ll: x int64 [B][T] and z [K][%d] or [B][K][%d] expected, got %s %s and %s"
                             % (nz, nz, x.dtype, tuple(x.shape), tuple(z.shape)))
        x = x.contiguous()
        z = z.contiguous().float()
        K = z.shape[-2]
        z_stride = 0 if z.dim() == 2 else K * nz
        ws = torch.empty(self.lib.lv_dec_cond_ll_f32_ws_floats(V, H, nz, B, T), dtype=torch.float32, device=device)
        out = torch.empty(B, K, dtype=torch.float32, device=device)
        self.lib.lv_dec_cond_ll_f32(P(x), B, T, P(z), z_stride, K, P(v["embed.weight"]), P(v["trans_linear.weight"]),
                                    P(v["lstm.weight_ih_l0"]), P(v["lstm.weight_hh_l0"]), P(v["lstm.bias_ih_l0"]),
                                    P(v["lstm.bias_hh_l0"]), P(v["pred_linear.weight"]), V, ni, H, nz, P(ws), P(out),
                                    stream_ptr(device))
        return out

    @staticmethod
    def mh_default_iters_per_launch(T):
        return max(1, 2048 // max(1, int(T) - 1))

    def mh_chain(self, x, z0, draw, burn_in, thin, nsamples, std, iters_per_launch=None):
        device = x.device
        if z0.device != device:
            raise _lib.LvaeError("mh_chain: z0 is on %s, x on %s" % (z0.device, device))
        self.ensure(device)
        V, ni, H, nz = self.dims()
        if x.dim() != 2 or x.dtype != torch.int64 or z0.dim() != 3 or z0.shape[0] != x.shape[0] or z0.shape[2] != nz:
            raise ValueError("mh_chain: x int64 [B][T] and z0 [B][C][%d] expected, got %s %s and %s"
                             % (nz, x.dtype, tuple(x.shape), tuple(z0.shape)))
        burn_in, thin, nsamples = int(burn_in), int(thin), int(nsamples)
        if burn_in < 0 or thin < 1 or nsamples < 1:
            raise ValueError("mh_chain: burn_in >= 0, thin >= 1, nsamples >= 1 expected")
        B, T = x.shape
        C = z0.shape[1]
        total = burn_in + nsamples * thin
        per = self.mh_default_iters_per_launch(T) if iters_per_launch is None else int(iters_per_launch)
        if per < 1:
            raise ValueError("mh_chain: iters_per_launch >= 1 expected")
        chunks = []
        for i0 in range(0, total, per):
            n = min(per, total - i0)
            eps, u = draw(i0, n)
            if eps.device != device or u.device != device:
                raise _lib.LvaeError("mh_chain: noise is on %s / %s, x on %s" % (eps.device, u.device, device))
            if tuple(eps.shape) != (n, B, C, nz) or tuple(u.shape) != (n, B, C):
                raise ValueError("mh_chain: eps [%d][%d][%d][%d] and u [%d][%d][%d] expected, got %s and %s"
                                 % (n, B, C, nz, n, B, C, tuple(eps.shape), tuple(u.shape)))
            chunks.append((i0, n, eps.contiguous().float(), u.contiguous().float()))
        x = x.contiguous()
        v = self.flat.views
        s = stream_ptr(device)
        f32 = dict(dtype=torch.float32, device=device)
        i32 = dict(dtype=torch.int32, device=device)
        ws = torch.empty(self.lib.lv_mh_chain_f32_ws_floats(V, H, nz, B, T), **f32)
        cur = z0.detach().float().contiguous().clone()
        cur_ll, accepts = torch.zeros(B, C, **f32), torch.zeros(B, C, **i32)
        samples = torch.empty(B, nsamples, C, nz, **f32)
        ratios, flags = torch.empty(total, B, C, **f32), torch.empty(total, B, C, **i32)
        self.lib.lv_mh_chain_prep_f32(P(x), B, T, P(v["embed.weight"]), P(v["trans_linear.weight"]), P(v["lstm.weight_ih_l0"]),
                                      P(v["lstm.weight_hh_l0"]), P(v["lstm.bias_ih_l0"]), P(v["lstm.bias_hh_l0"]),
                                      P(v["pred_linear.weight"]), V, ni, H, nz, P(ws), s)
        for i0, n, eps, u in chunks:
            self.lib.lv_mh_chain_f32(P(x), B, T, P(ws), V, H, nz, C, P(cur), P(cur_ll), P(accepts), P(eps), P(u), n, i0, burn_in,
                                     thin, nsamples, float(std), 1 if i0 == 0 else 0, P(samples), P(ratios, i0 * B * C),
                                     P(flags, i0 * B * C), s)
        return {"samples": samples, "cur": cur, "log_joint": cur_ll, "accepts": accepts, "ratios": ratios, "flags": flags,
                "iterations": total}

    def backward(self, drec, gen=None, partial_dz=False):
        x, z2, mask_in, mask_out, sc_in, sc_out, B, T, g = self.last
        if gen is not None and gen != g:
            raise _lib.LvaeError("decoder activations were overwritten by a later forward(); the HIP engine keeps "
                                 "one in-flight step per module")
        ns = self.last_ns
        Bd, Td = B * ns, T - 1
        f = self.flat
        lib, s = self.lib, stream_ptr(x.device)
        V, ni, H, nz = self.dims()
        w = self._ws(Bd, Td, ns)
        v, gv = f.views, f.gviews
        drec = drec.contiguous()
        if drec.numel() != Bd:
            raise _lib.LvaeError("backward takes drec per decoder row (%d values for %d samples per sentence), got %d" % (Bd, ns, drec.numel()))
        ids = x if ns == 1 else w.x_rep
        wih = v["lstm.weight_ih_l0"]
        gwih = gv["lstm.weight_ih_l0"]
        dev = x.device
        pad_idx = self.m.embed.padding_idx
        pad_idx = V - 1 if pad_idx is None else int(pad_idx)
        b16 = self._b16(Bd, Td, ns)
        if b16 is not None and self.fused_nll:
            lib.lv_softmax_nll_bwd_h16(P(b16.l16), b16.ldv, P(w.lse), P(ids), T, 1, P(drec), P(b16.dl), b16.ldv, Td, Bd, V, s)
        elif b16 is not None:
            lib.lv_softmax_nll_bwd_b16(P(w.logits), w.ldl, P(w.lse), P(ids), T, 1, P(drec), P(b16.dl), b16.ldv, Td, Bd, V, s)
        else:
            lib.lv_softmax_nll_bwd_f32(P(w.logits), w.ldl, P(w.lse), P(ids), T, 1, P(drec), Td, Bd, V, s)
        ctx, sws = self._fork(dev)
        with ctx:
            if b16 is not None and self.fold and "pred" in self.fold:
                sq, only = self.fold["pred"]
                gws = sws if sws is not None else _gemm_ws(lib, s)
                if lib.lv_gemm_b16_sumsq_parts(V, H, Td * Bd, gws.numel()) != sq.numel():
                    raise RuntimeError("norm folding: the plan's partial count does not match this launch's tile plan")
# ... 400 lines not shown
```

Before: 11610.

## Fuse LSTM input projection into persistent forward kernel instead of separate Gx GEMM

Adds a persistent LSTM forward variant that computes the input projection (X·Wih plus bias/addend) inside the recurrent kernel with MFMA. Input weights are held partly in LDS and partly in registers, and x tiles are prefetched a few timesteps ahead. This skips the separate Gx GEMM launch and the round trip of the large Gx buffer through memory, and Gx is now allocated lazily. It is enabled by default for the encoder and decoder when batch rows ≤4 and ni=512. The cost is extra LDS, register pressure and per-step MFMA work on the latency-critical recurrent path.

```diff
diff --git a/include/lvae.h b/include/lvae.h
--- a/include/lvae.h
+++ b/include/lvae.h
@@ -86,6 +86,9 @@
 int lv_lstm_persist16_pack2_h16(const float* whh, float* wpk_fwd, float* wpk_bwd, int H, void* stream);
 int lv_lstm_fwd_bf16_persist16(const float* gx, const float* wpk, float* hs, float* cs, float* saved, float* xch, int* status,
                                int T, int B, int R, int flags, int H, void* stream);
+int lv_lstm_fwd_bf16_persist16_x(const void* x16, long ldx, const void* wih16, int ni, const float* addend, long addend_row_stride,
+                                 const float* wpk, float* hs, float* cs, float* saved, float* xch, int* status,
+                                 int T, int B, int R, int flags, int H, void* stream);
 int lv_lstm_bwd_bf16_persist16(const float* dh_ext, const float* dh_last, const float* wpk, const float* saved, const float* hs,
                                const float* cs, uint16_t* dG16, float* dGsum, float* xch, int* status, float* dh0, float* dc0,
                                int tanh_init, int T, int B, int R, int flags, int H, void* stream);
diff --git a/profiles/microbench/lstm_fixed_cost_probe.py b/profiles/microbench/lstm_fixed_cost_probe.py
--- a/profiles/microbench/lstm_fixed_cost_probe.py
+++ b/profiles/microbench/lstm_fixed_cost_probe.py
@@ -24,6 +24,27 @@
     e1.record(); torch.cuda.synchronize()
     return e0.elapsed_time(e1) * 1e3 / n
 
+
+if "--fused-gx" in sys.argv:
+    NI = 512
+    W16 = ((torch.rand(4 * H, NI, device=dev) * 2 - 1) * 0.03).to(torch.bfloat16).view(torch.int16)
+    add = torch.randn(B, 4 * H, device=dev) * 0.1
+    FF = lambda: 1 | _xch_flags(wi, "f", R, "cpu")
+    res = {}
+    for T in (40, 200):
+        gx = torch.randn(T, B, 4 * H, device=dev) * 0.5
+        X16 = torch.randn(T * B, NI, device=dev).to(torch.bfloat16).view(torch.int16)
+        hs = torch.zeros(T + 1, B, H, device=dev); cs = torch.zeros(T + 1, B, H, device=dev)
+        saved = torch.empty(lib.lv_lstm_persist16_saved_floats(T, R), device=dev)
+        res[T] = (t(lambda: lib.lv_lstm_fwd_bf16_persist16(P(gx), P(wf), P(hs), P(cs), P(saved), P(xch), P(st), T, B, R, FF(), H, s)),
+                  t(lambda: lib.lv_lstm_fwd_bf16_persist16_x(P(X16), NI, P(W16), NI, P(add), 4 * H, P(wf), P(hs), P(cs), P(saved), P(xch),
+                                                             P(st), T, B, R, FF(), H, s)))
+        print("T=%3d: forward reading Gx %7.1f us, forming Gx itself %7.1f us (back-to-back launches)" % (T, res[T][0], res[T][1]))
+    for name, col in (("reading Gx", 0), ("forming Gx", 1)):
+        b = (res[200][col] - res[40][col]) / 160.0
+        print("%s: fixed %.1f us per launch + %.3f us per timestep" % (name, res[40][col] - 40 * b, b))
+    print("status", int(st.item()))
+    sys.exit(0)
 
 Ts = [1, 2, 4, 8, 16, 50, 100, 200]
 rows = []
diff --git a/vae_lagging_encoder_amd/_lib.py b/vae_lagging_encoder_amd/_lib.py
--- a/vae_lagging_encoder_amd/_lib.py
+++ b/vae_lagging_encoder_amd/_lib.py
@@ -77,6 +77,7 @@
     "lv_lstm_persist16_pack2": [_vp, _vp, _vp, _i, _vp],
     "lv_lstm_persist16_pack2_h16": [_vp, _vp, _vp, _i, _vp],
     "lv_lstm_fwd_bf16_persist16": [_vp, _vp, _vp, _vp, _vp, _vp, _vp, _i, _i, _i, _i, _i, _vp],
+    "lv_lstm_fwd_bf16_persist16_x": [_vp, _l, _vp, _i, _vp, _l, _vp, _vp, _vp, _vp, _vp, _vp, _i, _i, _i, _i, _i, _vp],
     "lv_lstm_bwd_bf16_persist16": [_vp, _vp, _vp, _vp, _vp, _vp, _vp, _vp, _vp, _vp, _vp, _vp, _i, _i, _i, _i, _i, _i, _vp],
     "lv_transpose_f32": [_vp, _vp, _i, _i, _vp],
     "lv_transpose_ld_f32": [_vp, _l, _vp, _l, _i, _i, _vp],
diff --git a/vae_lagging_encoder_amd/csrc/lv_device.h b/vae_lagging_encoder_amd/csrc/lv_device.h
--- a/vae_lagging_encoder_amd/csrc/lv_device.h
+++ b/vae_lagging_encoder_amd/csrc/lv_device.h
@@ -206,6 +206,10 @@
     return d;
 }
 static inline f32x4 lv_mfma_16x16x32_f16_areg_first(uint4 a, uint4 b) { return lv_mfma_16x16x32_f16_areg(a, b, f32x4{0.f, 0.f, 0.f, 0.f}); }
+template <bool F16> static inline f32x4 lv_mfma_16x16x32_vreg(uint4 a, uint4 b, f32x4 c) {
+    return F16 ? lv_mfma_16x16x32_f16_areg(a, b, c) : lv_emu_mfma_16x16x32_bf16(a, b, c);
+}
+template <bool F16> static inline f32x4 lv_mfma_16x16x32_vreg_first(uint4 a, uint4 b) { return lv_mfma_16x16x32_vreg<F16>(a, b, f32x4{0.f, 0.f, 0.f, 0.f}); }
 #else
 #include <hip/hip_runtime.h>
 typedef float f32x4 __attribute__((ext_vector_type(4)));
@@ -280,6 +284,19 @@
     const lv_u32x4v av = {a.x, a.y, a.z, a.w}, bv = {b.x, b.y, b.z, b.w};
     f32x4 c;
     asm volatile("v_mfma_f32_16x16x32_f16 %0, %1, %2, 0" : "=v"(c) : "a"(av), "v"(bv));
+    return c;
+}
+template <bool F16> __device__ __forceinline__ f32x4 lv_mfma_16x16x32_vreg(uint4 a, uint4 b, f32x4 c) {
+    const lv_u32x4v av = {a.x, a.y, a.z, a.w}, bv = {b.x, b.y, b.z, b.w};
+    if constexpr (F16) asm volatile("v_mfma_f32_16x16x32_f16 %0, %1, %2, %0" : "+v"(c) : "v"(av), "v"(bv));
+    else asm volatile("v_mfma_f32_16x16x32_bf16 %0, %1, %2, %0" : "+v"(c) : "v"(av), "v"(bv));
+    return c;
+}
+template <bool F16> __device__ __forceinline__ f32x4 lv_mfma_16x16x32_vreg_first(uint4 a, uint4 b) {
+    const lv_u32x4v av = {a.x, a.y, a.z, a.w}, bv = {b.x, b.y, b.z, b.w};
+    f32x4 c;
+    if constexpr (F16) asm volatile("v_mfma_f32_16x16x32_f16 %0, %1, %2, 0" : "=&v"(c) : "v"(av), "v"(bv));
+    else asm volatile("v_mfma_f32_16x16x32_bf16 %0, %1, %2, 0" : "=&v"(c) : "v"(av), "v"(bv));
     return c;
 }
 #define LV_MFMA_DRAIN() asm volatile("s_nop 15\n\ts_nop 3" ::: "memory")
diff --git a/vae_lagging_encoder_amd/csrc/lv_lstm_persist16.hip b/vae_lagging_encoder_amd/csrc/lv_lstm_persist16.hip
--- a/vae_lagging_encoder_amd/csrc/lv_lstm_persist16.hip
+++ b/vae_lagging_encoder_amd/csrc/lv_lstm_persist16.hip
@@ -95,6 +95,7 @@
     int* status;
     int T, B, R;
     uint4* clr; long clr_n;
+    const uint16_t* x16; long ldx; const uint16_t* wih; const float* add; long add_ld;
 };
 
 __device__ __forceinline__ void clear_other_half(uint4* q, long n) {
@@ -118,12 +119,29 @@
     int abort;
 };
 
-template <int RP, bool LOCAL, bool F16 = false>
+constexpr int XNI = 512;
+constexpr int XKS = XNI / 32;
+#ifndef LV_XIN_KS_LDS
+#define LV_XIN_KS_LDS 12
+#endif
+constexpr int XKL = LV_XIN_KS_LDS;
+constexpr int XS_PITCH = XNI / 8 + 2;
+struct __attribute__((aligned(16))) Fwd16XLds : Fwd16Lds<4> {
+    uint4 wih[4][XKL][2][64];
+    uint4 xs[16 * XS_PITCH];
+    f32x4 rb[2][16][RED_SLOTS];
+};
+template <bool C, class A, class B> struct lv_pick_t { typedef A type; };
+template <class A, class B> struct lv_pick_t<false, A, B> { typedef B type; };
+
+template <int RP, bool LOCAL, bool F16 = false, bool XIN = false>
 __global__ __launch_bounds__(256) void lstm_fwd_persist_k16_kernel(Fwd16P p) {
+    static_assert(!XIN || RP == 4, "the fused input projection maps the tile's 16 columns to 4 steps x 4 rows");
     auto h16 = [](float v) -> uint32_t { return F16 ? (uint32_t)lv_f32_to_f16_bits(v) : lv_f32_to_bf16_bits(v); };
     auto put = [](gran_t* q, gran_t v) { if (LOCAL) lv_xcd_store_u64(q, v); else gran_store(q, v); };
     constexpr int NP = Cfg16<RP>::NP, SBK = Cfg16<RP>::SBK, GJ = Cfg16<RP>::GJ;
-    LV_BLOCK_SHARED(Fwd16Lds<RP>, sm);
+    typedef typename lv_pick_t<XIN, Fwd16XLds, Fwd16Lds<RP>>::type Lds;
+    LV_BLOCK_SHARED(Lds, sm);
     int& s_abort = sm.abort;
     const int tid = (int)threadIdx.x, l = tid & 63, w = tid >> 6;
     const int group = (int)blockIdx.x % PGROUPS, member = (int)blockIdx.x / PGROUPS;
@@ -134,6 +152,19 @@
     clear_other_half(p.clr, p.clr_n);
     if (rows == 0) return;
     if (tid == 0) s_abort = 0;
+    const int kq = l >> 4;
+
+    uint4 xwr[XIN ? XKS - XKL : 1][2];
+    if constexpr (XIN) {
+        const uint16_t* wb = p.wih + (long)(128 * member + 32 * w + (l & 15)) * XNI + 8 * kq;
+#pragma unroll
+        for (int ks = 0; ks < XKS; ++ks)
+#pragma unroll
+            for (int j = 0; j < 2; ++j) {
+                const uint4 v = *reinterpret_cast<const uint4*>(wb + (long)(16 * j) * XNI + 32 * ks);
+                if (ks < XKL) sm.wih[w][ks][j][l] = v; else xwr[ks - XKL][j] = v;
+            }
+    }
 
     uint4 wreg[8][8];
     {
@@ -180,10 +211,17 @@
         if (own[q] && even) put(hx_g + (long)prow[q] * (PH / 2) + (punit >> 1), ((gran_t)1u << 32) | (gran_t)(mine | (next << 16)));
     }
 
-    float4 gxb[NP][SBK];
+    float4 gxb[XIN ? 1 : NP][XIN ? 1 : SBK];
+    f32x4 addv[NP];
+    if constexpr (XIN) {
+#pragma unroll
+        for (int q = 0; q < NP; ++q)
+            addv[q] = *reinterpret_cast<const f32x4*>(p.add + (long)(b0 + (own[q] ? prow[q] : 0)) * p.add_ld + 4 * punit);
+    }
     f32x4 recb[NP][SBK];
     float cb[NP][SBK], hb[NP][SBK];
     auto load_slots = [&](int tb, int lo, int hi) {
+        if constexpr (XIN) return;
 #pragma unroll
         for (int q = 0; q < NP; ++q)
 #pragma unroll
@@ -208,12 +246,65 @@
                 }
             }
     };
+    f32x4 xr[XIN ? 4 : 1];
+    auto x_load = [&](int t0) {
+        if constexpr (XIN) {
+            const int r = w < rows ? w : 0;
+#pragma unroll
+            for (int j = 0; j < 4; ++j) {
+                const int t = t0 + j < T ? t0 + j : T - 1;
+                xr[j] = *reinterpret_cast<const f32x4*>(p.x16 + ((long)t * B + b0 + r) * p.ldx + 8 * l);
+            }
+        }
+    };
+    auto x_stage = [&]() {
+        if constexpr (XIN) {
+#pragma unroll
+            for (int j = 0; j < 4; ++j) *reinterpret_cast<f32x4*>(&sm.xs[(4 * j + w) * XS_PITCH + l]) = xr[j];
+        }
+    };
+    auto x_product = [&](int par) {
+        if constexpr (XIN) {
+            f32x4 a0, a1;
+            const uint4* xb = sm.xs + (l & 15) * XS_PITCH + kq;
+            uint4 bf[XKS], w0[XKS], w1[XKS];
+            auto frag = [&](auto KS) {
+                constexpr int ks = decltype(KS)::value;
+                if constexpr (ks < XKS) {
+                    bf[ks] = xb[4 * ks];
+                    if constexpr (ks < XKL) { w0[ks] = sm.wih[w][ks][0][l]; w1[ks] = sm.wih[w][ks][1][l]; }
+                    else { w0[ks] = xwr[ks - XKL][0]; w1[ks] = xwr[ks - XKL][1]; }
+                }
+            };
+            auto step = [&](auto KS) {
+                constexpr int ks = decltype(KS)::value;
+                frag(lv_const<ks + 2>());
+                LV_SCHED_BARRIER();
+                a0 = ks == 0 ? lv_mfma_16x16x32_vreg_first<F16>(w0[ks], bf[ks]) : lv_mfma_16x16x32_vreg<F16>(w0[ks], bf[ks], a0);
+                a1 = ks == 0 ? lv_mfma_16x16x32_vreg_first<F16>(w1[ks], bf[ks]) : lv_mfma_16x16x32_vreg<F16>(w1[ks], bf[ks], a1);
+            };
+            static_assert(XKS == 16, "sixteen k-steps, written out");
+            frag(lv_const<0>()); frag(lv_const<1>());
+            step(lv_const<0>()); step(lv_const<1>()); step(lv_const<2>()); step(lv_const<3>());
+            step(lv_const<4>()); step(lv_const<5>()); step(lv_const<6>()); step(lv_const<7>());
+            step(lv_const<8>()); step(lv_const<9>()); step(lv_const<10>()); step(lv_const<11>());
+            step(lv_const<12>()); step(lv_const<13>()); step(lv_const<14>()); step(lv_const<15>());
+            LV_MFMA_DRAIN();
+            LV_MFMA_RESULT(a0);
+            LV_MFMA_RESULT(a1);
+            f32x4* rd = sm.rb[par][l & 15];
+            rd[8 * w + kq] = a0;
+            rd[8 * w + 4 + kq] = a1;
+        }
+    };
     load_slots(0, 0, SBK);
+    x_load(0);
+    x_stage();
     __syncthreads();
+    x_product(0);
 
     const int nq = rows * 128;
     const int brow = (l & 15) < rows ? (l & 15) : 0;
-    const int kq = l >> 4;
     uint32_t abl_keep[8] = {0u, 0u, 0u, 0u, 0u, 0u, 0u, 0u};
     for (int tb = 0; tb < T; tb += SBK) {
 #pragma unroll
@@ -292,6 +383,8 @@
             }
             if (s2 == 0 && tb > 0) { store_block(tb - SBK); load_slots(tb, SBK - 1, SBK); }
             if (s2 == SBK - 1) load_slots(tb + SBK, 0, SBK - 1);
+            if ((s2 & 3) == 0) x_load(t + 4);
+            if ((s2 & 3) == 2) x_stage();
             LV_TRACE_MARK(t, 1);
             LV_WAIT_LDS();
             LV_TRACE_MARK(t, 2);
@@ -340,7 +433,12 @@
                 if (own[q]) {
                     const f32x4 q0 = sm.red[t & 1][0][prow[q]][uw], q1 = sm.red[t & 1][1][prow[q]][uw];
                     const f32x4 q2 = sm.red[t & 1][2][prow[q]][uw], q3 = sm.red[t & 1][3][prow[q]][uw];
-                    const float4 gxv = gxb[q][s2];
+                    float4 gxv;
+                    if constexpr (XIN) {
+                        const f32x4 xv = sm.rb[(t >> 2) & 1][4 * (t & 3) + prow[q]][uw];
+                        gxv = make_float4(xv[0] + addv[q][0], xv[1] + addv[q][1], xv[2] + addv[q][2], xv[3] + addv[q][3]);
+                    } else
+                        gxv = gxb[q][s2];
                     auto sg_ = [](float x) { return (LV_P16_ABL & 4) ? 0.5f + 0.25f * x : lv_sigmoid_fast(x); };
                     auto th_ = [](float x) { return (LV_P16_ABL & 4) ? 0.9f * x : lv_tanh_fast(x); };
                     const float ig = sg_(gxv.x + ((q0[0] + q1[0]) + (q2[0] + q3[0])));
@@ -360,6 +458,7 @@
                     put(hx_g + (long)((t + 1) & 1) * hx_par + (long)prow[q] * (PH / 2) + (punit >> 1),
                         ((gran_t)(uint32_t)(t + 2) << 32) | (gran_t)(mine | (next << 16)));
             }
+            if ((s2 & 3) == 3) x_product(((t + 1) >> 2) & 1);
             LV_TRACE_MARK(t, 5);
         }
     }
@@ -865,6 +964,37 @@
         if (R <= 4) LV_LAUNCH_RESIDENT((lstm_fwd_persist_k16_kernel<4, false>), grid, block, 0, stream, p);
         else if (R <= 8) LV_LAUNCH_RESIDENT((lstm_fwd_persist_k16_kernel<8, false>), grid, block, 0, stream, p);
         else LV_LAUNCH_RESIDENT((lstm_fwd_persist_k16_kernel<16, false>), grid, block, 0, stream, p);
+    }
+    LV_CHECK_LAUNCH();
+    return LV_OK;
+}
+
+extern "C" int lv_lstm_fwd_bf16_persist16_x(const void* x16, long ldx, const void* wih16, int ni, const float* addend,
+                                            long addend_row_stride, const float* wpk, float* hs, float* cs, float* saved, float* xch,
+                                            int* status, int T, int B, int R, int flags, int H, void* stream) {
+    if (!x16 || !wih16 || !addend || !wpk || !hs || !cs || !saved || !xch || !status) return LV_ERR_ARG;
+    if (T < 0 || B <= 0 || H <= 0 || ni <= 0 || ldx < ni || addend_row_stride < 0) return LV_ERR_SHAPE;
+    if (H != PH || ni != XNI || !check_R(B, R) || R > 4) return LV_ERR_UNSUPPORTED;
+    if (addend_row_stride != 0 && addend_row_stride < 4 * PH) return LV_ERR_SHAPE;
+    if ((((uintptr_t)wpk) & 15) != 0 || (((uintptr_t)saved) & 15) != 0 || (((uintptr_t)xch) & 15) != 0 || (((uintptr_t)x16) & 15) != 0 ||
+        (((uintptr_t)wih16) & 15) != 0 || (((uintptr_t)addend) & 15) != 0 || (ldx & 7) != 0 || (addend_row_stride & 3) != 0)
+        return LV_ERR_ALIGN;
+    if (lv_device_cus() < PGROUPS * PMEMBERS) return LV_ERR_UNSUPPORTED;
+    if (T == 0) return LV_OK;
+    char* const xb = reinterpret_cast<char*>(xch);
+    const int dbl = (flags >> 1) & 1, half = dbl ? (flags >> 2) & 1 : 0;
+    gran_t* hx = reinterpret_cast<gran_t*>(xb + XCH_FWD_OFF[half]);
+    if (!dbl) (void)hipMemsetAsync(hx, 0, (size_t)XCH_FWD16_BYTES, (hipStream_t)stream);
+    Fwd16P p{nullptr, reinterpret_cast<const uint4*>(wpk), hs, cs, saved, hx, status, T, B, R,
+             dbl ? reinterpret_cast<uint4*>(xb + XCH_FWD_OFF[1 - half]) : nullptr, XCH_FWD16_BYTES / 16,
+             static_cast<const uint16_t*>(x16), ldx, static_cast<const uint16_t*>(wih16), addend, addend_row_stride};
+    const dim3 grid(PGROUPS * PMEMBERS), block(256);
+    if (flags & 32) {
+        if (flags & 1) LV_LAUNCH_RESIDENT((lstm_fwd_persist_k16_kernel<4, true, true, true>), grid, block, 0, stream, p);
+        else LV_LAUNCH_RESIDENT((lstm_fwd_persist_k16_kernel<4, false, true, true>), grid, block, 0, stream, p);
+    } else {
+        if (flags & 1) LV_LAUNCH_RESIDENT((lstm_fwd_persist_k16_kernel<4, true, false, true>), grid, block, 0, stream, p);
+        else LV_LAUNCH_RESIDENT((lstm_fwd_persist_k16_kernel<4, false, false, true>), grid, block, 0, stream, p);
     }
     LV_CHECK_LAUNCH();
     return LV_OK;
diff --git a/vae_lagging_encoder_amd/engine.py b/vae_lagging_encoder_amd/engine.py
--- a/vae_lagging_encoder_amd/engine.py
+++ b/vae_lagging_encoder_amd/engine.py
@@ -377,6 +377,27 @@
 def _persistent_ok(eng, img, B, H, device, max_b):
     return (eng.precision == "bf16" and img is not None and eng.persistent and H == _PERSIST_H and B <= max_b
             and torch.device(device).type == "cuda" and torch.cuda.get_device_properties(device).multi_processor_count >= 256)
+
+
+FUSED_GX = os.environ.get("LVAE_FUSED_GX", "1") != "0"
+FUSED_GX_ENC = True
+FUSED_GX_DEC = True
+_FUSED_GX_NI = 512
+
+
+def _fused_gx_ok(eng, img, B, H, ni, device, layer_on):
+    if not (FUSED_GX and layer_on and ni == _FUSED_GX_NI and eng.ws_evictable and _persistent_ok(eng, img, B, H, device, _PERSIST_MAX_B)):
+        return False
+    if _persist_rows(eng, B) > 4:
+        return False
+    return not (torch.cuda.is_current_stream_capturing() or (eng._wimg is not None and getattr(eng._wimg, "xstate", {}).get("captured")))
+
+
+def _gx_buffer(c, w, rows, H):
+    if w.Gx is None:
+        w.Gx = c.f32(rows, 4 * H)
+        c.grew(w.ws_key, rows * 4 * H * 4)
+    return w.Gx
 
 
 def weights_version(eng):
@@ -547,7 +568,9 @@
             raise _lib.LvaeError("%s: %s is on %s, x on %s" % (what, name, t.device, dev))
 
 
-def _lstm_forward(eng, lib, s, img, w, Gx, whh, mask, scale, hdrop, T, B, H, device, steps=None):
+def _lstm_forward(eng, lib, s, img, w, Gx, whh, mask, scale, hdrop, T, B, H, device, steps=None, xin=None):
+    if xin is not None and not (steps is None and _persistent_ok(eng, img, B, H, device, _PERSIST_MAX_B)):
+        raise _lib.LvaeError("the fused input projection exists in the persistent forward only")
     args = (Gx, whh, P(w.hs), P(w.cs), P(w.gates), mask, scale, hdrop)
     w.saved_layout = ("canonical", T, B, 0)
     if steps is not None:
@@ -565,8 +588,12 @@
         need = lib.lv_lstm_persist16_saved_floats(T, rows)
         if w.gates.numel() < need:
             w.gates = torch.empty(need, dtype=torch.float32, device=w.gates.device)
-        lib.lv_lstm_fwd_bf16_persist16(Gx, P(wi.fwd16), P(w.hs), P(w.cs), P(w.gates), P(wi.xch), P(eng.status), T, B, rows,
-                                       eng.persist_flags | _xch_flags(wi, "f", rows, device, T) | (32 if getattr(wi, "h16", False) else 0), H, s)
+        flags = eng.persist_flags | _xch_flags(wi, "f", rows, device, T) | (32 if getattr(wi, "h16", False) else 0)
+        if xin is not None:
+            lib.lv_lstm_fwd_bf16_persist16_x(P(img.X), img.ni, P(wi.W), img.ni, xin[0], xin[1], P(wi.fwd16), P(w.hs), P(w.cs),
+                                             P(w.gates), P(wi.xch), P(eng.status), T, B, rows, flags, H, s)
+        else:
+            lib.lv_lstm_fwd_bf16_persist16(Gx, P(wi.fwd16), P(w.hs), P(w.cs), P(w.gates), P(wi.xch), P(eng.status), T, B, rows, flags, H, s)
         w.saved_layout = ("persist16", T, B, rows)
     else:
         lib.lv_lstm_fwd_bf16_ug(*args, P(w.lstm_ws), T, B, H, s)
@@ -651,7 +678,7 @@
     def usable(precision, native16, ni, H):
         return precision == "bf16" and native16 and ni % 8 == 0 and H % 8 == 0
 
-    def forward(self, lib, s, X, W16, Gx, add_a, add_b, rows, wsc, addend_um=None, gather=None, h16=False):
+    def forward(self, lib, s, X, W16, Gx, add_a, add_b, rows, wsc, addend_um=None, gather=None, h16=False, product=True):
         TB, ni, H = self.TB, self.ni, self.H
         if addend_um is not None:
             addend = addend_um
@@ -666,6 +693,8 @@
             emb, ids, ids_stride, keep, kscale, T, B, V = gather
             assert keep is None
             lib.lv_cvt_h16_f32(emb, ni, TB, ni, 0, ids, ids_stride, B, V, P(self.X), ni, P(self.XT), self.ldr, s)
+            if not product:
+                return addend, 4 * H if rows > 1 else 0
             ws = _gemm_ws(lib, s)
             with _prof("gemm_bf16", 2.0 * TB * 4 * H * ni):
                 lib.lv_gemm_h16(TB, 4 * H, ni, 1.0, P(self.X), ni, W16, ni, Gx, 4 * H, 0, addend, 4 * H if rows > 1 else 0, rows, None, 0, 1,
@@ -676,6 +705,8 @@
             lib.lv_embed_gather_b16(emb, ids, ids_stride, keep, kscale, T, B, ni, V, P(self.X), ni, P(self.XT), self.ldr, s)
         else:
             lib.lv_cvt_bf16_f32(X, ni, TB, ni, P(self.X), ni, P(self.XT), self.ldr, s)
+        if not product:
+            return addend, 4 * H if rows > 1 else 0
         _gemm16(lib, s, 0, TB, 4 * H, ni, P(self.X), ni, W16, ni, Gx, 4 * H,
                 add1=addend, ld1=4 * H if rows > 1 else 0, mod1=rows)
 
@@ -851,7 +882,7 @@
         def build():
             w = _NS()
             w.X = c.f32(T * B, ni)
-            w.Gx = c.f32(T * B, 4 * H)
+            w.Gx, w.ws_key = None, (B, T)
             w.hs = torch.zeros(T + 1, B, H, dtype=torch.float32, device=c.device)
             w.cs = torch.zeros(T + 1, B, H, dtype=torch.float32, device=c.device)
             w.gates = c.f32(_saved_floats(self, T, B, H))
@@ -893,6 +924,11 @@
         self._sort = _sorted_tokens(self, lib, s, x, x_key, T, T, B, V, w)
         biases = dict(add1=P(v["lstm.bias_ih_l0"]), ld1=0, mod1=1, add2=P(v["lstm.bias_hh_l0"]), ld2=0, mod2=1)
         gx_unit_major = True
+        xin = None
+        fuse_gx = (img is not None and not exact and steps is None and getattr(self, "gx_round", None) is None
+                   and _fused_gx_ok(self, img, B, H, ni, x.device, FUSED_GX_ENC))
+        if not fuse_gx:
+            _gx_buffer(self.wsc, w, T * B, H)
         if split:
             self._exact_forward_split(lib, s, img, w, x, T, B, V, ni, H)
         elif img is not None and "gx" in exact:
@@ -908,8 +944,8 @@
                 gx_unit_major = True
         elif img is not None:
             wi = self.refresh_weight_images(B, x.device)
-            img.forward(lib, s, None, P(wi.W), P(w.Gx), P(v["lstm.bias_ih_l0"]), P(v["lstm.bias_hh_l0"]), 1, self.wsc,
-                        gather=(P(v["embed.weight"]), P(x), T, None, 1.0, T, B, V), h16=self._h16_now)
+            xin = img.forward(lib, s, None, P(wi.W), None if fuse_gx else P(w.Gx), P(v["lstm.bias_ih_l0"]), P(v["lstm.bias_hh_l0"]), 1,
+                              self.wsc, gather=(P(v["embed.weight"]), P(x), T, None, 1.0, T, B, V), h16=self._h16_now, product=not fuse_gx)
         else:
             _gemm(lib, s, 0, 1, T * B, 4 * H, ni, P(w.X), ni, P(v["lstm.weight_ih_l0"]), ni, P(w.Gx), 4 * H,
                   prec=self.precision, **biases)
@@ -922,7 +958,8 @@
             self._exact_recurrence(lib, s, img, w, gx_unit_major, T, B, H, x.device)
         else:
             with _prof("lstm_fwd_enc", float(T), 1 if _persistent_ok(self, img, B, H, x.device, _PERSIST_MAX_B) else T):
-                _lstm_forward(self, lib, s, img, w, P(w.Gx), P(v["lstm.weight_hh_l0"]), None, 1.0, None, T, B, H, x.device, steps=steps)
+                _lstm_forward(self, lib, s, img, w, None if fuse_gx else P(w.Gx), P(v["lstm.weight_hh_l0"]), None, 1.0, None, T, B, H,
+                              x.device, steps=steps, xin=xin)
         if head is not None and not fused_ends_ok(B, nz2 // 2, head[0].shape[1]):
             eps, z, kl = head
             _gemm(lib, s, 0, 1, B, nz2, H, P(w.hs, T * B * H), H, P(v["linear.weight"]), H, P(w.mulv), nz2)
@@ -1152,7 +1189,7 @@
                 w.x_rep = torch.empty(Bd, Td + 1, dtype=torch.int64, device=c.device)
                 w.Zp_um = c.f32(Bd, 4 * H)
             w.Zp = c.f32(Bd, 4 * H)
-            w.Gx = c.f32(Td * Bd, 4 * H)
+            w.Gx, w.ws_key = None, key
             w.hs = c.f32(Td + 1, Bd, H)
             w.cs = c.f32(Td + 1, Bd, H)
             w.gates = c.f32(_saved_floats(self, Td, Bd, H))
@@ -1276,6 +1313,11 @@
             lib.lv_tanh_f32(P(w.cs), P(w.hs), Bd * H, s)
             _gemm(lib, s, 0, 1, Bd, 4 * H, nz, P(z2), nz, P(wih, ni), ni + nz, P(w.Zp), 4 * H,
                   add1=P(v["lstm.bias_ih_l0"]), ld1=0, mod1=1, add2=P(v["lstm.bias_hh_l0"]), ld2=0, mod2=1)
+        xin = None
+        fuse_gx = (ns == 1 and img is not None and steps is None and _fused_gx_ok(self, img, Bd, H, ni, x.device, FUSED_GX_DEC)
+                   and self._b16(Bd, Td, ns) is not None)
+        if not fuse_gx:
+            _gx_buffer(self.wsc, w, Td * Bd, H)
         if ns > 1:
             zp = w.Zp
             if img is not None and not fused:
@@ -1289,10 +1331,11 @@
             lib.lv_gx_expand_add_f32(P(w.Gxw), P(zp), P(w.Gx), Td, B, ns, 4 * H, s)
         elif img is not None:
             wi = self.refresh_weight_images(B, x.device)
+            gxp = None if fuse_gx else P(w.Gx)
             if fused:
-                img.forward(lib, s, None, P(wi.W), P(w.Gx), None, None, B, self.wsc, addend_um=P(w.Zp), gather=gather)
+                xin = img.forward(lib, s, None, P(wi.W), gxp, None, None, B, self.wsc, addend_um=P(w.Zp), gather=gather, product=not fuse_gx)
             else:
-                img.forward(lib, s, None, P(wi.W), P(w.Gx), P(w.Zp), None, B, self.wsc, gather=gather)
+                xin = img.forward(lib, s, None, P(wi.W), gxp, P(w.Zp), None, B, self.wsc, gather=gather, product=not fuse_gx)
         else:
             _gemm(lib, s, 0, 1, Td * B, 4 * H, ni, P(w.X), ni, P(wih), ni + nz, P(w.Gx), 4 * H,
                   add1=P(w.Zp), ld1=4 * H, mod1=B, prec=self.precision)
@@ -1300,7 +1343,8 @@
         late_mask = b16 is not None and _persistent_ok(self, img, Bd, H, x.device, _PERSIST_MAX_B)
         with _prof("lstm_fwd_dec", float(Td), 1 if _persistent_ok(self, img, Bd, H, x.device, _PERSIST_MAX_B) else Td):
             if late_mask:
-                _lstm_forward(self, lib, s, img, w, P(w.Gx), P(v["lstm.weight_hh_l0"]), None, 1.0, None, Td, Bd, H, x.device)
+                _lstm_forward(self, lib, s, img, w, None if fuse_gx else P(w.Gx), P(v["lstm.weight_hh_l0"]), None, 1.0, None, Td, Bd, H,
+                              x.device, xin=xin)
             else:
                 _lstm_forward(self, lib, s, img, w, P(w.Gx), P(v["lstm.weight_hh_l0"]), P(mask_out), sc_out, P(w.O), Td, Bd, H, x.device,
                               steps=steps)
```

After: 12070, median of 6. 1.04x the previous value.
